# codename0og/codename-rvc-fork-3

Measured on AMD Instinct MI355X. Metric: 48 kHz audio samples/sec end-to-end VC, higher is better.
Workload: dtype f32 (vocoder ResBlock convs and upsamplers, HuBERT, RMVPE's U-Net convs: fp32 operands as exact bf16x3 splits on the bf16 matrix cores -- six products of order <= 2^-16 per multiply-add, fp32 accumulate; everything else fp32 / fp64)

## Files before the change

### codename-rvc-fork-3_amd/csrc/attention.hip

```cpp
#include <stdlib.h>

#include "common.h"

namespace rvc {

constexpr int ATT_W = 10;
constexpr int ATT_NREL = 2 * ATT_W + 1;

__device__ __forceinline__ float fast_exp2(float x) { return __builtin_amdgcn_exp2f(x); }

struct AttParams {
    const float *qkv;
    const float *emb_k;
    const float *emb_v;
    float *out;
    float *part_o;
    float *part_ml;
    int64_t T;
    int n_heads, n_splits, tiles_per_split;
    float scale_log2e;
};

template <int D, bool REL>
__global__ void __launch_bounds__(64) __attribute__((amdgpu_waves_per_eu(1, 2)))
attention_qkv_kernel(const AttParams p) {
    constexpr int NJ = D / 8;
    constexpr int ND = D / 32;
    __shared__ float rel_s[REL ? 32 * 33 : 1];
    __shared__ float band_s[REL ? 32 * 33 : 1];
    const int lane = threadIdx.x, j = lane & 31, h = lane >> 5;
    const int64_t T = p.T;
    const int n_heads = p.n_heads;
    const int64_t q0 = (int64_t)blockIdx.x * 32;
    const int head = blockIdx.y % n_heads;
    const int64_t b = blockIdx.y / n_heads;
    const int split = blockIdx.z;
    const int64_t rs = (int64_t)3 * n_heads * D;
    const float *qp = p.qkv + b * T * rs + (int64_t)head * D;
    const char *kp = reinterpret_cast<const char *>(qp + (int64_t)n_heads * D);
    const char *vp = reinterpret_cast<const char *>(qp + (int64_t)2 * n_heads * D);
    const uint32_t rs_b = (uint32_t)rs * 4u;
    const int nt_all = (int)((T + 31) / 32);
    const int t_begin = split * p.tiles_per_split;
    const int t_end = min(nt_all, t_begin + p.tiles_per_split);
    const bool partial = (T & 31) != 0;

    f32x4 qf[NJ];
    {
        const int64_t q = q0 + j < T ? q0 + j : T - 1;
        const float *ptr = qp + q * rs + 4 * h;
#pragma unroll
        for (int jj = 0; jj < NJ; ++jj) qf[jj] = *reinterpret_cast<const f32x4 *>(ptr + 8 * jj) * p.scale_log2e;
    }
    auto load_k = [&](f32x4 (&ka)[NJ], int t) __attribute__((always_inline)) {
        const int64_t key = (int64_t)t * 32 + j;
        const uint32_t off = (uint32_t)(key < T ? key : T - 1) * rs_b + 16u * h;
#pragma unroll
        for (int jj = 0; jj < NJ; ++jj) ka[jj] = *reinterpret_cast<const f32x4 *>(kp + off + 32u * jj);
    };
    uint32_t voff[16];
#pragma unroll
    for (int r = 0; r < 16; ++r) voff[r] = (uint32_t)((r & 3) + 8 * (r >> 2) + 4 * h) * rs_b + 4u * j;
    auto load_v = [&](float (&va)[16][ND], int t) __attribute__((always_inline)) {
        const char *vt = vp + (int64_t)t * 32 * rs_b;
        if (t + 1 < nt_all || !partial) {
#pragma unroll
            for (int r = 0; r < 16; ++r)
#pragma unroll
                for (int dt = 0; dt < ND; ++dt) va[r][dt] = *reinterpret_cast<const float *>(vt + voff[r] + 128u * dt);
        } else {
#pragma unroll
            for (int r = 0; r < 16; ++r) {
                const int64_t key = (int64_t)t * 32 + (r & 3) + 8 * (r >> 2) + 4 * h;
                const uint32_t off = (uint32_t)(key < T ? key : T - 1) * rs_b + 4u * j;
#pragma unroll
                for (int dt = 0; dt < ND; ++dt) va[r][dt] = *reinterpret_cast<const float *>(vp + off + 128u * dt);
            }
        }
    };
    auto scores = [&](const f32x4 (&ka)[NJ]) __attribute__((always_inline)) {
        f32x16 s;
#pragma unroll
        for (int r = 0; r < 16; ++r) s[r] = 0.f;
#pragma unroll
        for (int jj = 0; jj < NJ; ++jj)
#pragma unroll
            for (int e = 0; e < 4; ++e) s = mfma32(ka[jj][e], qf[jj][e], s);
        return s;
    };

    f32x16 o[ND];
#pragma unroll
    for (int dt = 0; dt < ND; ++dt)
#pragma unroll
        for (int r = 0; r < 16; ++r) o[dt][r] = 0.f;
    float m = -INFINITY, l = 0.f;

    if constexpr (REL) {
        f32x4 ek[NJ];
        const float *eptr = p.emb_k + (int64_t)(j < ATT_NREL ? j : 0) * D + 4 * h;
#pragma unroll
        for (int jj = 0; jj < NJ; ++jj) {
            ek[jj] = *reinterpret_cast<const f32x4 *>(eptr + 8 * jj);
            if (j >= ATT_NREL) ek[jj] = f32x4{0.f, 0.f, 0.f, 0.f};
        }
        const f32x16 rl = scores(ek);
#pragma unroll
        for (int r = 0; r < 16; ++r) {
            const int rr = (r & 3) + 8 * (r >> 2) + 4 * h;
            rel_s[j * 33 + rr] = rl[r];
            band_s[j * 33 + rr] = 0.f;
        }
        __syncthreads();
    }

    auto step = [&](int t, f32x4 (&k_cur)[NJ], const f32x4 (&k_next)[NJ], f32x16 &s_cur, f32x16 &s_next)
                    __attribute__((always_inline)) {
        float va[16][ND];
        load_v(va, t);
        if (t + 2 < t_end) load_k(k_cur, t + 2);
        if (t + 1 < t_end) s_next = scores(k_next);
        const bool near_diag = REL && (int64_t)t * 32 + 31 + ATT_W >= q0 && (int64_t)t * 32 <= q0 + 31 + ATT_W;
        int rr[16];
        if constexpr (REL) {
            if (near_diag) {
#pragma unroll
                for (int r = 0; r < 16; ++r) {
                    rr[r] = (int)((int64_t)t * 32 + (r & 3) + 8 * (r >> 2) + 4 * h - (q0 + j)) + ATT_W;
                    const bool in = rr[r] >= 0 && rr[r] < ATT_NREL;
                    const float add = rel_s[j * 33 + (in ? rr[r] : 0)];
                    s_cur[r] += in ? add : 0.f;
                }
            }
        }
        if (t + 1 == nt_all && partial) {
#pragma unroll
            for (int r = 0; r < 16; ++r)
                s_cur[r] = (int64_t)t * 32 + (r & 3) + 8 * (r >> 2) + 4 * h < T ? s_cur[r] : -INFINITY;
        }
        float mloc = s_cur[0];
#pragma unroll
        for (int r = 1; r < 16; ++r) mloc = fmaxf(mloc, s_cur[r]);
        mloc = fmaxf(mloc, __shfl_xor(mloc, 32));
        if (__any(mloc > m + 8.f)) {
            const float m_new = fmaxf(m, mloc);
            const float alpha = fast_exp2(m - m_new);
            l *= alpha;
#pragma unroll
            for (int dt = 0; dt < ND; ++dt)
#pragma unroll
                for (int r = 0; r < 16; ++r) o[dt][r] *= alpha;
            if constexpr (REL) {
#pragma unroll
                for (int r = 0; r < 16; ++r) band_s[j * 33 + 2 * r + h] *= alpha;
            }
            m = m_new;
        }
        float psum = 0.f;
#pragma unroll
        for (int r = 0; r < 16; ++r) {
            s_cur[r] = fast_exp2(s_cur[r] - m);
            psum += s_cur[r];
        }
        l += psum;
        if constexpr (REL) {
            if (near_diag) {
#pragma unroll
                for (int r = 0; r < 16; ++r)
                    if (rr[r] >= 0 && rr[r] < ATT_NREL) band_s[j * 33 + rr[r]] = s_cur[r];
            }
        }
#pragma unroll
        for (int r = 0; r < 16; ++r)
#pragma unroll
            for (int dt = 0; dt < ND; ++dt) o[dt] = mfma32(va[r][dt], s_cur[r], o[dt]);
    };

    if (t_begin < t_end) {
        f32x4 ka[NJ], kb[NJ];
        f32x16 sa, sb;
        load_k(ka, t_begin);
        if (t_begin + 1 < t_end) load_k(kb, t_begin + 1);
        sa = scores(ka);
        for (int t = t_begin; t < t_end; t += 2) {
            step(t, ka, kb, sa, sb);
            if (t + 1 < t_end) step(t + 1, kb, ka, sb, sa);
        }
    }
    if constexpr (REL) {
        __syncthreads();
#pragma unroll
        for (int sidx = 0; sidx < 16; ++sidx) {
            const int r = 2 * sidx + h;
            const float bval = band_s[j * 33 + r];
            const float *ev = p.emb_v + (int64_t)(r < ATT_NREL ? r : 0) * D + j;
#pragma unroll
            for (int dt = 0; dt < ND; ++dt) o[dt] = mfma32(ev[32 * dt], bval, o[dt]);
        }
    }
    l += __shfl_xor(l, 32);
    if (q0 + j < T) {
        if (p.n_splits == 1) {
            const float inv = 1.f / l;
            float *op = p.out + (b * T + q0 + j) * (int64_t)n_heads * D + (int64_t)head * D + 4 * h;
#pragma unroll
            for (int dt = 0; dt < ND; ++dt)
#pragma unroll
                for (int g = 0; g < 4; ++g) {
                    f32x4 v = {o[dt][4 * g], o[dt][4 * g + 1], o[dt][4 * g + 2], o[dt][4 * g + 3]};
                    *reinterpret_cast<f32x4 *>(op + 32 * dt + 8 * g) = v * inv;
                }
        } else {
            const int64_t row = ((b * n_heads + head) * p.n_splits + split) * T + q0 + j;
            float *op = p.part_o + row * D + 4 * h;
#pragma unroll
            for (int dt = 0; dt < ND; ++dt)
#pragma unroll
                for (int g = 0; g < 4; ++g) {
                    f32x4 v = {o[dt][4 * g], o[dt][4 * g + 1], o[dt][4 * g + 2], o[dt][4 * g + 3]};
                    *reinterpret_cast<f32x4 *>(op + 32 * dt + 8 * g) = v;
                }
            if (h == 0) {
                p.part_ml[row * 2] = m;
                p.part_ml[row * 2 + 1] = l;
            }
        }
    }
}

__global__ void __launch_bounds__(256)
attention_combine_kernel(const float *__restrict__ part_o, const float *__restrict__ part_ml, float *__restrict__ out,
                         int64_t T, int n_heads, int n_splits, int D) {
    const int64_t idx = (int64_t)blockIdx.x * 256 + threadIdx.x;
    const int d4n = D / 4;
    const int64_t total = (int64_t)gridDim.y * n_heads * T * d4n;
    (void)total;
    const int64_t b = blockIdx.y;
    if (idx >= (int64_t)n_heads * T * d4n) return;
    const int d4 = (int)(idx % d4n);
    const int64_t t = (idx / d4n) % T;
    const int head = (int)(idx / d4n / T);
    float mstar = -INFINITY;
    for (int s = 0; s < n_splits; ++s) mstar = fmaxf(mstar, part_ml[(((b * n_heads + head) * n_splits + s) * T + t) * 2]);
    f32x4 acc = {0.f, 0.f, 0.f, 0.f};
    float lsum = 0.f;
    for (int s = 0; s < n_splits; ++s) {
        const int64_t row = ((b * n_heads + head) * n_splits + s) * T + t;
        const float wgt = fast_exp2(part_ml[row * 2] - mstar);
        lsum += wgt * part_ml[row * 2 + 1];
        acc += *reinterpret_cast<const f32x4 *>(part_o + row * D + 4 * d4) * wgt;
    }
    *reinterpret_cast<f32x4 *>(out + (b * T + t) * (int64_t)n_heads * D + (int64_t)head * D + 4 * d4) = acc * (1.f / lsum);
}

struct AttBfParams {
    const float *qkv;
    const void *frag;
    float *out, *part_o, *part_ml;
    int64_t T;
    int n_heads, n_splits, tiles_per_split;
    float scale_log2e;
};
constexpr int ABF_TILE_BYTES = 24 * 1024, ABF_NW = 8;
typedef void __attribute__((address_space(3))) *abf_lptr_t;

__device__ __forceinline__ void abf_split8(const float (&v)[8], u32x4 (&out)[3]) {
    f32x2 r[4] = {f32x2{v[0], v[1]}, f32x2{v[2], v[3]}, f32x2{v[4], v[5]}, f32x2{v[6], v[7]}};
#pragma unroll
    for (int level = 0; level < 3; ++level)
#pragma unroll
        for (int q = 0; q < 4; ++q) {
            const unsigned w = split_word(r[q]);
            out[level][q] = w;
            if (level < 2) r[q] = r[q] - f32x2{__uint_as_float(w << 16), __uint_as_float(w & 0xffff0000u)};
        }
}

__global__ void __launch_bounds__(512) attention_pack_kv_kernel(const float *__restrict__ qkv, unsigned char *__restrict__ frag, int64_t T, int n_heads) {
    const int lane = threadIdx.x & 63, wave = threadIdx.x >> 6, i = lane & 31, h = lane >> 5;
    const int64_t tile = blockIdx.x, n_tiles = gridDim.x;
    const int head = blockIdx.y % n_heads;
    const int64_t b = blockIdx.y / n_heads;
    const int64_t rs = (int64_t)3 * n_heads * 64;
    const float *base = qkv + b * T * rs + (int64_t)head * 64;
    float v[8];
    int piece0;
    if (wave < 4) {
        const int64_t key = tile * 32 + i;
        const float *ptr = base + (int64_t)n_heads * 64 + (key < T ? key : 0) * rs + 16 * wave + 8 * h;
#pragma unroll
        for (int e = 0; e < 8; ++e) v[e] = key < T ? ptr[e] : 0.f;
        piece0 = wave * 3;
    } else {
        const int db = (wave - 4) >> 1, ks = wave & 1;
#pragma unroll
        for (int e = 0; e < 8; ++e) {
            const int r = 8 * ks + e;
            const int64_t key = tile * 32 + (r & 3) + 8 * (r >> 2) + 4 * h;
            v[e] = key < T ? base[(int64_t)2 * n_heads * 64 + key * rs + 32 * db + i] : 0.f;
        }
        piece0 = 12 + (db * 2 + ks) * 3;
    }
    u32x4 d[3];
    abf_split8(v, d);
    unsigned char *dst = frag + ((int64_t)blockIdx.y * n_tiles + tile) * ABF_TILE_BYTES + lane * 16;
#pragma unroll
    for (int sp = 0; sp < 3; ++sp) *reinterpret_cast<u32x4 *>(dst + (piece0 + sp) * 1024) = d[sp];
}

template <int DBG = 0>
__global__ void __launch_bounds__(512) __attribute__((amdgpu_waves_per_eu(2, 2)))
attention_bf_kernel(const AttBfParams p) {
    extern __shared__ __attribute__((aligned(16))) unsigned char abf_smem[];
    const int tid = threadIdx.x, lane = tid & 63, j = lane & 31, h = lane >> 5;
    const int wave = __builtin_amdgcn_readfirstlane(tid >> 6);
    const int64_t T = p.T;
    const int n_heads = p.n_heads;
    const int64_t q0 = ((int64_t)blockIdx.x * ABF_NW + wave) * 32;
    const bool active = q0 < T;
    const int head = blockIdx.y % n_heads;
    const int64_t b = blockIdx.y / n_heads;
    const int split = blockIdx.z;
    const int64_t rs = (int64_t)3 * n_heads * 64;
    const int nt_all = (int)((T + 31) / 32);
    const int t_begin = split * p.tiles_per_split;
    const int t_end = (DBG & 16) ? min(nt_all, t_begin + 1) : min(nt_all, t_begin + p.tiles_per_split);
    const bool partial = (T & 31) != 0;
    constexpr int ia6[6] = {0, 1, 0, 2, 1, 0}, ib6[6] = {2, 1, 1, 0, 0, 0};

    const int64_t n_frag = (int64_t)gridDim.y * nt_all * ABF_TILE_BYTES;
    const __amdgpu_buffer_rsrc_t frs = __builtin_amdgcn_make_buffer_rsrc((void *)p.frag, 0, (int)n_frag, RSRC_RAW32);
    const int bh_base = (int)((int64_t)blockIdx.y * nt_all) * ABF_TILE_BYTES;
    constexpr int HALF = ABF_TILE_BYTES / 2;
    auto dma = [&](int tk, int kslot, int tv, int vslot) __attribute__((always_inline)) {
#pragma unroll
        for (int n = 0; n < 3; ++n) {
            const int piece = wave + ABF_NW * n;
            if (piece < 12) {
                if (tk >= 0) __builtin_amdgcn_raw_ptr_buffer_load_lds(frs, (abf_lptr_t)(abf_smem + kslot * HALF + piece * 1024), 16, 16 * lane, bh_base + tk * ABF_TILE_BYTES + piece * 1024, 0, 0);
            } else {
                if (tv >= 0) __builtin_amdgcn_raw_ptr_buffer_load_lds(frs, (abf_lptr_t)(abf_smem + 2 * HALF + vslot * HALF + (piece - 12) * 1024), 16, 16 * lane, bh_base + tv * ABF_TILE_BYTES + piece * 1024, 0, 0);
            }
        }
    };
    if (t_begin < t_end) {
        dma(t_begin, 0, t_begin, 0);
        dma(t_begin + 1 < t_end ? t_begin + 1 : -1, 1, -1, 0);
    }
    u32x4 qf[4][3];
    {
        const int64_t q = q0 + j < T ? q0 + j : T - 1;
        const float *ptr = p.qkv + b * T * rs + (int64_t)head * 64 + q * rs + 8 * h;
#pragma unroll
        for (int ks = 0; ks < 4; ++ks) {
            const f32x4 lo = *reinterpret_cast<const f32x4 *>(ptr + 16 * ks) * p.scale_log2e, hi = *reinterpret_cast<const f32x4 *>(ptr + 16 * ks + 4) * p.scale_log2e;
            const float v[8] = {lo.x, lo.y, lo.z, lo.w, hi.x, hi.y, hi.z, hi.w};
            abf_split8(v, qf[ks]);
        }
    }
    auto scores = [&](int kslot) __attribute__((always_inline)) {
        const unsigned char *kk = abf_smem + kslot * HALF + lane * 16;
        f32x16 sc;
#pragma unroll
        for (int r = 0; r < 16; ++r) sc[r] = 0.f;
#pragma unroll
        for (int ks = 0; ks < 4; ++ks) {
            bf16x8 kf[3];
#pragma unroll
            for (int sp = 0; sp < 3; ++sp) if (!(DBG & 4)) kf[sp] = __builtin_bit_cast(bf16x8, *reinterpret_cast<const u32x4 *>(kk + (ks * 3 + sp) * 1024));
#pragma unroll
            for (int i = 0; i < 6; ++i) if (!(DBG & 1)) sc = __builtin_amdgcn_mfma_f32_32x32x16_bf16(kf[ia6[i]], __builtin_bit_cast(bf16x8, qf[ks][ib6[i]]), sc, 0, 0, 0);
        }
        return sc;
    };

    f32x16 o[2];
#pragma unroll
    for (int db = 0; db < 2; ++db)
#pragma unroll
        for (int r = 0; r < 16; ++r) o[db][r] = 0.f;
    float m = -INFINITY, l = 0.f;

    if (t_begin < t_end) {
        asm volatile("s_waitcnt vmcnt(0)" ::: "memory");
        __builtin_amdgcn_s_barrier();
        f32x16 s_cur, s_next;
        if (active) s_cur = scores(0);
        asm volatile("s_waitcnt lgkmcnt(0)" ::: "memory");
        __builtin_amdgcn_s_barrier();
        for (int t = t_begin; t < t_end; ++t) {
            const int kb = (t - t_begin) & 1;
            if (!(DBG & 8)) dma(t + 2 < t_end ? t + 2 : -1, kb, t + 1 < t_end ? t + 1 : -1, kb ^ 1);
            if (active) {
                if (t + 1 < t_end) s_next = scores(kb ^ 1);
                f32x16 &sc = s_cur;
                if (t + 1 == nt_all && partial) {
#pragma unroll
                    for (int r = 0; r < 16; ++r) sc[r] = (int64_t)t * 32 + (r & 3) + 8 * (r >> 2) + 4 * h < T ? sc[r] : -INFINITY;
                }
                float mloc = sc[0];
#pragma unroll
                for (int r = 1; r < 16; ++r) mloc = fmaxf(mloc, sc[r]);
                mloc = fmaxf(mloc, __shfl_xor(mloc, 32));
                if (__any(mloc > m + 8.f)) {
                    const float m_new = fmaxf(m, mloc);
                    const float alpha = fast_exp2(m - m_new);
                    l *= alpha;
#pragma unroll
                    for (int db = 0; db < 2; ++db)
#pragma unroll
                        for (int r = 0; r < 16; ++r) o[db][r] *= alpha;
                    m = m_new;
                }
                float psum = 0.f;
                if (!(DBG & 2)) {
#pragma unroll
                    for (int r = 0; r < 16; ++r) {
                        sc[r] = fast_exp2(sc[r] - m);
                        psum += sc[r];
                    }
                }
                l += psum;
                u32x4 pf[2][3];
#pragma unroll
                for (int ks = 0; ks < 2; ++ks) {
                    const float v[8] = {sc[8 * ks], sc[8 * ks + 1], sc[8 * ks + 2], sc[8 * ks + 3], sc[8 * ks + 4], sc[8 * ks + 5], sc[8 * ks + 6], sc[8 * ks + 7]};
                    if (!(DBG & 2)) abf_split8(v, pf[ks]);
                }
                const unsigned char *vv = abf_smem + 2 * HALF + kb * HALF + lane * 16;
#pragma unroll
                for (int ks = 0; ks < 2; ++ks)
#pragma unroll
                    for (int db = 0; db < 2; ++db) {
                        bf16x8 vf[3];
#pragma unroll
                        for (int sp = 0; sp < 3; ++sp)
                            if (!(DBG & 4)) vf[sp] = __builtin_bit_cast(bf16x8, *reinterpret_cast<const u32x4 *>(vv + ((db * 2 + ks) * 3 + sp) * 1024));
#pragma unroll
                        for (int i = 0; i < 6; ++i)
                            if (!(DBG & 1)) o[db] = __builtin_amdgcn_mfma_f32_32x32x16_bf16(vf[ia6[i]], __builtin_bit_cast(bf16x8, pf[ks][ib6[i]]), o[db], 0, 0, 0);
                    }
                s_cur = s_next;
            }
            asm volatile("s_waitcnt vmcnt(0) lgkmcnt(0)" ::: "memory");
            __builtin_amdgcn_s_barrier();
        }
    }
    l += __shfl_xor(l, 32);
    if (active && q0 + j < T) {
        if (p.n_splits == 1) {
            const float inv = 1.f / l;
            float *op = p.out + (b * T + q0 + j) * (int64_t)n_heads * 64 + (int64_t)head * 64 + 4 * h;
#pragma unroll
            for (int db = 0; db < 2; ++db)
#pragma unroll
                for (int g = 0; g < 4; ++g) {
                    f32x4 v = {o[db][4 * g], o[db][4 * g + 1], o[db][4 * g + 2], o[db][4 * g + 3]};
                    *reinterpret_cast<f32x4 *>(op + 32 * db + 8 * g) = v * inv;
                }
        } else {
            const int64_t row = ((b * n_heads + head) * p.n_splits + split) * T + q0 + j;
            float *op = p.part_o + row * 64 + 4 * h;
#pragma unroll
            for (int db = 0; db < 2; ++db)
#pragma unroll
                for (int g = 0; g < 4; ++g) {
                    f32x4 v = {o[db][4 * g], o[db][4 * g + 1], o[db][4 * g + 2], o[db][4 * g + 3]};
                    *reinterpret_cast<f32x4 *>(op + 32 * db + 8 * g) = v;
                }
            if (h == 0) {
                p.part_ml[row * 2] = m;
                p.part_ml[row * 2 + 1] = l;
            }
        }
    }
}

static bool att_bf_enabled() {
    static const int on = knob("RVC_ATT_BF", 1);
    return on != 0;
}
static int choose_splits_bf(int64_t n_frames, int n_heads, int batch) {
    const int64_t nt = ceil_div(n_frames, 32);
    const int64_t groups = ceil_div(n_frames, 32 * ABF_NW) * n_heads * batch;
    int best = 1;
    double best_cost = 1e30;
    for (int s = 1; s <= 8 && s <= nt; ++s) {
        const double cost = (double)ceil_div(groups * s, 256) / s + 0.02 * s;
        if (cost < best_cost - 1e-9) { best_cost = cost; best = s; }
    }
    return best;
}
static size_t att_bf_workspace(int batch, int64_t n_frames, int n_heads, size_t *off_ml, size_t *off_frag) {
    const int splits = choose_splits_bf(n_frames, n_heads, batch);
    const size_t rows = splits == 1 ? 0 : (size_t)batch * n_heads * splits * (size_t)n_frames;
    const size_t o_bytes = align_up(rows * 64 * sizeof(float), 256), ml_bytes = align_up(rows * 2 * sizeof(float), 256);
    if (off_ml) *off_ml = o_bytes;
    if (off_frag) *off_frag = o_bytes + ml_bytes;
    return o_bytes + ml_bytes + align_up((size_t)batch * n_heads * (size_t)ceil_div(n_frames, 32) * ABF_TILE_BYTES, 256);
}

static int choose_splits(int64_t n_frames, int n_heads, int batch) {
    static const int forced = knob("RVC_ATT_SPLITS", 0);
    const int64_t nt = ceil_div(n_frames, 32);
    const int64_t pairs = nt * n_heads * batch;
    int best = 1;
    double best_cost = 1e30;
    for (int s = 1; s <= 8 && s <= nt; ++s) {
        const double cost = (double)ceil_div(pairs * s, 1024) / s + 0.02 * s;
        if (cost < best_cost - 1e-9) { best_cost = cost; best = s; }
    }
    if (forced > 0 && forced <= nt) best = forced;
    return best;
}

}

using namespace rvc;

static bool attention_shape_ok(int batch, int64_t n_frames, int n_heads, int head_dim) {
    return batch > 0 && n_heads > 0 && n_frames >= 0 && (head_dim == 64 || head_dim == 96);
}

extern "C" int rvc_attention_workspace_bytes(int batch, int64_t n_frames, int n_heads, int head_dim, size_t *bytes) {
    if (!bytes) return fail("rvc_attention_workspace_bytes: null pointer");
    if (head_dim != 64 && head_dim != 96) return fail("rvc_attention_workspace_bytes: head_dim must be 64 or 96, got %d", head_dim);
    if (!attention_shape_ok(batch, n_frames, n_heads, head_dim)) return fail("rvc_attention_workspace_bytes: bad shape");
    const int splits = choose_splits(n_frames, n_heads, batch);
    const size_t rows = (size_t)batch * n_heads * splits * (size_t)n_frames;
    *bytes = splits == 1 ? 256 : align_up(rows * head_dim * sizeof(float), 256) + align_up(rows * 2 * sizeof(float), 256);
    if (head_dim == 64 && att_bf_enabled()) {
        const size_t bf = att_bf_workspace(batch, n_frames, n_heads, nullptr, nullptr);
        if (bf > *bytes) *bytes = bf;
    }
    return 0;
}

template <int D, bool REL>
static int launch_attention(AttParams &p, int batch, hipStream_t stream) {
    dim3 grid((unsigned)ceil_div(p.T, 32), (unsigned)(p.n_heads * batch), (unsigned)p.n_splits);
    hipLaunchKernelGGL((attention_qkv_kernel<D, REL>), grid, dim3(64), 0, stream, p);
    RVC_LAUNCH_CHECK();
    if (p.n_splits > 1) {
        const int64_t work = (int64_t)p.n_heads * p.T * (D / 4);
        hipLaunchKernelGGL(attention_combine_kernel, dim3((unsigned)ceil_div(work, 256), (unsigned)batch), dim3(256), 0, stream,
                           p.part_o, p.part_ml, p.out, p.T, p.n_heads, p.n_splits, D);
        RVC_LAUNCH_CHECK();
    }
    return 0;
}

extern "C" int rvc_attention_qkv_f32(const float *qkv_dev, const float *emb_rel_k_dev, const float *emb_rel_v_dev,
                                     float *out_dev, int batch, int64_t n_frames, int n_heads, int head_dim, float scale,
                                     void *workspace_dev, size_t workspace_bytes, void *stream) {
    if (!qkv_dev || !out_dev) return fail("rvc_attention_qkv_f32: null pointer");
    if (head_dim != 64 && head_dim != 96) return fail("rvc_attention_qkv_f32: head_dim must be 64 or 96, got %d", head_dim);
    if ((emb_rel_k_dev == nullptr) != (emb_rel_v_dev == nullptr)) return fail("rvc_attention_qkv_f32: emb_rel_k and emb_rel_v go together");
    if (!attention_shape_ok(batch, n_frames, n_heads, head_dim)) return fail("rvc_attention_qkv_f32: bad shape");
    if (n_frames == 0) return 0;
    if ((int64_t)n_frames * 3 * n_heads * head_dim * 4 >= ((int64_t)1 << 32))
        return fail("rvc_attention_qkv_f32: one batch element of %lld frames exceeds the 4 GB the kernel addresses", (long long)n_frames);
    if (head_dim == 64 && !emb_rel_k_dev && att_bf_enabled() && fits_2gib((int64_t)batch * n_heads * ceil_div(n_frames, 32), ABF_TILE_BYTES)) {
        size_t off_ml = 0, off_frag = 0;
        const size_t need = att_bf_workspace(batch, n_frames, n_heads, &off_ml, &off_frag);
        if (!workspace_dev || workspace_bytes < need) return fail("rvc_attention_qkv_f32: workspace too small (%zu < %zu)", workspace_bytes, need);
        AttBfParams q;
        q.qkv = qkv_dev; q.out = out_dev; q.T = n_frames; q.n_heads = n_heads; q.scale_log2e = scale * 1.4426950408889634f;
        q.n_splits = choose_splits_bf(n_frames, n_heads, batch);
        q.tiles_per_split = (int)ceil_div(ceil_div(n_frames, 32), q.n_splits);
        q.part_o = (float *)workspace_dev; q.part_ml = (float *)((char *)workspace_dev + off_ml); q.frag = (char *)workspace_dev + off_frag;
        hipStream_t st = (hipStream_t)stream;
        const unsigned n_tiles = (unsigned)ceil_div(n_frames, 32);
        const dim3 bgrid((unsigned)ceil_div(n_frames, 32 * ABF_NW), (unsigned)(n_heads * batch), (unsigned)q.n_splits);
        const auto run = [&](auto kernel) -> int {
            if (reserve_whole_cu((const void *)kernel, "rvc_attention_qkv_f32")) return 1;
            hipLaunchKernelGGL(attention_pack_kv_kernel, dim3(n_tiles, (unsigned)(n_heads * batch)), dim3(512), 0, st, qkv_dev, (unsigned char *)q.frag, q.T, n_heads);
            RVC_LAUNCH_CHECK();
            hipLaunchKernelGGL(kernel, bgrid, dim3(512), LDS_WHOLE_CU, st, q);
            RVC_LAUNCH_CHECK();
            return 0;
        };
        int dbg = 0;
#ifdef RVC_ABLATE
        static const int dbg_knob = knob("RVC_ATT_DBG", 0);
        dbg = dbg_knob;
#endif
        int rc;
        switch (dbg) {
#ifdef RVC_ABLATE
            case 1: rc = run(attention_bf_kernel<1>); break;
            case 2: rc = run(attention_bf_kernel<2>); break;
            case 4: rc = run(attention_bf_kernel<4>); break;
            case 8: rc = run(attention_bf_kernel<8>); break;
            case 16: rc = run(attention_bf_kernel<16>); break;
            case 7: rc = run(attention_bf_kernel<7>); break;
#endif
            default: rc = run(attention_bf_kernel<0>); break;
        }
        if (rc) return 1;
        if (q.n_splits > 1) {
            const int64_t work = (int64_t)n_heads * q.T * (64 / 4);
            hipLaunchKernelGGL(attention_combine_kernel, dim3((unsigned)ceil_div(work, 256), (unsigned)batch), dim3(256), 0, st,
                               q.part_o, q.part_ml, q.out, q.T, n_heads, q.n_splits, 64);
            RVC_LAUNCH_CHECK();
        }
        return 0;
    }
    AttParams p;
    p.qkv = qkv_dev; p.emb_k = emb_rel_k_dev; p.emb_v = emb_rel_v_dev; p.out = out_dev;
    p.T = n_frames; p.n_heads = n_heads; p.scale_log2e = scale * 1.4426950408889634f;
    p.n_splits = choose_splits(n_frames, n_heads, batch);
    p.tiles_per_split = (int)ceil_div(ceil_div(n_frames, 32), p.n_splits);
    p.part_o = nullptr; p.part_ml = nullptr;
    if (p.n_splits > 1) {
        size_t need = 0;
        if (rvc_attention_workspace_bytes(batch, n_frames, n_heads, head_dim, &need)) return 1;
        if (!workspace_dev || workspace_bytes < need) return fail("rvc_attention_qkv_f32: workspace too small (%zu < %zu)", workspace_bytes, need);
        const size_t rows = (size_t)batch * n_heads * p.n_splits * (size_t)n_frames;
        p.part_o = (float *)workspace_dev;
        p.part_ml = (float *)((char *)workspace_dev + align_up(rows * head_dim * sizeof(float), 256));
    }
    const bool rel = emb_rel_k_dev != nullptr;
    hipStream_t st = (hipStream_t)stream;
    if (head_dim == 64) return rel ? launch_attention<64, true>(p, batch, st) : launch_attention<64, false>(p, batch, st);
    return rel ? launch_attention<96, true>(p, batch, st) : launch_attention<96, false>(p, batch, st);
}
```

### codename-rvc-fork-3_amd/csrc/bf16x3.h

```cpp
#pragma once

#include <hip/hip_runtime.h>

namespace rvc {

typedef __bf16 bf16x2 __attribute__((ext_vector_type(2)));
typedef __bf16 bf16x8 __attribute__((ext_vector_type(8)));
typedef float f32x2 __attribute__((ext_vector_type(2)));
typedef unsigned u32x2 __attribute__((ext_vector_type(2)));
typedef unsigned u32x4 __attribute__((ext_vector_type(4)));

constexpr int RSRC_RAW32 = 0x00020000;
constexpr unsigned BUF_OOB = 0x80000000u;

__device__ __forceinline__ float sub_np(float a, float b) {
    float r;
    asm("v_sub_f32 %0, %1, %2" : "=v"(r) : "v"(a), "v"(b));
    return r;
}
__device__ __forceinline__ float add_np(float a, float b) {
    float r;
    asm("v_add_f32 %0, %1, %2" : "=v"(r) : "v"(a), "v"(b));
    return r;
}
__device__ __forceinline__ float mul_np(float a, float b) {
    float r;
    asm("v_mul_f32 %0, %1, %2" : "=v"(r) : "v"(a), "v"(b));
    return r;
}

__device__ __forceinline__ unsigned split_word(f32x2 v) { return __builtin_bit_cast(unsigned, __builtin_convertvector(v, bf16x2)); }
__device__ __forceinline__ f32x2 split_rest(f32x2 v, unsigned w) { return v - f32x2{__uint_as_float(w << 16), __uint_as_float(w & 0xffff0000u)}; }
__device__ __forceinline__ void split3(f32x2 v, unsigned w[3]) {
#pragma unroll
    for (int level = 0; level < 3; ++level) {
        w[level] = split_word(v);
        if (level < 2) v = split_rest(v, w[level]);
    }
}
__device__ __forceinline__ void split3_np(float a, float b, unsigned w[3]) {
#pragma unroll
    for (int level = 0; level < 3; ++level) {
        const unsigned ww = split_word(f32x2{a, b});
        w[level] = ww;
        if (level < 2) {
            a = sub_np(a, __uint_as_float(ww << 16));
            b = sub_np(b, __uint_as_float(ww & 0xffff0000u));
        }
    }
}

}
```

### codename-rvc-fork-3_amd/csrc/linbf.hip

```cpp
#include <stdlib.h>

#include <mutex>
#include <vector>

#include "conv.h"

namespace rvc {

struct LinBfParams {
    const void *a = nullptr;
    const void *xs = nullptr;
    const float *bias = nullptr;
    float *y = nullptr;
    void *ys = nullptr;
    int M = 0, K = 0;
    int64_t N = 0, n_pad = 0;
    int mode = 0;
    int64_t x_row_stride = 0, x_plane = 0;
    int steps_per_part = 0;
    int n_col_blocks = 0;
};

constexpr int LBF_BN = 128, LBF_NTH = 512;
constexpr int LBF_SLAB_STEP = 12 * 1024;
constexpr int LBF_B_CHUNK = 3 * LBF_BN * 64;
typedef void __attribute__((address_space(3))) *lbf_lptr_t;

template <int MI>
struct LbfGeom {
    static constexpr int BM = 64 * MI;
    static constexpr int A_STEP = 2 * MI * 3 * 1024;
    static constexpr int D = MI == 2 ? 2 : 1;
    static constexpr int A_RING = 2 * (D + 1), B_RING = D + 1;
    static constexpr int NPIECE = 2 * 2 * MI * 3 + 24;
    static constexpr int UPW = (NPIECE + 7) / 8;
    static constexpr int LDS_USED = A_RING * A_STEP + B_RING * LBF_B_CHUNK;
    static_assert(LDS_USED <= 163840, "");
};

template <int MI>
__global__ void __launch_bounds__(LBF_NTH) __attribute__((amdgpu_waves_per_eu(2, 2)))
linbf_kernel(const LinBfParams p) {
    using GM = LbfGeom<MI>;
    constexpr int BM = GM::BM, A_STEP = GM::A_STEP, D = GM::D, A_RING = GM::A_RING, B_RING = GM::B_RING, NPIECE = GM::NPIECE, UPW = GM::UPW;
    extern __shared__ __attribute__((aligned(16))) unsigned char lbf_smem[];
    unsigned char *const a_ring = lbf_smem;
    unsigned char *const b_ring = lbf_smem + A_RING * A_STEP;
    const int tid = threadIdx.x, lane = tid & 63;
    const int wave = __builtin_amdgcn_readfirstlane(tid >> 6);
    __builtin_assume(wave >= 0 && wave < 8);
    const int wm = wave >> 2, wn = wave & 3;
    const int half = lane >> 5, l31 = lane & 31;
    const int n_m = p.M / BM;
    const int xcd = blockIdx.x & 7, slot = blockIdx.x >> 3;
    const int pairs = p.n_col_blocks * n_m, per_xcd = (pairs + 7) / 8;
    const int w = xcd * per_xcd + slot;
    if (slot >= per_xcd || w >= pairs) return;
    const int col_blk = w / n_m, mblk = w - col_blk * n_m, part = blockIdx.y;
    const int m0 = mblk * BM;
    const int64_t n0 = (int64_t)col_blk * LBF_BN;
    const int n_chunks = p.steps_per_part / 2, s_first = part * p.steps_per_part;
    const int K = p.K;

    const __amdgpu_buffer_rsrc_t ars = __builtin_amdgcn_make_buffer_rsrc((void *)p.a, 0, (int)((int64_t)p.M * K * 6), RSRC_RAW32);
    const __amdgpu_buffer_rsrc_t xrs = __builtin_amdgcn_make_buffer_rsrc((void *)p.xs, 0, (int)(3 * p.x_plane * 2), RSRC_RAW32);
    const int slab_row = (K / 16) * LBF_SLAB_STEP;
    const int plane = (int)(p.x_plane * 2);
    const int row_bytes = (int)(p.x_row_stride * 2);
    const int b_r = lane >> 2, b_j = lane & 3;
    auto dma = [&](int c) __attribute__((always_inline)) {
        const int sg = s_first + 2 * c;
        unsigned char *bslot = b_ring + (c % B_RING) * LBF_B_CHUNK;
#pragma unroll
        for (int i = 0; i < UPW; ++i) {
            int pc = wave + 8 * i;
            if (pc >= NPIECE) pc -= 8;
            if (pc < 12 * MI) {
                const int st = pc / (6 * MI), f = pc - st * (6 * MI);
                const int rb = (m0 >> 5) + f / 3, sp = f - (f / 3) * 3;
                unsigned char *aslot = a_ring + ((2 * c + st) % A_RING) * A_STEP;
                __builtin_amdgcn_raw_ptr_buffer_load_lds(ars, (lbf_lptr_t)(aslot + f * 1024), 16, 16 * lane,
                                                         (rb >> 2) * slab_row + (sg + st) * LBF_SLAB_STEP + ((rb & 3) * 3 + sp) * 1024, 0, 0);
            } else {
                const int q = pc - 12 * MI, sp = q >> 3, r16 = q & 7;
                const int row = r16 * 16 + b_r;
                const int seg = b_j ^ ((row >> 2) & 3);
                const int voff = (int)(n0 + row) * row_bytes + seg * 16;
                __builtin_amdgcn_raw_ptr_buffer_load_lds(xrs, (lbf_lptr_t)(bslot + sp * (LBF_BN * 64) + r16 * 1024), 16, voff, sp * plane + sg * 32, 0, 0);
            }
        }
    };

    f32x16 acc[MI];
#pragma unroll
    for (int mi = 0; mi < MI; ++mi)
#pragma unroll
        for (int r = 0; r < 16; ++r) acc[mi][r] = 0.f;
    auto rd = [&](const unsigned char *ptr) __attribute__((always_inline)) {
        return __builtin_bit_cast(bf16x8, *reinterpret_cast<const u32x4 *>(ptr));
    };
    const int nrow = wn * 32 + l31;
    const int b_lane = nrow * 64, b_sw = (nrow >> 2) & 3;

    auto wait_newer = [&](int newer) __attribute__((always_inline)) {
        if (newer >= 1 && D >= 2) asm volatile("s_waitcnt vmcnt(%0)" ::"n"(UPW) : "memory");
        else asm volatile("s_waitcnt vmcnt(0)" ::: "memory");
    };
    static_assert(D <= 2, "wait_newer distinguishes 0 and 1 newer requests");
#pragma unroll
    for (int c = 0; c < D; ++c)
        if (c < n_chunks) dma(c);
    wait_newer((n_chunks - 1 < D - 1) ? n_chunks - 1 : D - 1);
    lds_barrier();
    for (int c = 0; c < n_chunks; ++c) {
        if (c + D < n_chunks) dma(c + D);
        const unsigned char *bslot = b_ring + (c % B_RING) * LBF_B_CHUNK + b_lane;
#pragma unroll
        for (int t = 0; t < 2; ++t) {
            const unsigned char *ab = a_ring + ((2 * c + t) % A_RING) * A_STEP + wm * MI * 3 * 1024 + lane * 16;
            bf16x8 fa[MI][3], fb[3];
#pragma unroll
            for (int sp = 0; sp < 3; ++sp) fb[sp] = rd(bslot + sp * (LBF_BN * 64) + (((2 * t + half) ^ b_sw) * 16));
#pragma unroll
            for (int mi = 0; mi < MI; ++mi)
#pragma unroll
                for (int sp = 0; sp < 3; ++sp) fa[mi][sp] = rd(ab + (mi * 3 + sp) * 1024);
            constexpr int ia[6] = {2, 0, 1, 1, 0, 0}, ib[6] = {0, 2, 1, 0, 1, 0};
#pragma unroll
            for (int i = 0; i < 6; ++i)
#pragma unroll
                for (int mi = 0; mi < MI; ++mi)
                    acc[mi] = __builtin_amdgcn_mfma_f32_32x32x16_bf16(fa[mi][ia[i]], fb[ib[i]], acc[mi], 0, 0, 0);
        }
        const int newer = (n_chunks - 2 - c) < (D - 1) ? (n_chunks - 2 - c) : (D - 1);
        wait_newer(newer);
        lds_barrier();
    }

    if (p.mode == 1) {
        const int64_t n = n0 + nrow;
        const bool live = n < p.N;
#pragma unroll
        for (int mi = 0; mi < MI; ++mi) {
            const int mb = m0 + wm * 32 * MI + mi * 32;
#pragma unroll
            for (int rp = 0; rp < 2; ++rp) {
                f32x2 v[2][2];
#pragma unroll
                for (int g = 0; g < 2; ++g) {
                    f32x4 o;
#pragma unroll
                    for (int r = 0; r < 4; ++r) o[r] = acc[mi][4 * (2 * rp + g) + r];
                    if (p.bias) o += *reinterpret_cast<const f32x4 *>(p.bias + mb + 4 * half + 8 * (2 * rp + g));
#pragma unroll
                    for (int r = 0; r < 4; ++r) o[r] = 0.5f * o[r] * (1.f + erff(o[r] * 0.70710678118654752f));
                    v[g][0] = f32x2{o[0], o[1]};
                    v[g][1] = f32x2{o[2], o[3]};
                }
#pragma unroll
                for (int sp = 0; sp < 3; ++sp) {
                    unsigned w[2][2];
#pragma unroll
                    for (int g = 0; g < 2; ++g)
#pragma unroll
                        for (int h = 0; h < 2; ++h) {
                            w[g][h] = split_word(v[g][h]);
                            v[g][h] = split_rest(v[g][h], w[g][h]);
                        }
                    const unsigned s0 = half ? w[0][0] : w[1][0], s1 = half ? w[0][1] : w[1][1];
                    const unsigned r0 = (unsigned)__shfl_xor((int)s0, 32, 64), r1 = (unsigned)__shfl_xor((int)s1, 32, 64);
                    const u32x4 out = half ? u32x4{r0, r1, w[1][0], w[1][1]} : u32x4{w[0][0], w[0][1], r0, r1};
                    const int m = mb + 16 * rp + 8 * half;
                    if (live) *reinterpret_cast<u32x4 *>(reinterpret_cast<unsigned char *>(p.ys) + (((int64_t)sp * p.n_pad + n) * p.M + m) * 2) = out;
                }
            }
        }
        return;
    }
#pragma unroll
    for (int mi = 0; mi < MI; ++mi) {
        const int64_t n = n0 + nrow;
        if (n >= p.N) continue;
        const int mb = m0 + wm * 32 * MI + mi * 32 + 4 * half;
#pragma unroll
        for (int rg = 0; rg < 4; ++rg) {
            const int m = mb + 8 * rg;
            f32x4 o;
#pragma unroll
            for (int r = 0; r < 4; ++r) o[r] = acc[mi][4 * rg + r];
            if (p.mode == 2) {
                *reinterpret_cast<f32x4 *>(p.y + ((int64_t)part * p.N + n) * p.M + m) = o;
                continue;
            }
            if (p.bias) o += *reinterpret_cast<const f32x4 *>(p.bias + m);
            if (p.mode == 0) {
                *reinterpret_cast<f32x4 *>(p.y + n * p.M + m) = o;
                continue;
            }
#pragma unroll
            for (int r = 0; r < 4; ++r) o[r] = 0.5f * o[r] * (1.f + erff(o[r] * 0.70710678118654752f));
            *reinterpret_cast<f32x4 *>(p.y + n * p.M + m) = o;
        }
    }
}

__global__ void __launch_bounds__(256) split_rows_kernel(const float *__restrict__ x, unsigned char *__restrict__ xs, int64_t n_rows,
                                                          int64_t n_pad, int k) {
    const int64_t i4 = (int64_t)blockIdx.x * 256 + threadIdx.x;
    const int64_t total4 = n_rows * k / 4;
    if (i4 >= total4) return;
    const f32x4 v = *reinterpret_cast<const f32x4 *>(x + i4 * 4);
    f32x2 v0 = {v.x, v.y}, v1 = {v.z, v.w};
#pragma unroll
    for (int sp = 0; sp < 3; ++sp) {
        const unsigned w0 = split_word(v0), w1 = split_word(v1);
        *reinterpret_cast<u32x2 *>(xs + ((int64_t)sp * n_pad * k + i4 * 4) * 2) = u32x2{w0, w1};
        v0 = split_rest(v0, w0);
        v1 = split_rest(v1, w1);
    }
}

__device__ __forceinline__ float ln_row_mean(float sum, float inv_m) {
    float mean = sum * inv_m;
    asm volatile("" : "+v"(mean));
    return mean;
}

template <int PER_LANE>
__global__ void __launch_bounds__(256) ln_reduce_kernel(const float *__restrict__ parts, int n_parts, const float *__restrict__ bias,
                                                         const float *__restrict__ res, const float *__restrict__ gamma,
                                                         const float *__restrict__ beta, float eps, float *__restrict__ y,
                                                         unsigned char *__restrict__ ys, int64_t n_rows, int64_t n_pad) {
    constexpr int M = 64 * PER_LANE, Q = PER_LANE / 4;
    const int lane = threadIdx.x & 63;
    const int64_t n = (int64_t)blockIdx.x * 4 + (threadIdx.x >> 6);
    if (n >= n_rows) return;
    f32x4 v[Q];
#pragma unroll
    for (int q = 0; q < Q; ++q) {
        const int m = (q * 64 + lane) * 4;
        f32x4 a = bias ? *reinterpret_cast<const f32x4 *>(bias + m) : f32x4{0.f, 0.f, 0.f, 0.f};
        for (int s = 0; s < n_parts; ++s) a += *reinterpret_cast<const f32x4 *>(parts + ((int64_t)s * n_rows + n) * M + m);
        if (res) a += *reinterpret_cast<const f32x4 *>(res + n * M + m);
        v[q] = a;
    }
    float sum = 0.f;
#pragma unroll
    for (int q = 0; q < Q; ++q) sum += (v[q].x + v[q].y) + (v[q].z + v[q].w);
#pragma unroll
    for (int o = 32; o > 0; o >>= 1) sum += __shfl_xor(sum, o, 64);
    const float mean = ln_row_mean(sum, 1.f / M);
    float sq = 0.f;
#pragma unroll
    for (int q = 0; q < Q; ++q) {
        const f32x4 d = v[q] - mean;
        sq += (d.x * d.x + d.y * d.y) + (d.z * d.z + d.w * d.w);
    }
#pragma unroll
    for (int o = 32; o > 0; o >>= 1) sq += __shfl_xor(sq, o, 64);
    const float rstd = 1.f / sqrtf(sq * (1.f / M) + eps);
#pragma unroll
    for (int q = 0; q < Q; ++q) {
        const int m = (q * 64 + lane) * 4;
        f32x4 o = (v[q] - mean) * rstd;
        if (gamma) o *= *reinterpret_cast<const f32x4 *>(gamma + m);
        if (beta) o += *reinterpret_cast<const f32x4 *>(beta + m);
        if (y) *reinterpret_cast<f32x4 *>(y + n * M + m) = o;
        if (ys) {
            f32x2 v0 = {o.x, o.y}, v1 = {o.z, o.w};
#pragma unroll
            for (int sp = 0; sp < 3; ++sp) {
                const unsigned w0 = split_word(v0), w1 = split_word(v1);
                *reinterpret_cast<u32x2 *>(ys + (((int64_t)sp * n_pad + n) * M + m) * 2) = u32x2{w0, w1};
                v0 = split_rest(v0, w0);
                v1 = split_rest(v1, w1);
            }
        }
    }
}

template <int MI>
static int linbf_launch(LinBfParams p, int parts, hipStream_t stream) {
    if (reserve_whole_cu((const void *)linbf_kernel<MI>, "linear bf16x3 (pre-split)")) return 1;
    p.n_col_blocks = (int)ceil_div(p.N, LBF_BN);
    const int n_m = p.M / LbfGeom<MI>::BM;
    dim3 grid((unsigned)(ceil_div((int64_t)p.n_col_blocks * n_m, 8) * 8), (unsigned)parts, 1);
    hipLaunchKernelGGL(linbf_kernel<MI>, grid, dim3(LBF_NTH), LDS_WHOLE_CU, stream, p);
    RVC_LAUNCH_CHECK();
    return 0;
}

}

using namespace rvc;

extern "C" int rvc_split_rows_bf16x3(const float *x_dev, void *xs_dev, int64_t n_rows, int64_t n_rows_padded, int k, void *stream) {
    if (!x_dev || !xs_dev) return fail("rvc_split_rows_bf16x3: null pointer");
    if (k % 16 || n_rows_padded < n_rows || n_rows < 0) return fail("rvc_split_rows_bf16x3: k must be a multiple of 16, n_rows_padded >= n_rows");
    if (n_rows == 0) return 0;
    const int64_t total4 = n_rows * k / 4;
    hipLaunchKernelGGL(split_rows_kernel, dim3((unsigned)ceil_div(total4, 256)), dim3(256), 0, (hipStream_t)stream, x_dev,
                       reinterpret_cast<unsigned char *>(xs_dev), n_rows, n_rows_padded, k);
    RVC_LAUNCH_CHECK();
    return 0;
}

namespace {
int linbf_dispatch(const char *who, const void *xs_dev, int64_t x_row_stride, int64_t x_plane, const void *a_dev, const float *bias_dev,
                   float *y_dev, void *ys_dev, int64_t n_rows, int64_t n_rows_padded, int in_features, int out_features, int mode,
                   int k_parts, void *stream) {
    if (!xs_dev || !a_dev) return fail("%s: null pointer", who);
    if (out_features % 128 || in_features % 16) return fail("%s: out_features must be a multiple of 128, in_features of 16", who);
    if (mode < 0 || mode > 3) return fail("%s: mode must be 0 (fp32 + bias), 1 (bias + GELU -> planes), 2 (partial sums) or 3 (bias + GELU -> fp32)", who);
    if ((mode == 1) ? !ys_dev : !y_dev) return fail("%s: the output of mode %d is missing", who, mode);
    if (k_parts < 1 || (in_features / 32) % k_parts || in_features % 32) return fail("%s: in_features must be a multiple of 32 and k_parts divide in_features / 32", who);
    if (k_parts > 1 && mode != 2) return fail("%s: several K parts only produce partial sums (mode 2)", who);
    if (n_rows_padded % LBF_BN || n_rows_padded < n_rows) return fail("%s: n_rows_padded must be a multiple of 128 and >= n_rows", who);
    if (!fits_2gib((int64_t)out_features * in_features, 6) || !fits_2gib(3 * x_plane, 2) ||
        !fits_2gib((n_rows_padded + LBF_BN) * x_row_stride, 2))
        return fail("%s: an operand exceeds 2 GiB", who);
    if (x_row_stride % 8) return fail("%s: rows must start on 16-byte boundaries", who);
    if (n_rows <= 0) return 0;
    LinBfParams p;
    p.a = a_dev; p.xs = xs_dev; p.bias = bias_dev; p.y = y_dev; p.ys = ys_dev;
    p.M = out_features; p.K = in_features; p.N = n_rows; p.n_pad = n_rows_padded; p.mode = mode;
    p.x_row_stride = x_row_stride; p.x_plane = x_plane;
    p.steps_per_part = in_features / 16 / k_parts;
    const int64_t cols = ceil_div(n_rows, LBF_BN);
    const int cus = 256;
    auto cost = [&](int rows_per_block, double rel) {
        if (out_features % rows_per_block) return 1e30;
        return (double)ceil_div(cols * (out_features / rows_per_block) * k_parts, cus) * rel;
    };
    static const int by_cu_time = knob("RVC_LBF_TP", 0);
    if (by_cu_time) {
        auto cu_time = [&](int rows_per_block, double rel) { return out_features % rows_per_block ? 1e30 : cols * (out_features / rows_per_block) * k_parts * rel; };
        const double t128 = cu_time(128, 1.0), t192 = cu_time(192, 1.5 * 0.85), t256 = cu_time(256, 1.85);
        if (t192 <= t128 && t192 <= t256) return linbf_launch<3>(p, k_parts, (hipStream_t)stream);
        if (t256 < t128) return linbf_launch<4>(p, k_parts, (hipStream_t)stream);
        return linbf_launch<2>(p, k_parts, (hipStream_t)stream);
    }
    const double c128 = cost(128, 1.0), c192 = cost(192, 1.5 * 0.85), c256 = cost(256, 1.85);
    if (c256 < c128 && c256 <= c192) return linbf_launch<4>(p, k_parts, (hipStream_t)stream);
    const bool use192 = c192 < c128;
    return use192 ? linbf_launch<3>(p, k_parts, (hipStream_t)stream) : linbf_launch<2>(p, k_parts, (hipStream_t)stream);
}
}

extern "C" int rvc_linear_bf16x3_presplit(const void *xs_dev, const void *a_dev, const float *bias_dev, float *y_dev, void *ys_dev,
                                          int64_t n_rows, int64_t n_rows_padded, int in_features, int out_features, int mode, int k_parts,
                                          void *stream) {
    return linbf_dispatch("rvc_linear_bf16x3_presplit", xs_dev, in_features, n_rows_padded * in_features, a_dev, bias_dev, y_dev, ys_dev,
                          n_rows, n_rows_padded, in_features, out_features, mode, k_parts, stream);
}

extern "C" int rvc_conv1d_frames_bf16x3(const void *xs_dev, int64_t n_frames_in, int64_t n_frames_in_padded, int channels, int taps,
                                        int stride, const void *a_dev, const float *bias_dev, float *y_dev, void *ys_dev,
                                        int64_t n_frames_out_padded, int out_channels, int mode, void *stream) {
    if (taps < 1 || stride < 1 || channels < 8 || n_frames_in_padded < n_frames_in) return fail("rvc_conv1d_frames_bf16x3: bad argument");
    if (mode == 2) return fail("rvc_conv1d_frames_bf16x3: modes 0 (fp32 + bias), 1 (bias + GELU -> planes), 3 (bias + GELU -> fp32)");
    const int64_t n_out = n_frames_in >= taps ? (n_frames_in - taps) / stride + 1 : 0;
    return linbf_dispatch("rvc_conv1d_frames_bf16x3", xs_dev, (int64_t)stride * channels, n_frames_in_padded * channels, a_dev, bias_dev,
                          y_dev, ys_dev, n_out, n_frames_out_padded, taps * channels, out_channels, mode, 1, stream);
}

extern "C" int rvc_bias_residual_layernorm_bf16x3(const float *parts_dev, int n_parts, const float *bias_dev, const float *res_dev,
                                                  const float *gamma_dev, const float *beta_dev, float eps, float *y_dev, void *ys_dev,
                                                  int64_t n_rows, int64_t n_rows_padded, int features, void *stream) {
    if (!parts_dev || (!y_dev && !ys_dev)) return fail("rvc_bias_residual_layernorm_bf16x3: null pointer");
    if (n_parts < 1 || n_rows_padded < n_rows) return fail("rvc_bias_residual_layernorm_bf16x3: bad argument");
    if (n_rows <= 0) return 0;
    dim3 grid((unsigned)ceil_div(n_rows, 4));
    unsigned char *ys = reinterpret_cast<unsigned char *>(ys_dev);
    hipStream_t st = (hipStream_t)stream;
    if (features == 768)
        hipLaunchKernelGGL(ln_reduce_kernel<12>, grid, dim3(256), 0, st, parts_dev, n_parts, bias_dev, res_dev, gamma_dev, beta_dev, eps, y_dev, ys, n_rows, n_rows_padded);
    else if (features == 1024)
        hipLaunchKernelGGL(ln_reduce_kernel<16>, grid, dim3(256), 0, st, parts_dev, n_parts, bias_dev, res_dev, gamma_dev, beta_dev, eps, y_dev, ys, n_rows, n_rows_padded);
    else if (features == 256)
        hipLaunchKernelGGL(ln_reduce_kernel<4>, grid, dim3(256), 0, st, parts_dev, n_parts, bias_dev, res_dev, gamma_dev, beta_dev, eps, y_dev, ys, n_rows, n_rows_padded);
    else
        return fail("rvc_bias_residual_layernorm_bf16x3: features must be 256, 768 or 1024 (HuBERT-base: 768)");
    RVC_LAUNCH_CHECK();
    return 0;
}
```

### codename-rvc-fork-3_amd/rvc_amd/_native.py

```python
from __future__ import annotations

import ctypes
import threading
import os
from ctypes import POINTER, c_char_p, c_float, c_int, c_int64, c_size_t, c_void_p

import torch

_HERE = os.path.dirname(os.path.abspath(__file__))
LIB_PATH = os.path.join(_HERE, "_lib", "librvc_amd.so")
if os.environ.get("RVC_AMD_LIB"):
    LIB_PATH = os.path.abspath(os.environ["RVC_AMD_LIB"])
    print(f"[rvc_amd] RVC_AMD_LIB: loading {LIB_PATH} instead of the product library", flush=True)


class NativeError(RuntimeError):
    pass


if not os.path.isfile(LIB_PATH):
    raise ImportError(
        f"{LIB_PATH} is missing: build it with `python -c 'import __graft_entry__ as g; g.build()'` "
        "(hipcc --offload-arch=gfx950).  rvc_amd has no fallback path without its HIP library.")

_lib = ctypes.CDLL(LIB_PATH)


class DecoderConfig(ctypes.Structure):
    _fields_ = [
        ("kind", c_int), ("sample_rate", c_int), ("in_channels", c_int), ("upsample_initial_channel", c_int),
        ("gin_channels", c_int), ("n_ups", c_int), ("upsample_rates", c_int * 8), ("upsample_kernel_sizes", c_int * 8),
        ("n_res_kernels", c_int), ("res_kernel_sizes", c_int * 4), ("res_dilations", c_int * 4),
        ("n_res_dilations", c_int), ("weight_storage", c_int),
    ]


class DecoderNoise(ctypes.Structure):
    _fields_ = [("src_rand_dev", c_void_p), ("src_randn_dev", c_void_p), ("adain_randn_dev", c_void_p)]


SYMBOLS = {
    "rvc_abi_version": (c_int, []),
    "rvc_last_error": (c_char_p, []),
    "rvc_knn_index_aux_bytes": (c_int, [c_int64, c_int, POINTER(c_size_t)]),
    "rvc_knn_index_build": (c_int, [c_void_p, c_int64, c_int, c_void_p, c_size_t, c_void_p]),
    "rvc_knn_set_mode": (c_int, [c_int]),
    "rvc_knn_rank_candidates": (c_int, [c_void_p, c_void_p, c_int64, c_int, c_void_p, c_int64, c_void_p, c_int, c_int, c_void_p,
                                        c_void_p, c_void_p]),
    "rvc_knn_workspace_bytes": (c_int, [c_int64, c_int64, c_int, c_int, POINTER(c_size_t)]),
    "rvc_knn_search": (c_int, [c_void_p, c_void_p, c_int64, c_int, c_void_p, c_int64, c_int, c_void_p, c_void_p,
                               c_void_p, c_size_t, c_void_p]),
    "rvc_knn_blend": (c_int, [c_void_p, c_int, c_void_p, c_void_p, c_void_p, c_int64, c_int, c_float, c_void_p,
                              c_void_p]),
    "rvc_logmel_workspace_bytes": (c_int, [c_int, c_int64, POINTER(c_size_t)]),
    "rvc_logmel_rmvpe": (c_int, [c_void_p, c_int, c_int64, c_void_p, c_int64, c_void_p, c_size_t, c_void_p]),
    "rvc_mel_create": (c_int, [c_int, c_int, c_int, c_int, c_float, c_float, c_void_p, c_int, POINTER(c_void_p)]),
    "rvc_mel_destroy": (c_int, [c_void_p]),
    "rvc_mel_frames": (c_int, [c_void_p, c_int64, POINTER(c_int64)]),
    "rvc_mel_workspace_bytes": (c_int, [c_void_p, c_int, c_int64, POINTER(c_size_t)]),
    "rvc_mel_forward": (c_int, [c_void_p, c_void_p, c_int, c_int64, c_void_p, c_void_p, c_void_p, c_size_t, c_void_p]),
    "rvc_resample_poly_f64": (c_int, [c_void_p, c_int64, c_int, c_int, c_void_p, c_int64, c_void_p, c_int64, c_void_p]),
    "rvc_filtfilt_workspace_bytes": (c_int, [c_int64, POINTER(c_size_t)]),
    "rvc_filtfilt_order5": (c_int, [c_void_p, c_int64, c_void_p, c_void_p, c_void_p, c_size_t, c_void_p]),
    "rvc_bigru_workspace_bytes": (c_int, [c_int, POINTER(c_size_t)]),
    "rvc_bigru_forward": (c_int, [c_void_p, c_void_p, c_void_p, c_void_p, c_int, c_int64, c_int, c_void_p, c_size_t,
                                  c_void_p]),
    "rvc_bigru_status": (c_int, [c_void_p, c_int, POINTER(c_int), c_void_p]),
    "rvc_bigru_set_spin_limit": (c_int, [ctypes.c_uint]),
    "rvc_attention_workspace_bytes": (c_int, [c_int, c_int64, c_int, c_int, POINTER(c_size_t)]),
    "rvc_attention_qkv_f32": (c_int, [c_void_p, c_void_p, c_void_p, c_void_p, c_int, c_int64, c_int, c_int, c_float,
                                      c_void_p, c_size_t, c_void_p]),
    "rvc_bias_relu_add_f32": (c_int, [c_void_p, c_void_p, c_void_p, c_void_p, c_int, c_int, c_int64, c_int, c_void_p]),
    "rvc_gate_tanh_sigmoid_f32": (c_int, [c_void_p, c_void_p, c_int, c_int, c_int64, c_void_p]),
    "rvc_rownorm_gelu_f32": (c_int, [c_void_p, c_void_p, c_void_p, c_void_p, c_int, c_int, c_int64, ctypes.c_float, c_void_p]),
    "rvc_set_concurrency_hint": (c_int, [c_int]),
    "rvc_decoder_create": (c_int, [POINTER(DecoderConfig), POINTER(c_void_p)]),
    "rvc_decoder_set_tensor": (c_int, [c_void_p, c_char_p, c_void_p, POINTER(c_int64), c_int]),
    "rvc_decoder_finalize": (c_int, [c_void_p]),
    "rvc_decoder_destroy": (c_int, [c_void_p]),
    "rvc_decoder_upp": (c_int, [c_void_p]),
    "rvc_decoder_workspace_bytes": (c_int, [c_void_p, c_int, c_int64, POINTER(c_size_t)]),
    "rvc_decoder_forward": (c_int, [c_void_p, c_void_p, c_void_p, c_void_p, POINTER(DecoderNoise), c_int, c_int64,
                                    c_void_p, c_void_p, c_size_t, c_void_p]),
    "rvc_decoder_window_margin": (c_int, [POINTER(DecoderConfig), POINTER(c_int)]),
    "rvc_decoder_forward_window": (c_int, [c_void_p, c_void_p, c_void_p, c_void_p, POINTER(DecoderNoise), c_int, c_int64, c_int64,
                                           c_int64, c_void_p, c_void_p, c_size_t, c_void_p]),
    "rvc_decoder_set_tap": (c_int, [c_void_p, c_int, c_void_p]),
    "rvc_decoder_set_concurrency_hint": (c_int, [c_void_p, c_int]),
    "rvc_decoder_set_branch_parallel": (c_int, [c_void_p, c_int]),
    "rvc_posconv_bf16x3_weight_bytes": (c_int, [c_int, c_int, c_int, POINTER(c_size_t)]),
    "rvc_posconv_bf16x3_pack_weight": (c_int, [c_void_p, c_int, c_int, c_int, c_void_p, c_void_p]),
    "rvc_posconv_gelu_bf16x3": (c_int, [c_void_p, c_void_p, c_void_p, c_void_p, c_int64, c_int, c_int, c_int, c_int, c_void_p]),
    "rvc_hubert_conv0_workspace_bytes": (c_int, [c_int, POINTER(c_size_t)]),
    "rvc_hubert_conv0_frames_bf16x3": (c_int, [c_void_p, c_int64, c_void_p, c_int, c_int, c_int, c_void_p, c_void_p, c_float, c_void_p,
                                               c_size_t, c_void_p, c_int64, c_void_p]),
    "rvc_conv1d_frames_bf16x3": (c_int, [c_void_p, c_int64, c_int64, c_int, c_int, c_int, c_void_p, c_void_p, c_void_p, c_void_p, c_int64,
                                         c_int, c_int, c_void_p]),
    "rvc_conv1d_pack_weight": (c_int, [c_void_p, c_int, c_int, c_int, c_void_p, c_void_p]),
    "rvc_conv1d_forward": (c_int, [c_void_p, c_void_p, c_void_p, c_void_p, c_void_p, c_void_p, c_int, c_int, c_int,
                                   c_int64, c_int, c_int, c_float, c_float, c_void_p]),
    "rvc_conv1d_wino_pack_weight": (c_int, [c_void_p, c_int, c_int, c_int, c_void_p, c_void_p]),
    "rvc_conv1d_wino_forward": (c_int, [c_void_p, c_void_p, c_void_p, c_void_p, c_void_p, c_void_p, c_int, c_int, c_int,
                                        c_int64, c_int, c_int, c_float, c_float, c_void_p]),
    "rvc_conv1d_winobf_weight_bytes": (c_int, [c_int, c_int, c_int, POINTER(c_size_t)]),
    "rvc_conv1d_winobf_pack_weight": (c_int, [c_void_p, c_int, c_int, c_int, c_void_p, c_void_p]),
    "rvc_conv1d_winobf_forward": (c_int, [c_void_p, c_void_p, c_void_p, c_void_p, c_void_p, c_void_p, c_int, c_int, c_int,
                                          c_int64, c_int, c_int, c_float, c_float, c_void_p]),
    "rvc_resblock_bf16x3_weight_bytes": (c_int, [c_int, c_int, POINTER(c_size_t)]),
    "rvc_resblock_bf16x3_pack_weight": (c_int, [c_void_p, c_void_p, c_int, c_int, c_void_p, c_void_p]),
    "rvc_resblock_bf16x3_forward": (c_int, [c_void_p, c_void_p, c_void_p, c_void_p, c_void_p, c_void_p, c_int, c_int, c_int64, c_int,
                                            c_int, c_float, c_float, c_void_p]),
    "rvc_resblock_bf16w_weight_bytes": (c_int, [c_int, c_int, POINTER(c_size_t)]),
    "rvc_resblock_bf16w_pack_weight": (c_int, [c_void_p, c_void_p, c_int, c_int, c_void_p, c_void_p]),
    "rvc_resblock_bf16w_forward": (c_int, [c_void_p, c_void_p, c_void_p, c_void_p, c_void_p, c_void_p, c_int, c_int, c_int64, c_int,
                                           c_int, c_float, c_float, c_void_p]),
    "rvc_resblock_bf16x3_set_enabled": (c_int, [c_int]),
    "rvc_upsample_bf16x3_weight_bytes": (c_int, [c_int, c_int, c_int, c_int, c_int, c_int, POINTER(c_size_t)]),
    "rvc_upsample_bf16x3_pack_weight": (c_int, [c_void_p, c_void_p, c_void_p, c_int, c_int, c_int, c_int, c_int, c_int, c_void_p, c_void_p]),
    "rvc_upsample_bf16x3_forward": (c_int, [c_void_p, c_void_p, c_int64, c_void_p, c_void_p, c_void_p, c_int, c_int, c_int, c_int64, c_int, c_int,
                                            c_int, c_int, c_int, c_int, c_float, c_void_p]),
    "rvc_conv1d_f16x2_weight_bytes": (c_int, [c_int, c_int, POINTER(c_size_t)]),
    "rvc_conv1d_f16x2_pack_weight": (c_int, [c_void_p, c_int, c_int, c_void_p, c_void_p]),
    "rvc_conv1d_f16x2_forward": (c_int, [c_void_p, c_void_p, c_void_p, c_void_p, c_void_p, c_void_p, c_int, c_int, c_int64, c_int,
                                         c_int, c_float, c_float, c_void_p]),
    "rvc_decoder_set_arithmetic": (c_int, [c_void_p, c_int]),
    "rvc_conv1d_bf16w_weight_bytes": (c_int, [c_int, c_int, POINTER(c_size_t)]),
    "rvc_conv1d_bf16w_pack_weight": (c_int, [c_void_p, c_int, c_int, c_void_p, c_void_p]),
    "rvc_conv1d_bf16w_forward": (c_int, [c_void_p, c_void_p, c_void_p, c_void_p, c_void_p, c_void_p, c_int, c_int, c_int64, c_int,
                                         c_int, c_float, c_float, c_void_p]),
    "rvc_gemm_bf16x3_weight_bytes": (c_int, [c_int, c_int, POINTER(c_size_t)]),
    "rvc_gemm_bf16x3_pack_weight": (c_int, [c_void_p, c_int, c_int, c_int, c_void_p, c_void_p]),
    "rvc_linear_bf16x3": (c_int, [c_void_p, c_void_p, c_void_p, c_void_p, c_void_p, c_int64, c_int, c_int, c_int, c_void_p]),
    "rvc_conv1d_bf16x3": (c_int, [c_void_p, c_void_p, c_void_p, c_void_p, c_int, c_int, c_int, c_int64, c_int, c_int, c_int, c_int,
                                  c_void_p]),
    "rvc_split_rows_bf16x3": (c_int, [c_void_p, c_void_p, c_int64, c_int64, c_int, c_void_p]),
    "rvc_linear_bf16x3_presplit": (c_int, [c_void_p, c_void_p, c_void_p, c_void_p, c_void_p, c_int64, c_int64, c_int, c_int, c_int, c_int,
                                           c_void_p]),
    "rvc_bias_residual_layernorm_bf16x3": (c_int, [c_void_p, c_int, c_void_p, c_void_p, c_void_p, c_void_p, c_float, c_void_p, c_void_p,
                                                   c_int64, c_int64, c_int, c_void_p]),
    "rvc_conv2d_packed_floats": (c_int, [c_int, c_int, c_int, c_int, POINTER(c_size_t)]),
    "rvc_conv2d_pack_weight": (c_int, [c_void_p, c_int, c_int, c_int, c_int, c_void_p, c_void_p]),
    "rvc_conv2d_workspace_bytes": (c_int, [c_int, c_int, c_int, c_int, c_int, c_int, c_int, POINTER(c_size_t)]),
    "rvc_conv2d_bf16x3_supported": (c_int, [c_int, c_int, c_int, c_int]),
    "rvc_conv2d_bf16x3_weight_bytes": (c_int, [c_int, c_int, c_int, c_int, POINTER(c_size_t)]),
    "rvc_conv2d_bf16x3_pack_weight": (c_int, [c_void_p, c_int, c_int, c_int, c_int, c_void_p, c_void_p]),
    "rvc_conv2d_bf16x3_workspace_bytes": (c_int, [c_int, c_int, c_int, c_int, c_int, POINTER(c_size_t)]),
    "rvc_conv2d_bf16x3_forward": (c_int, [c_void_p, c_void_p, c_void_p, c_void_p, c_void_p, c_int, c_int, c_int, c_int, c_int, c_int,
                                          c_void_p, c_size_t, c_void_p]),
    "rvc_conv2d_forward": (c_int, [c_void_p, c_void_p, c_void_p, c_void_p, c_void_p, c_int, c_int, c_int, c_int, c_int, c_int,
                                   c_int, c_int, c_void_p, c_size_t, c_void_p]),
    "rvc_comm_unique_id": (c_int, [c_void_p]),
    "rvc_comm_create": (c_int, [c_void_p, c_int, c_int, POINTER(c_void_p)]),
    "rvc_comm_destroy": (c_int, [c_void_p]),
    "rvc_comm_info": (c_int, [c_void_p, POINTER(c_int), POINTER(c_int), POINTER(c_int), c_char_p, c_size_t]),
    "rvc_index_broadcast": (c_int, [c_void_p, c_void_p, c_size_t, c_int, c_void_p]),
    "rvc_checksum64": (c_int, [c_void_p, c_size_t, c_void_p, c_void_p]),
    "rvc_glu_dwconv_silu_f32": (c_int, [c_void_p, c_void_p, c_void_p, c_void_p, c_int64, c_int, c_int, c_void_p]),
    "rvc_layernorm_rows_f32": (c_int, [c_void_p, c_void_p, c_void_p, c_float, c_void_p, c_int64, c_int, c_void_p]),
    "rvc_groupnorm_workspace_bytes": (c_int, [c_int, c_int64, c_int, POINTER(c_size_t)]),
    "rvc_groupnorm_lrelu_f32": (c_int, [c_void_p, c_void_p, c_void_p, c_int, c_float, c_float, c_void_p, c_int, c_int64, c_void_p,
                                        c_size_t, c_void_p]),
    "rvc_fcpe_decode_f32": (c_int, [c_void_p, c_void_p, c_int, c_int, c_float, c_float, c_void_p, c_void_p, c_int64, c_void_p]),
    "rvc_kmeans_workspace_bytes": (c_int, [c_int64, c_int64, c_int, POINTER(c_size_t)]),
    "rvc_kmeans_assign": (c_int, [c_void_p, c_int64, c_int, c_void_p, c_int64, c_void_p, c_void_p, c_void_p, c_size_t, c_void_p]),
    "rvc_kmeans_update": (c_int, [c_void_p, c_int64, c_int, c_void_p, c_void_p, c_int64, c_void_p, c_void_p, c_void_p, c_size_t,
                                  c_void_p]),
    "rvc_lfilter_order5_warmup": (c_int, [c_void_p, POINTER(c_int64)]),
    "rvc_lfilter_order5_f64": (c_int, [c_void_p, c_int64, c_void_p, c_void_p, c_void_p]),
    "rvc_frame_rms_frames": (c_int, [c_int64, c_int64, c_int64, POINTER(c_int64), POINTER(c_size_t)]),
    "rvc_frame_rms_f64": (c_int, [c_void_p, c_int64, c_int64, c_int64, c_void_p, c_int64, c_void_p, c_size_t, c_void_p]),
    "rvc_slice_export_f32": (c_int, [c_void_p, c_int64, c_void_p, c_void_p, c_void_p, c_void_p, c_int64, c_int, c_int, c_void_p,
                                     c_int64, c_void_p, c_int64, c_void_p, c_int64, c_void_p]),
    "rvc_spectral_gate_params": (c_int, [c_int, POINTER(c_int), POINTER(c_int), POINTER(ctypes.c_double), c_void_p, c_void_p]),
    "rvc_spectral_gate_workspace_bytes": (c_int, [c_int64, c_int, c_int64, c_int64, POINTER(c_size_t)]),
    "rvc_spectral_gate_f32": (c_int, [c_void_p, c_int64, c_int, c_float, c_int64, c_int64, c_void_p, c_void_p, c_size_t, c_void_p]),
    "rvc_formant_shift_workspace_bytes": (c_int, [c_int64, c_int, POINTER(c_size_t)]),
    "rvc_formant_shift_f32": (c_int, [c_void_p, c_int64, c_int, ctypes.c_double, ctypes.c_double, c_int, c_void_p, c_void_p, c_size_t,
                                      c_void_p]),
    "rvc_mrstft_sums_workspace_bytes": (c_int, [c_int64, POINTER(c_int), POINTER(c_int), POINTER(c_int), c_int, POINTER(c_size_t)]),
    "rvc_mrstft_sums_f32": (c_int, [c_void_p, c_void_p, c_int64, POINTER(c_int), POINTER(c_int), POINTER(c_int), c_int, ctypes.c_double,
                                    c_void_p, c_void_p, c_size_t, c_void_p]),
    "rvc_si_sdr_sums_workspace_bytes": (c_int, [c_int64, POINTER(c_size_t)]),
    "rvc_si_sdr_sums_f32": (c_int, [c_void_p, c_void_p, c_int64, c_void_p, c_void_p, c_size_t, c_void_p]),
    "rvc_mean_abs_diff_workspace_bytes": (c_int, [c_int64, c_int64, POINTER(c_size_t)]),
    "rvc_mean_abs_diff_f32": (c_int, [c_void_p, c_int64, c_void_p, c_int64, c_int64, c_int64, c_void_p, c_void_p, c_size_t, c_void_p]),
}

for _name, (_res, _args) in SYMBOLS.items():
    _fn = getattr(_lib, _name)
    _fn.restype = _res
    _fn.argtypes = _args

ABI_VERSION = 4
if _lib.rvc_abi_version() != ABI_VERSION:
    raise ImportError(f"librvc_amd.so ABI {_lib.rvc_abi_version()} != {ABI_VERSION}: rebuild it")


def _check(rc: int, what: str):
    if rc != 0:
        raise NativeError(f"{what}: {_lib.rvc_last_error().decode(errors='replace')}")


def _stream() -> int:
    return torch.cuda.current_stream().cuda_stream


def _call(name: str, device: torch.device, *args, stream: bool = True) -> None:
    if device.index != torch.cuda.current_device():
        if device.type != "cuda" or device.index is None:
            raise NativeError(f"{name}: every tensor must live in HBM, got one on {device}")
        with torch.cuda.device(device):
            return _call(name, device, *args, stream=stream)
    if stream:
        args += (torch.cuda.current_stream(device.index).cuda_stream,)
    _check(getattr(_lib, name)(*args), name)


def _device(*tensors) -> torch.device:
    device = None
    for t in tensors:
        if t is None:
            continue
        if device is None:
            device = t.device
        elif t.device != device:
            raise NativeError(f"the tensors of one call must share a device, got {device} and {t.device}")
    return device


def _cuda_device(device=None) -> torch.device:
    device = torch.device("cuda" if device is None else device)
    if device.type != "cuda":
        raise NativeError(f"a HIP device is needed, got {device} (no CPU fallback)")
    return device if device.index is not None else torch.device("cuda", torch.cuda.current_device())


def _ptr(t):
    return t.data_ptr() if t is not None else None


def _host(w: torch.Tensor) -> torch.Tensor:
    return w.detach().float().cpu().contiguous()


def _dev_f32(t: torch.Tensor, name: str) -> torch.Tensor:
    if not t.is_cuda:
        raise NativeError(f"{name} must live in HBM (got a {t.device} tensor); the HIP path has no CPU fallback")
    if t.dtype != torch.float32:
        raise NativeError(f"{name} must be float32, got {t.dtype}")
    return t.contiguous()


class _Workspace:

    def __init__(self):
        self._buf = {}
        self._lock = threading.Lock()

    def get(self, tag: str, nbytes: int, device) -> torch.Tensor:
        key = (tag, str(device), torch.cuda.current_stream(device).cuda_stream)
        with self._lock:
            buf = self._buf.get(key)
            if buf is None or buf.numel() < nbytes:
                buf = torch.empty(max(nbytes, 256), dtype=torch.uint8, device=device)
                self._buf[key] = buf
        return buf


_ws = _Workspace()


def _size(query: str, device, *dims) -> int:
    need = c_size_t()
    _call(query, device, *dims, ctypes.byref(need), stream=False)
    return need.value


def _workspace(tag: str, device, query: str, *dims) -> torch.Tensor:
    return _ws.get(tag, _size(query, device, *dims), device)


def _pack_slab(stem: str, device, host: tuple, size_dims: tuple, pack_dims: tuple = None) -> torch.Tensor:
    device = _cuda_device(device)
    slab = torch.empty(_size(stem + "_weight_bytes", device, *size_dims) // 2, dtype=torch.int16, device=device)
    _call(stem + "_pack_weight", device, *(_ptr(w) for w in host), *(size_dims if pack_dims is None else pack_dims), slab.data_ptr())
    return slab


def knn_index_build(index: torch.Tensor) -> torch.Tensor:
    index = _dev_f32(index, "index")
    n, d = index.shape[0], index.shape[1]
    aux = torch.empty(_size("rvc_knn_index_aux_bytes", index.device, n, d), dtype=torch.uint8, device=index.device)
    _call("rvc_knn_index_build", index.device, index.data_ptr(), n, d, aux.data_ptr(), aux.numel())
    return aux


knn_index_norms = knn_index_build


def knn_set_mode(mode: int) -> None:
    _check(_lib.rvc_knn_set_mode(int(mode)), "rvc_knn_set_mode")


def knn_search(index: torch.Tensor, aux: torch.Tensor, queries: torch.Tensor, k: int = 8):
    index, queries = _dev_f32(index, "index"), _dev_f32(queries, "queries")
    if not aux.is_cuda or aux.dtype != torch.uint8:
        raise NativeError("aux must be the uint8 HBM blob returned by knn_index_build")
    dev = _device(index, aux, queries)
    nq = queries.shape[0]
    d2 = torch.empty((nq, k), dtype=torch.float32, device=dev)
    ids = torch.empty((nq, k), dtype=torch.int64, device=dev)
    if nq == 0:
        return d2, ids
    ws = _workspace("knn", dev, "rvc_knn_workspace_bytes", index.shape[0], nq, index.shape[1], k)
    _call("rvc_knn_search", dev, index.data_ptr(), aux.data_ptr(), index.shape[0], index.shape[1], queries.data_ptr(), nq, k,
          d2.data_ptr(), ids.data_ptr(), ws.data_ptr(), ws.numel())
    return d2, ids


def knn_rank_candidates(index: torch.Tensor, aux: torch.Tensor, queries: torch.Tensor, cand: torch.Tensor, k: int = 8):
    index, queries = _dev_f32(index, "index"), _dev_f32(queries, "queries")
    if not cand.is_cuda or cand.dtype != torch.int32 or cand.dim() != 2 or cand.shape[0] != queries.shape[0]:
        raise NativeError("cand must be an int32 HBM tensor [n_queries, cap]")
    cand = cand.contiguous()
    dev = _device(index, aux, queries, cand)
    nq = queries.shape[0]
    d2 = torch.empty((nq, k), dtype=torch.float32, device=dev)
    ids = torch.empty((nq, k), dtype=torch.int64, device=dev)
    _call("rvc_knn_rank_candidates", dev, index.data_ptr(), aux.data_ptr(), index.shape[0], index.shape[1], queries.data_ptr(), nq,
          cand.data_ptr(), cand.shape[1], k, d2.data_ptr(), ids.data_ptr())
    return d2, ids


def knn_blend(index: torch.Tensor, feats: torch.Tensor, d2: torch.Tensor, ids: torch.Tensor, index_rate: float):
    index, feats, d2 = _dev_f32(index, "index"), _dev_f32(feats, "feats"), _dev_f32(d2, "d2")
    ids = ids.contiguous()
    out = torch.empty_like(feats)
    _call("rvc_knn_blend", _device(index, feats, d2, ids), index.data_ptr(), index.shape[1], feats.data_ptr(), d2.data_ptr(),
          ids.data_ptr(), feats.shape[0], d2.shape[1], float(index_rate), out.data_ptr())
    return out


def kmeans_assign(x: torch.Tensor, centroids: torch.Tensor):
    x, centroids = _dev_f32(x, "x"), _dev_f32(centroids, "centroids")
    if x.dim() != 2 or centroids.dim() != 2 or x.shape[1] != centroids.shape[1]:
        raise NativeError(f"x {tuple(x.shape)} and centroids {tuple(centroids.shape)} must be [n, d] and [k, d]")
    dev = _device(x, centroids)
    n, d = x.shape
    ids = torch.empty(n, dtype=torch.int32, device=dev)
    d2 = torch.empty(n, dtype=torch.float32, device=dev)
    if n == 0:
        return ids, d2
    ws = _workspace("kmeans", dev, "rvc_kmeans_workspace_bytes", n, centroids.shape[0], d)
    _call("rvc_kmeans_assign", dev, x.data_ptr(), n, d, centroids.data_ptr(), centroids.shape[0], ids.data_ptr(), d2.data_ptr(),
          ws.data_ptr(), ws.numel())
    return ids, d2


def kmeans_update(x: torch.Tensor, order: torch.Tensor, offsets: torch.Tensor, old: torch.Tensor) -> torch.Tensor:
    x, old = _dev_f32(x, "x"), _dev_f32(old, "old")
    n, d = x.shape
    k = old.shape[0]
    if (not order.is_cuda or order.dtype != torch.int32 or order.numel() != n or not offsets.is_cuda
            or offsets.dtype != torch.int64 or offsets.numel() != k + 1 or old.shape[1] != d):
        raise NativeError("order must be an int32 HBM tensor [n], offsets an int64 HBM tensor [k + 1], old [k, d]")
    if n == 0:
        return old.clone()
    order, offsets = order.contiguous(), offsets.contiguous()
    dev = _device(x, order, offsets, old)
    out = torch.empty_like(old)
    ws = _workspace("kmeans", dev, "rvc_kmeans_workspace_bytes", n, k, d)
    _call("rvc_kmeans_update", dev, x.data_ptr(), n, d, order.data_ptr(), offsets.data_ptr(), k, old.data_ptr(), out.data_ptr(),
          ws.data_ptr(), ws.numel())
    return out


def knn_roofline_report(n_rows: int, n_queries: int, dim: int, seconds: float, peak_hbm_gbs: float,
                        peak_f32_tflops: float, peak_f16_tflops: float, traffic=None, traffic_source=None) -> dict:
    screened = n_queries > 64 and n_rows >= 16384 and dim % 256 == 0
    stream = n_queries <= 64
    q_tile = 256 if screened else (32 if stream else 128)
    passes = -(-n_queries // q_tile)
    bytes_8d = passes * n_rows * dim * 4.0
    bytes_moved = passes * n_rows * dim * (2.0 if screened else 4.0) + (8.0 * n_queries * dim * 4 if screened else 0.0)
    flops = 2.0 * n_queries * n_rows * dim
    mfma_peak = peak_f16_tflops if screened else peak_f32_tflops
    hbm_gbs = bytes_moved / seconds / 1e9
    mfma_tf = flops / seconds / 1e12
    bound = "hbm" if stream else "mfma"
    out = {"kernel": ("knn_screen_kernel<false> (sample) + knn_select_kernel + knn_screen_kernel<true> (main, fp16 MFMA) + "
                      "knn_finalize_kernel (exact fp32 re-scoring)" if screened else
                      ("knn_direct_kernel" if stream else "knn_partial_kernel") + " + knn_finalize_kernel"),
           "regime": "fp16-screened, exact re-scoring" if screened else ("fp32 streaming" if stream else "fp32 GEMM"),
           "shape": f"{n_queries} queries x {n_rows} rows x {dim}", "bound": bound, "query_tile": q_tile, "passes": passes,
           "bytes_per_pass_8d": n_rows * dim * 4}
    if bound == "hbm":
        out.update({"achieved": round(hbm_gbs, 1), "peak": peak_hbm_gbs, "unit": "GB/s", "frac": round(hbm_gbs / peak_hbm_gbs, 4),
                    "frac_is": "physical: bytes the pass reads (n_rows x dim x 4) / search time / HBM peak"})
    else:
        out.update({"achieved": round(mfma_tf, 2), "peak": mfma_peak, "unit": "TFLOP/s", "frac": round(mfma_tf / mfma_peak, 4),
                    "frac_is": "2 x queries x rows x dim / search time / the dense " + ("fp16" if screened else "fp32") + " MFMA peak "
                               "(round 5 and earlier printed an HBM fraction here: now hbm_frac_physical / frac_8d)"})
    out.update({"bytes_moved_per_search": bytes_moved,
                "hbm_gbs_physical": round(hbm_gbs, 1), "hbm_frac_physical": round(hbm_gbs / peak_hbm_gbs, 4),
                "achieved_8d": round(bytes_8d / seconds / 1e9, 1), "frac_8d": round(bytes_8d / seconds / 1e9 / peak_hbm_gbs, 4),
                "frac_8d_is": "SURVEY 8d's formula (passes x n_rows x dim x 4 B / t / 8 TB/s): fp32 bytes the screened kernel never reads -- a footnote",
                "traffic": traffic, "traffic_source": traffic_source,
                "mfma_tflops": round(mfma_tf, 2), "mfma_frac": round(mfma_tf / mfma_peak, 4),
                "mfma_peak_used": "fp16 dense 2500 TF" if screened else "fp32 157.3 TF",
                "avg_search_ms": round(seconds * 1e3, 4)})
    return out


def logmel_rmvpe(audio: torch.Tensor, pad_to: int = 32) -> tuple[torch.Tensor, int]:
    audio = _dev_f32(audio, "audio")
    b, n = audio.shape
    t = n // 160 + 1
    t_pad = pad_to * ((t - 1) // pad_to + 1) if pad_to > 1 else t
    mel = torch.empty((b, 128, t_pad), dtype=torch.float32, device=audio.device)
    ws = _workspace("logmel", audio.device, "rvc_logmel_workspace_bytes", b, n)
    _call("rvc_logmel_rmvpe", audio.device, audio.data_ptr(), b, n, mel.data_ptr(), t_pad, ws.data_ptr(), ws.numel())
    return mel, t


class MelTransform:

    def __init__(self, n_fft: int, hop: int, win_length: int, pad: int, mel_matrix, mag_eps: float = 0.0, log_floor: float = 1e-5,
                 device=None):
        import numpy as np
        m = np.ascontiguousarray(mel_matrix, dtype=np.float32)
        if m.ndim != 2 or m.shape[1] != n_fft // 2 + 1:
            raise NativeError(f"mel matrix must be [n_mels, {n_fft // 2 + 1}], got {m.shape}")
        self.n_fft, self.hop, self.n_mels, self.bins = n_fft, hop, m.shape[0], n_fft // 2 + 1
        self.device = _cuda_device(device)
        self._h = c_void_p()
        with torch.cuda.device(self.device):
            _check(_lib.rvc_mel_create(n_fft, hop, win_length, pad, float(mag_eps), float(log_floor), m.ctypes.data, m.shape[0],
                                       ctypes.byref(self._h)), "rvc_mel_create")

    def __del__(self):
        if getattr(self, "_h", None) and _lib is not None:
            _lib.rvc_mel_destroy(self._h)
            self._h = None

    def n_frames(self, n_samples: int) -> int:
        t = c_int64()
        _check(_lib.rvc_mel_frames(self._h, n_samples, ctypes.byref(t)), "rvc_mel_frames")
        return t.value

    def forward(self, audio: torch.Tensor, want_mel: bool = True, want_spec: bool = False):
        audio = _dev_f32(audio, "audio")
        dev = self.device
        if audio.device != dev:
            raise NativeError(f"MelTransform of {dev} got audio on {audio.device}")
        b, n = audio.shape
        t = self.n_frames(n)
        mel = torch.empty((b, self.n_mels, t), dtype=torch.float32, device=dev) if want_mel else None
        spec = torch.empty((b, self.bins, t), dtype=torch.float32, device=dev) if want_spec else None
        ws = _workspace("mel", dev, "rvc_mel_workspace_bytes", self._h, b, n)
        _call("rvc_mel_forward", dev, self._h, audio.data_ptr(), b, n, _ptr(mel), _ptr(spec), ws.data_ptr(), ws.numel())
        return mel, spec


def resample_poly(x: torch.Tensor, up: int, down: int, h: torch.Tensor) -> torch.Tensor:
    if not (x.is_cuda and x.dtype == torch.float64 and x.dim() == 1 and h.is_cuda and h.dtype == torch.float64):
        raise NativeError("resample_poly wants 1-D float64 HBM tensors")
    x, h = x.contiguous(), h.contiguous()
    n_out = -(-x.numel() * up // down)
    y = torch.empty(n_out, dtype=torch.float64, device=x.device)
    _call("rvc_resample_poly_f64", _device(x, h), x.data_ptr(), x.numel(), int(up), int(down), h.data_ptr(), h.numel(), y.data_ptr(), n_out)
    return y


_ff_coef_cache = {}


def _filtfilt_coef(b, a):
    import numpy as np
    from scipy import signal
    key = (tuple(b), tuple(a))
    if key not in _ff_coef_cache:
        b = np.asarray(b, dtype=np.float64)
        a = np.asarray(a, dtype=np.float64)
        if not (b.shape == (6,) and a.shape == (6,) and a[0] == 1.0):
            raise NativeError("filtfilt_order5 wants b[6], a[6] with a[0] == 1")
        _ff_coef_cache[key] = np.ascontiguousarray(np.concatenate([b, a, signal.lfilter_zi(b, a)]))
    return _ff_coef_cache[key]


def filtfilt_order5(x: torch.Tensor, b, a) -> torch.Tensor:
    if not x.is_cuda or x.dtype != torch.float64 or x.dim() != 1:
        raise NativeError("filtfilt_order5 wants a 1-D float64 HBM tensor")
    x = x.contiguous()
    coef = _filtfilt_coef(b, a)
    y = torch.empty_like(x)
    ws = _workspace("filtfilt", x.device, "rvc_filtfilt_workspace_bytes", x.numel())
    _call("rvc_filtfilt_order5", x.device, x.data_ptr(), x.numel(), coef.ctypes.data, y.data_ptr(), ws.data_ptr(), ws.numel())
    return y


def _lfilter_coef(b, a):
    import numpy as np
    b = np.asarray(b, dtype=np.float64)
    a = np.asarray(a, dtype=np.float64)
    if b.shape != (6,) or a.shape != (6,):
        raise NativeError("lfilter_order5 wants b[6], a[6]")
    return np.ascontiguousarray(np.concatenate([b, a]))


def lfilter_warmup(b, a) -> int:
    coef, warm = _lfilter_coef(b, a), c_int64()
    _check(_lib.rvc_lfilter_order5_warmup(coef.ctypes.data, ctypes.byref(warm)), "rvc_lfilter_order5_warmup")
    return warm.value


def lfilter_order5(x: torch.Tensor, b, a) -> torch.Tensor:
    if not torch.is_tensor(x) or not x.is_cuda or x.dtype != torch.float64 or x.dim() != 1:
        raise NativeError("lfilter_order5 wants a 1-D float64 HBM tensor")
    x = x.contiguous()
    coef = _lfilter_coef(b, a)
    y = torch.empty_like(x)
    if x.numel() == 0:
        lfilter_warmup(b, a)
        return y
    _call("rvc_lfilter_order5_f64", x.device, x.data_ptr(), x.numel(), coef.ctypes.data, y.data_ptr())
    return y


def frame_rms(x: torch.Tensor, frame_length: int, hop_length: int) -> torch.Tensor:
    if not torch.is_tensor(x) or not x.is_cuda or x.dtype != torch.float64 or x.dim() != 1:
        raise NativeError("frame_rms wants a 1-D float64 HBM tensor")
    x = x.contiguous()
    n_frames, need = c_int64(), c_size_t()
    _check(_lib.rvc_frame_rms_frames(x.numel(), int(frame_length), int(hop_length), ctypes.byref(n_frames), ctypes.byref(need)),
           "rvc_frame_rms_frames")
    out = torch.empty(n_frames.value, dtype=torch.float64, device=x.device)
    ws = _ws.get("frame_rms", need.value, x.device)
    _call("rvc_frame_rms_f64", x.device, x.data_ptr() or ws.data_ptr(), x.numel(), int(frame_length), int(hop_length),
          out.data_ptr() or ws.data_ptr(), n_frames.value, ws.data_ptr(), ws.numel())
    return out


def slice_export(x: torch.Tensor, bounds, up: int, down: int, h: torch.Tensor):
    import numpy as np
    if not (torch.is_tensor(x) and x.is_cuda and x.dtype == torch.float64 and x.dim() == 1
            and torch.is_tensor(h) and h.is_cuda and h.dtype == torch.float64 and h.dim() == 1 and h.device == x.device):
        raise NativeError("slice_export wants 1-D float64 HBM tensors on one device")
    x, h = x.contiguous(), h.contiguous()
    try:
        tab = np.ascontiguousarray(np.asarray(bounds, dtype=np.int64).reshape(-1, 2))
    except (TypeError, ValueError, OverflowError) as e:
        raise NativeError(f"slice_export: bounds must be (start, end) integer pairs ({e})")
    up, down = int(up), int(down)
    if up < 1 or down < 1:
        raise NativeError(f"slice_export: up = {up}, down = {down} must be at least 1")
    n_seg = tab.shape[0]
    length = np.maximum(tab[:, 1] - tab[:, 0], 0)
    off_full = np.concatenate([[0], np.cumsum(length)]).astype(np.int64)
    off_lo = np.concatenate([[0], np.cumsum(-(-(length * up) // down))]).astype(np.int64)
    tables = torch.from_numpy(np.concatenate([tab.reshape(-1), off_full, off_lo])).to(x.device)
    full = torch.empty(int(off_full[-1]), dtype=torch.float32, device=x.device)
    lo = torch.empty(int(off_lo[-1]), dtype=torch.float32, device=x.device)
    seg_ptr = tables.data_ptr()
    _call("rvc_slice_export_f32", x.device, x.data_ptr() or seg_ptr, x.numel(), tab.ctypes.data, seg_ptr, seg_ptr + 16 * n_seg,
          seg_ptr + 16 * n_seg + 8 * (n_seg + 1), n_seg, up, down, h.data_ptr(), h.numel(),
          full.data_ptr() or seg_ptr, full.numel(), lo.data_ptr() or seg_ptr, lo.numel())
    return full, lo, off_full.tolist(), off_lo.tolist()


def spectral_gate_params(sr: int):
    import numpy as np
    nf, nt, b = c_int(), c_int(), ctypes.c_double()
    ft, tt = np.zeros(51, dtype=np.float64), np.zeros(51, dtype=np.float64)
    _check(_lib.rvc_spectral_gate_params(int(sr), ctypes.byref(nf), ctypes.byref(nt), ctypes.byref(b), ft.ctypes.data, tt.ctypes.data),
           "rvc_spectral_gate_params")
    return nf.value, nt.value, b.value, ft[:nf.value + 1].copy(), tt[:nt.value + 1].copy()


def spectral_gate(y: torch.Tensor, sr: int, prop_decrease: float = 1.0, chunk_size: int = 600000, padding: int = 30000) -> torch.Tensor:
    if not torch.is_tensor(y) or y.dim() != 1:
        raise NativeError("spectral_gate wants a 1-D float32 HBM tensor")
    y = _dev_f32(y, "y")
    out = torch.empty_like(y)
    n = y.numel()
    dims = (n, int(sr), int(chunk_size), int(padding))
    ws = _workspace("spectral_gate", y.device, "rvc_spectral_gate_workspace_bytes", *dims)
    _call("rvc_spectral_gate_f32", y.device, y.data_ptr() or ws.data_ptr(), n, int(sr), float(prop_decrease), int(chunk_size), int(padding),
          out.data_ptr() or ws.data_ptr(), ws.data_ptr(), ws.numel())
    return out


def formant_shift(x: torch.Tensor, sr: int, quefrency_s: float, distortion: float, group_frames: int = 0) -> torch.Tensor:
    if not torch.is_tensor(x) or x.dim() != 1:
        raise NativeError("formant_shift wants a 1-D float32 HBM tensor")
    x = _dev_f32(x, "x")
    n = x.numel()
    ws = _workspace("formant_shift", x.device, "rvc_formant_shift_workspace_bytes", n, int(group_frames))
    out = torch.empty_like(x)
    _call("rvc_formant_shift_f32", x.device, x.data_ptr(), n, int(sr), float(quefrency_s), float(distortion), int(group_frames),
          out.data_ptr(), ws.data_ptr(), ws.numel())
    return out


def _signal_pair(x: torch.Tensor, y: torch.Tensor, what: str):
    if x.dim() != 1 or y.dim() != 1 or x.shape != y.shape:
        raise NativeError(f"{what} wants two 1-D signals of equal length, got shapes {tuple(x.shape)} and {tuple(y.shape)}")
    _device(x, y)
    return _dev_f32(x, f"{what}: x"), _dev_f32(y, f"{what}: y")


def mrstft_sums(x: torch.Tensor, y: torch.Tensor, fft_sizes, hop_sizes, win_lengths, eps: float = 1e-8) -> torch.Tensor:
    x, y = _signal_pair(x, y, "mrstft_sums")
    n_res = len(fft_sizes)
    if not (len(hop_sizes) == len(win_lengths) == n_res):
        raise NativeError("mrstft_sums: fft_sizes, hop_sizes and win_lengths must have one entry per resolution")
    arr = [(c_int * max(n_res, 1))(*[int(v) for v in vals]) for vals in (fft_sizes, hop_sizes, win_lengths)]
    ws = _workspace("mrstft_sums", x.device, "rvc_mrstft_sums_workspace_bytes", x.numel(), *arr, n_res)
    out = torch.empty(max(n_res, 1), 4, dtype=torch.float64, device=x.device)
    _call("rvc_mrstft_sums_f32", x.device, x.data_ptr(), y.data_ptr(), x.numel(), *arr, n_res, float(eps), out.data_ptr(),
          ws.data_ptr(), ws.numel())
    return out


def si_sdr_sums(preds: torch.Tensor, target: torch.Tensor) -> torch.Tensor:
    preds, target = _signal_pair(preds, target, "si_sdr_sums")
    ws = _workspace("si_sdr_sums", preds.device, "rvc_si_sdr_sums_workspace_bytes", preds.numel())
    out = torch.empty(5, dtype=torch.float64, device=preds.device)
    _call("rvc_si_sdr_sums_f32", preds.device, preds.data_ptr(), target.data_ptr(), preds.numel(), out.data_ptr(), ws.data_ptr(), ws.numel())
    return out


def mean_abs_diff_sum(a: torch.Tensor, b: torch.Tensor, min_t: int) -> torch.Tensor:
    if a.dim() != 2 or b.dim() != 2 or a.shape[0] != b.shape[0]:
        raise NativeError(f"mean_abs_diff_sum wants two matrices with as many rows, got shapes {tuple(a.shape)} and {tuple(b.shape)}")
    if min_t > min(a.shape[1], b.shape[1]):
        raise NativeError(f"mean_abs_diff_sum: min_t = {min_t} exceeds a width ({a.shape[1]}, {b.shape[1]})")
    _device(a, b)
    a, b = (t if t.is_cuda and t.dtype == torch.float32 and t.stride(1) == 1 and t.stride(0) >= t.shape[1] else
            _dev_f32(t, "mean_abs_diff_sum: matrix") for t in (a, b))
    rows = a.shape[0]
    ws = _workspace("mean_abs_diff", a.device, "rvc_mean_abs_diff_workspace_bytes", rows, int(min_t))
    out = torch.empty(1, dtype=torch.float64, device=a.device)
    _call("rvc_mean_abs_diff_f32", a.device, a.data_ptr(), a.stride(0), b.data_ptr(), b.stride(0), rows, int(min_t), out.data_ptr(),
          ws.data_ptr(), ws.numel())
    return out


def bigru_forward(gi: torch.Tensor, whh_t: torch.Tensor, bhh: torch.Tensor, multi_cu: bool = True) -> torch.Tensor:
    gi, whh_t, bhh = _dev_f32(gi, "gi"), _dev_f32(whh_t, "whh_t"), _dev_f32(bhh, "bhh")
    dev = _device(gi, whh_t, bhh)
    b, t = gi.shape[0], gi.shape[1]
    out = torch.empty((b, t, 512), dtype=torch.float32, device=dev)
    ws = _workspace("bigru", dev, "rvc_bigru_workspace_bytes", b) if multi_cu else None
    _call("rvc_bigru_forward", dev, gi.data_ptr(), whh_t.data_ptr(), bhh.data_ptr(), out.data_ptr(), b, t, 256, _ptr(ws),
          ws.numel() if multi_cu else 0)
    return out


def bigru_redone(batch: int = 1, device=None) -> int:
    device = _cuda_device(device)
    ws = _workspace("bigru", device, "rvc_bigru_workspace_bytes", batch)
    n = c_int()
    _call("rvc_bigru_status", device, ws.data_ptr(), batch, ctypes.byref(n))
    return n.value


def bigru_set_spin_limit(polls: int) -> None:
    _check(_lib.rvc_bigru_set_spin_limit(int(polls)), "rvc_bigru_set_spin_limit")


def _is_f32_hbm(t: torch.Tensor) -> bool:
    return t.is_cuda and t.dtype == torch.float32 and t.is_contiguous()


def attention_qkv(qkv: torch.Tensor, n_heads: int, scale: float, emb_rel_k: torch.Tensor = None,
                  emb_rel_v: torch.Tensor = None) -> torch.Tensor:
    if not (_is_f32_hbm(qkv) and qkv.dim() == 3):
        raise NativeError("attention_qkv wants a contiguous float32 HBM tensor [B, T, 3 * n_heads * d]")
    b, t, c = qkv.shape
    hd = c // (3 * n_heads)
    rel = (emb_rel_k, emb_rel_v) if emb_rel_k is not None else (None, None)
    if rel[0] is not None and not all(e is not None and _is_f32_hbm(e) and tuple(e.shape) == (21, hd) for e in rel):
        raise NativeError(f"attention_qkv wants emb_rel_k and emb_rel_v as contiguous float32 HBM tensors [21, {hd}]")
    dev = _device(qkv, *rel)
    out = torch.empty(b, t, n_heads * hd, dtype=torch.float32, device=dev)
    ws = _workspace("attention", dev, "rvc_attention_workspace_bytes", b, t, n_heads, hd)
    _call("rvc_attention_qkv_f32", dev, qkv.data_ptr(), _ptr(rel[0]), _ptr(rel[1]), out.data_ptr(), b, t, n_heads, hd, float(scale),
          ws.data_ptr(), ws.numel())
    return out


def bias_relu_add_(x: torch.Tensor, bias: torch.Tensor = None, res: torch.Tensor = None, relu: bool = True) -> torch.Tensor:
    if not (_is_f32_hbm(x) and x.dim() >= 3):
        raise NativeError("bias_relu_add_ wants a contiguous float32 HBM tensor [B, C, ...]")
    b, c = x.shape[0], x.shape[1]
    inner = x.numel() // (b * c)
    if res is not None and not (_is_f32_hbm(res) and res.shape == x.shape):
        raise NativeError("bias_relu_add_ wants res as a contiguous float32 HBM tensor of x's shape")
    _call("rvc_bias_relu_add_f32", _device(x, bias, res), x.data_ptr(), _ptr(bias), _ptr(res), x.data_ptr(), b, c, inner, int(relu))
    return x


def rownorm_gelu_(x: torch.Tensor, gamma: torch.Tensor = None, beta: torch.Tensor = None, eps: float = 1e-5) -> torch.Tensor:
    if not (_is_f32_hbm(x) and x.dim() == 3):
        raise NativeError("rownorm_gelu_ wants a contiguous float32 HBM tensor [B, C, L]")
    b, c, length = x.shape
    _call("rvc_rownorm_gelu_f32", _device(x, gamma, beta), x.data_ptr(), _ptr(gamma), _ptr(beta), x.data_ptr(), b, c, length, float(eps))
    return x


def gate_tanh_sigmoid(x: torch.Tensor) -> torch.Tensor:
    if not (_is_f32_hbm(x) and x.dim() == 3 and x.shape[1] % 2 == 0):
        raise NativeError("gate_tanh_sigmoid wants a contiguous float32 HBM tensor [B, 2H, T]")
    b, c2, t = x.shape
    out = torch.empty(b, c2 // 2, t, dtype=torch.float32, device=x.device)
    _call("rvc_gate_tanh_sigmoid_f32", x.device, x.data_ptr(), out.data_ptr(), b, c2 // 2, t)
    return out


def set_concurrency_hint(utterances_in_flight: int) -> None:
    _check(_lib.rvc_set_concurrency_hint(int(utterances_in_flight)), "rvc_set_concurrency_hint")


COMM_ID_BYTES = 128


def comm_unique_id() -> bytes:
    buf = ctypes.create_string_buffer(COMM_ID_BYTES)
    _check(_lib.rvc_comm_unique_id(buf), "rvc_comm_unique_id")
    return buf.raw


class Comm:

    def __init__(self, unique_id: bytes, n_ranks: int, rank: int):
        if len(unique_id) != COMM_ID_BYTES:
            raise NativeError(f"Comm wants the {COMM_ID_BYTES}-byte id of comm_unique_id, got {len(unique_id)} bytes")
        self._h = c_void_p()
        _check(_lib.rvc_comm_create(ctypes.create_string_buffer(unique_id, COMM_ID_BYTES), int(n_ranks), int(rank),
                                    ctypes.byref(self._h)), "rvc_comm_create")

    def info(self) -> dict:
        n, r, v = c_int(), c_int(), c_int()
        path = ctypes.create_string_buffer(512)
        _check(_lib.rvc_comm_info(self._h, ctypes.byref(n), ctypes.byref(r), ctypes.byref(v), path, 512), "rvc_comm_info")
        return {"n_ranks": n.value, "rank": r.value, "rccl_version": v.value, "library": path.value.decode()}

    def broadcast_(self, t: torch.Tensor, root: int = 0) -> torch.Tensor:
        if not t.is_cuda or not t.is_contiguous():
            raise NativeError("Comm.broadcast_ wants a contiguous HBM tensor")
        _call("rvc_index_broadcast", t.device, self._h, t.data_ptr(), t.numel() * t.element_size(), int(root))
        return t

    def destroy(self):
        h, self._h = self._h, None
        if h:
            _check(_lib.rvc_comm_destroy(h), "rvc_comm_destroy")

    def __del__(self):
        if getattr(self, "_h", None) and _lib is not None:
            _lib.rvc_comm_destroy(self._h)
            self._h = None


def checksum64(t: torch.Tensor) -> torch.Tensor:
    if not t.is_cuda or not t.is_contiguous():
        raise NativeError("checksum64 wants a contiguous HBM tensor")
    out = torch.empty(2, dtype=torch.int64, device=t.device)
    _call("rvc_checksum64", t.device, t.data_ptr(), t.numel() * t.element_size(), out.data_ptr())
    return out


def conv1d_pack_weight(w: torch.Tensor, device) -> torch.Tensor:
    w = _host(w)
    packed = torch.empty(w.numel(), dtype=torch.float32, device=device)
    _call("rvc_conv1d_pack_weight", packed.device, w.data_ptr(), w.shape[0], w.shape[1], w.shape[2], packed.data_ptr())
    return packed


def conv1d_wino_pack_weight(w: torch.Tensor, device) -> torch.Tensor:
    w = _host(w)
    c_out, c_in, k = w.shape
    u = torch.empty(3 * ((k + 2) // 3) * c_in * c_out, dtype=torch.float32, device=device)
    _call("rvc_conv1d_wino_pack_weight", u.device, w.data_ptr(), c_out, c_in, k, u.data_ptr())
    return u


def conv1d_winobf_pack_weight(w: torch.Tensor, device) -> torch.Tensor:
    w = _host(w)
    return _pack_slab("rvc_conv1d_winobf", device, (w,), tuple(w.shape))


def _conv1d_square_pack(stem: str, w: torch.Tensor, device) -> torch.Tensor:
    w = _host(w)
    c, c_in, k = w.shape
    if c != c_in:
        raise NativeError(f"{stem[4:]}: a square conv expected, got {tuple(w.shape)}")
    return _pack_slab(stem, device, (w,), (c, k))


def conv1d_bf16w_pack_weight(w: torch.Tensor, device) -> torch.Tensor:
    return _conv1d_square_pack("rvc_conv1d_bf16w", w, device)


def conv1d_f16x2_pack_weight(w: torch.Tensor, device) -> torch.Tensor:
    return _conv1d_square_pack("rvc_conv1d_f16x2", w, device)


def _conv1d(name: str, x, w_packed, bias, c_out, k, dilation, slope_in, res, acc, out_scale, out):
    x = _dev_f32(x, "x")
    b, c_in, length = x.shape
    square = c_out is None
    y = out if out is not None else torch.empty((b, c_in if square else c_out, length), dtype=torch.float32, device=x.device)
    if square and y.data_ptr() == x.data_ptr():
        raise NativeError(f"{name[4:-8]}: x and y must not alias")
    _call(name, _device(x, w_packed, bias, res, acc, y), x.data_ptr(), w_packed.data_ptr(), _ptr(bias), _ptr(res), _ptr(acc), y.data_ptr(),
          b, *((c_in,) if square else (c_in, c_out)), length, k, dilation, float(slope_in), float(out_scale))
    return y


def conv1d_forward(x, w_packed, bias, c_out, k, dilation=1, slope_in=1.0, res=None, acc=None, out_scale=1.0):
    return _conv1d("rvc_conv1d_forward", x, w_packed, bias, c_out, k, dilation, slope_in, res, acc, out_scale, None)


def conv1d_forward_into(x, w_packed, bias, c_out, k, dilation=1, slope_in=1.0, res=None, acc=None, out_scale=1.0, out=None):
    return _conv1d("rvc_conv1d_forward", x, w_packed, bias, c_out, k, dilation, slope_in, res, acc, out_scale, out)


def conv1d_wino_forward(x, u_packed, bias, c_out, k, dilation=1, slope_in=1.0, res=None, acc=None, out_scale=1.0, out=None):
    return _conv1d("rvc_conv1d_wino_forward", x, u_packed, bias, c_out, k, dilation, slope_in, res, acc, out_scale, out)


def conv1d_winobf_forward(x, u_packed, bias, c_out, k, dilation=1, slope_in=1.0, res=None, acc=None, out_scale=1.0, out=None):
    return _conv1d("rvc_conv1d_winobf_forward", x, u_packed, bias, c_out, k, dilation, slope_in, res, acc, out_scale, out)


def conv1d_bf16w_forward(x, u_packed, bias, k, dilation=1, slope_in=1.0, res=None, acc=None, out_scale=1.0, out=None):
    return _conv1d("rvc_conv1d_bf16w_forward", x, u_packed, bias, None, k, dilation, slope_in, res, acc, out_scale, out)


def conv1d_f16x2_forward(x, u_packed, bias, k, dilation=1, slope_in=1.0, res=None, acc=None, out_scale=1.0, out=None):
    return _conv1d("rvc_conv1d_f16x2_forward", x, u_packed, bias, None, k, dilation, slope_in, res, acc, out_scale, out)


def resblock_bf16x3_pack_weight(w1: torch.Tensor, w2: torch.Tensor, device, bf16_taps: bool = False) -> torch.Tensor:
    w1, w2 = _host(w1), _host(w2)
    c, c_in, k = w1.shape
    if c != c_in or w2.shape != w1.shape:
        raise NativeError(f"resblock pair: square convs of one shape expected, got {tuple(w1.shape)} and {tuple(w2.shape)}")
    return _pack_slab("rvc_resblock_bf16w" if bf16_taps else "rvc_resblock_bf16x3", device, (w1, w2), (c, k))


def resblock_bf16x3_forward(x, u_packed, b1, b2, k, dilation=1, slope=0.1, acc=None, out_scale=1.0, out=None, bf16_taps: bool = False):
    x = _dev_f32(x, "x")
    b, c, length = x.shape
    y = out if out is not None else torch.empty_like(x)
    if y.data_ptr() == x.data_ptr():
        raise NativeError("resblock pair: x and y must not alias")
    _call("rvc_resblock_bf16w_forward" if bf16_taps else "rvc_resblock_bf16x3_forward", _device(x, u_packed, b1, b2, acc, y),
          x.data_ptr(), u_packed.data_ptr(), _ptr(b1), _ptr(b2), _ptr(acc), y.data_ptr(), b, c, length, k, dilation, float(slope),
          float(out_scale))
    return y


def upsample_bf16x3_pack_weight(up_w: torch.Tensor, noise_w, bias, rate: int, nc_stride: int, device):
    up_w = _host(up_w)
    c_in, c_out, ksize = up_w.shape
    nw = _host(noise_w).reshape(c_out, -1).contiguous() if noise_w is not None else None
    nc_k = nw.shape[1] if nw is not None else 0
    b = _host(bias) if bias is not None else None
    u = _pack_slab("rvc_upsample_bf16x3", device, (up_w, nw, b), (c_in, c_out, rate, ksize, nc_k, nc_stride))
    return u, (nw.to(device) if nw is not None else None), (b.to(device) if b is not None else None)


def upsample_bf16x3_forward(x, har, packed, c_out, rate, ksize, pad, nc_stride=1, nc_pad=0, slope=0.1):
    u, nw, bias = packed
    x = _dev_f32(x, "x")
    b, c_in, length = x.shape
    l_out = (length - 1) * rate - 2 * pad + ksize
    y = torch.empty((b, c_out, l_out), dtype=torch.float32, device=x.device)
    if har is not None:
        har = _dev_f32(har, "har")
    _call("rvc_upsample_bf16x3_forward", _device(x, har, u, bias), x.data_ptr(), _ptr(har), har.shape[-1] if har is not None else 0,
          u.data_ptr(), _ptr(bias), y.data_ptr(), b, c_in, c_out, length, rate, ksize, pad, nw.shape[1] if nw is not None else 0,
          nc_stride, nc_pad, float(slope))
    return y


def resblock_bf16x3_set_enabled(enabled: bool) -> None:
    _check(_lib.rvc_resblock_bf16x3_set_enabled(1 if enabled else 0), "rvc_resblock_bf16x3_set_enabled")


def gemm_bf16x3_pack_weight(w: torch.Tensor, device) -> torch.Tensor:
    w = _host(w)
    taps = w.shape[2] if w.dim() == 3 else 1
    m, k_total = w.shape[0], w.shape[1] * taps
    return _pack_slab("rvc_gemm_bf16x3", device, (w,), (m, k_total), (m, k_total, taps))


def linear_bf16x3(x: torch.Tensor, a_packed: torch.Tensor, bias, out_features: int, act: str = "none", res=None) -> torch.Tensor:
    x = _dev_f32(x, "x")
    in_features = x.shape[-1]
    n_rows = x.numel() // in_features
    y = torch.empty(x.shape[:-1] + (out_features,), dtype=torch.float32, device=x.device)
    if res is not None:
        res = _dev_f32(res, "res")
        if res.shape != y.shape:
            raise NativeError(f"linear_bf16x3: res {tuple(res.shape)} must have the result's shape {tuple(y.shape)}")
    _call("rvc_linear_bf16x3", _device(x, a_packed, bias, res), x.data_ptr(), a_packed.data_ptr(), _ptr(bias), _ptr(res), y.data_ptr(),
          n_rows, in_features, out_features, {"none": 0, "gelu": 1}[act])
    return y


def glu_dwconv_silu(x: torch.Tensor, w: torch.Tensor, bias: torch.Tensor) -> torch.Tensor:
    x, w, bias = _dev_f32(x, "x"), _dev_f32(w, "w"), _dev_f32(bias, "bias")
    n_rows, c = x.shape[0], x.shape[1] // 2
    y = torch.empty((n_rows, c), dtype=torch.float32, device=x.device)
    _call("rvc_glu_dwconv_silu_f32", _device(x, w, bias), x.data_ptr(), w.data_ptr(), bias.data_ptr(), y.data_ptr(), n_rows, c, w.shape[1])
    return y


def layernorm_rows(x: torch.Tensor, gamma: torch.Tensor, beta: torch.Tensor, eps: float = 1e-5) -> torch.Tensor:
    x, gamma, beta = _dev_f32(x, "x"), _dev_f32(gamma, "gamma"), _dev_f32(beta, "beta")
    f = x.shape[-1]
    y = torch.empty_like(x)
    _call("rvc_layernorm_rows_f32", _device(x, gamma, beta), x.data_ptr(), gamma.data_ptr(), beta.data_ptr(), float(eps), y.data_ptr(),
          x.numel() // f, f)
    return y


def groupnorm_lrelu(x: torch.Tensor, gamma: torch.Tensor, beta: torch.Tensor, groups: int, eps: float = 1e-5,
                    slope: float = 0.01) -> torch.Tensor:
    x = _dev_f32(x, "x")
    c, length = x.shape
    ws = _workspace("groupnorm", x.device, "rvc_groupnorm_workspace_bytes", c, length, groups)
    y = torch.empty_like(x)
    gamma, beta = _dev_f32(gamma, "gamma"), _dev_f32(beta, "beta")
    _call("rvc_groupnorm_lrelu_f32", _device(x, gamma, beta), x.data_ptr(), gamma.data_ptr(), beta.data_ptr(), groups, float(eps),
          float(slope), y.data_ptr(), c, length, ws.data_ptr(), ws.numel())
    return y


def fcpe_decode(logits: torch.Tensor, cent_table: torch.Tensor, out_dims: int, threshold: float, f0_min: float,
                want_latent: bool = False):
    logits, cent_table = _dev_f32(logits, "logits"), _dev_f32(cent_table, "cent_table")
    n_rows, ld = logits.shape
    if cent_table.numel() != out_dims:
        raise NativeError(f"cent_table has {cent_table.numel()} entries, out_dims is {out_dims}")
    dev = _device(logits, cent_table)
    f0 = torch.empty(n_rows, dtype=torch.float32, device=dev)
    latent = torch.empty((n_rows, out_dims), dtype=torch.float32, device=dev) if want_latent else None
    _call("rvc_fcpe_decode_f32", dev, logits.data_ptr(), cent_table.data_ptr(), out_dims, ld, float(threshold), float(f0_min),
          f0.data_ptr(), _ptr(latent), n_rows)
    return f0, latent


def rows_padded(n_rows: int, tile: int = 128) -> int:
    return -(-n_rows // tile) * tile


def planes_empty(n_rows: int, features: int, device) -> torch.Tensor:
    return torch.empty((3, rows_padded(n_rows), features), dtype=torch.bfloat16, device=device)


def split_rows_bf16x3(x: torch.Tensor, out: torch.Tensor | None = None) -> torch.Tensor:
    x = _dev_f32(x, "x")
    n_rows, k = x.shape
    xs = out if out is not None else planes_empty(n_rows, k, x.device)
    _call("rvc_split_rows_bf16x3", _device(x, xs), x.data_ptr(), xs.data_ptr(), n_rows, xs.shape[1], k)
    return xs


def linear_bf16x3_presplit(xs: torch.Tensor, a_packed: torch.Tensor, bias, n_rows: int, out_features: int, mode: str = "f32",
                           k_parts: int = 1, out: torch.Tensor | None = None) -> torch.Tensor:
    _, n_pad, in_features = xs.shape
    m = {"f32": 0, "gelu_planes": 1, "parts": 2, "gelu_f32": 3}[mode]
    if m in (0, 3):
        y = out if out is not None else torch.empty((n_rows, out_features), dtype=torch.float32, device=xs.device)
    elif m == 1:
        y = out if out is not None else torch.empty((3, n_pad, out_features), dtype=torch.bfloat16, device=xs.device)
    else:
        y = out if out is not None else torch.empty((k_parts, n_rows, out_features), dtype=torch.float32, device=xs.device)
    _call("rvc_linear_bf16x3_presplit", _device(xs, a_packed, bias, y), xs.data_ptr(), a_packed.data_ptr(), _ptr(bias),
          y.data_ptr() if m != 1 else None, y.data_ptr() if m == 1 else None, n_rows, n_pad, in_features, out_features, m, k_parts)
    return y


def posconv_bf16x3_pack_weight(w: torch.Tensor, groups: int, device) -> torch.Tensor:
    w = _host(w)
    return _pack_slab("rvc_posconv_bf16x3", device, (w,), (w.shape[0], groups, w.shape[2]))


def posconv_gelu_bf16x3(x: torch.Tensor, a_packed: torch.Tensor, bias, groups: int, taps: int, padding: int) -> torch.Tensor:
    x = _dev_f32(x, "x")
    t, d = x.shape
    y = torch.empty_like(x)
    _call("rvc_posconv_gelu_bf16x3", _device(x, a_packed, bias), x.data_ptr(), a_packed.data_ptr(), _ptr(bias), y.data_ptr(), t, d, groups,
          taps, padding)
    return y


def hubert_conv0_frames_bf16x3(wav: torch.Tensor, w: torch.Tensor, gamma, beta, eps: float, stride: int = 5) -> tuple[torch.Tensor, int]:
    wav = _dev_f32(wav, "wav")
    w2 = _dev_f32(w.reshape(w.shape[0], -1), "w")
    dev = _device(wav, w2, gamma, beta)
    c, taps = w2.shape
    n = wav.numel()
    frames = (n - taps) // stride + 1
    ys = planes_empty(frames, c, dev)
    ws = _workspace("hubert_conv0", dev, "rvc_hubert_conv0_workspace_bytes", c)
    _call("rvc_hubert_conv0_frames_bf16x3", dev, wav.data_ptr(), n, w2.data_ptr(), c, taps, stride, _ptr(gamma), _ptr(beta), float(eps),
          ws.data_ptr(), ws.numel(), ys.data_ptr(), ys.shape[1])
    return ys, frames


def conv1d_frames_bf16x3(xs: torch.Tensor, n_frames_in: int, a_packed: torch.Tensor, bias, out_channels: int, taps: int, stride: int,
                         mode: str = "gelu_planes") -> tuple[torch.Tensor, int]:
    _, n_pad_in, c = xs.shape
    m = {"f32": 0, "gelu_planes": 1, "gelu_f32": 3}[mode]
    frames = (n_frames_in - taps) // stride + 1
    if frames <= 0:
        raise NativeError("conv1d_frames_bf16x3: the input is shorter than one window")
    y = planes_empty(frames, out_channels, xs.device) if m == 1 else torch.empty((frames, out_channels), dtype=torch.float32, device=xs.device)
    _call("rvc_conv1d_frames_bf16x3", _device(xs, a_packed, bias), xs.data_ptr(), n_frames_in, n_pad_in, c, taps, stride, a_packed.data_ptr(),
          _ptr(bias), y.data_ptr() if m != 1 else None, y.data_ptr() if m == 1 else None, rows_padded(frames), out_channels, m)
    return y, frames


def bias_residual_layernorm_bf16x3(parts: torch.Tensor, bias, res, gamma, beta, eps: float, want_planes: bool = True,
                                   y: torch.Tensor | None = None, ys: torch.Tensor | None = None):
    n_parts, n_rows, m = parts.shape
    y = y if y is not None else torch.empty((n_rows, m), dtype=torch.float32, device=parts.device)
    if want_planes and ys is None:
        ys = planes_empty(n_rows, m, parts.device)
    _call("rvc_bias_residual_layernorm_bf16x3", _device(parts, bias, res, gamma, beta, y, ys), parts.data_ptr(), n_parts, _ptr(bias),
          _ptr(res), _ptr(gamma), _ptr(beta), float(eps), y.data_ptr(), _ptr(ys), n_rows, ys.shape[1] if ys is not None else n_rows, m)
    return y, ys


def conv1d_bf16x3(x: torch.Tensor, a_packed: torch.Tensor, bias, c_out: int, k: int, stride: int = 1, padding: int = 0,
                  act: str = "none") -> torch.Tensor:
    x = _dev_f32(x, "x")
    b, c_in, l_in = x.shape
    l_out = max((l_in + 2 * padding - k) // stride + 1, 0)
    y = torch.empty((b, c_out, l_out), dtype=torch.float32, device=x.device)
    if y.numel() == 0:
        return y
    _call("rvc_conv1d_bf16x3", _device(x, a_packed, bias), x.data_ptr(), a_packed.data_ptr(), _ptr(bias), y.data_ptr(), b, c_in, c_out, l_in,
          k, stride, padding, {"none": 0, "gelu": 1}[act])
    return y


def conv2d_pack_weight(w: torch.Tensor, device) -> torch.Tensor:
    w = _host(w)
    device = _cuda_device(device)
    out = torch.empty(_size("rvc_conv2d_packed_floats", device, *w.shape), dtype=torch.float32, device=device)
    _call("rvc_conv2d_pack_weight", device, w.data_ptr(), *w.shape, out.data_ptr())
    return out


def conv2d_supported(c_in: int, width: int) -> bool:
    return c_in % 8 == 0 and 4 <= width <= 128 and width & (width - 1) == 0


def conv2d_bf16x3_supported(c_in: int, c_out: int, height: int, width: int) -> bool:
    return bool(_lib.rvc_conv2d_bf16x3_supported(c_in, c_out, height, width))


def conv2d_bf16x3_packable(c_in: int, c_out: int) -> bool:
    m_pad = (c_out + 31) // 32 * 32
    return c_in % 16 == 0 and (m_pad in (32, 64) or m_pad % 128 == 0)


def conv2d_bf16x3_pack_weight(w: torch.Tensor, device) -> torch.Tensor:
    w = _host(w)
    return _pack_slab("rvc_conv2d_bf16x3", device, (w,), tuple(w.shape))


def _conv2d(stem: str, x, w_packed, bias, c_out, taps: tuple, relu, res, out):
    x = _dev_f32(x, "x")
    b, c_in, h, wd = x.shape
    y = out if out is not None else torch.empty((b, c_out, h, wd), dtype=torch.float32, device=x.device)
    dev = _device(x, w_packed, bias, res, y)
    need = _size(stem + "_workspace_bytes", dev, b, c_in, c_out, h, wd, *taps)
    ws = _ws.get("conv2d", need, dev) if need else None
    _call(stem + "_forward", dev, x.data_ptr(), w_packed.data_ptr(), _ptr(bias), _ptr(res), y.data_ptr(), b, c_in, c_out, h, wd, *taps,
          1 if relu else 0, _ptr(ws), need)
    return y


def conv2d_forward(x, w_packed, bias, c_out, ksize=3, relu=False, res=None, out=None):
    return _conv2d("rvc_conv2d", x, w_packed, bias, c_out, (ksize, ksize), relu, res, out)


def conv2d_bf16x3_forward(x, u, bias, c_out, relu=False, res=None, out=None):
    return _conv2d("rvc_conv2d_bf16x3", x, u, bias, c_out, (), relu, res, out)


DEC_KINDS = {"HiFi-GAN": 0, "MRF HiFi-GAN": 1, "RefineGAN": 2}
DEC_ARITHMETIC = {"exact": 0, "fp16x2": 1}


def _decoder_config(vocoder, sr, *, in_channels=192, upsample_initial_channel=512, gin_channels=256,
                    upsample_rates=(12, 10, 2, 2), upsample_kernel_sizes=(24, 20, 4, 4), res_kernel_sizes=(3, 7, 11),
                    res_dilations=(1, 3, 5), weight_storage: str = "f32") -> DecoderConfig:
    cfg = DecoderConfig()
    cfg.kind = DEC_KINDS[vocoder]
    cfg.sample_rate = sr
    cfg.in_channels = in_channels
    cfg.upsample_initial_channel = upsample_initial_channel
    cfg.gin_channels = gin_channels
    cfg.n_ups = len(upsample_rates)
    for i, (u, k) in enumerate(zip(upsample_rates, upsample_kernel_sizes)):
        cfg.upsample_rates[i] = int(u)
        cfg.upsample_kernel_sizes[i] = int(k)
    cfg.n_res_kernels = len(res_kernel_sizes)
    for i, k in enumerate(res_kernel_sizes):
        cfg.res_kernel_sizes[i] = int(k)
    cfg.weight_storage = {"f32": 0, "bf16": 1}[weight_storage]
    cfg.n_res_dilations = len(res_dilations)
    for i, d in enumerate(res_dilations):
        cfg.res_dilations[i] = int(d)
    return cfg


def _window_margin(cfg: DecoderConfig) -> int:
    frames = c_int()
    _check(_lib.rvc_decoder_window_margin(ctypes.byref(cfg), ctypes.byref(frames)), "rvc_decoder_window_margin")
    return frames.value


def decoder_window_margin(vocoder: str, sr: int = 48000, **config) -> int:
    return _window_margin(_decoder_config(vocoder, sr, **config))


class Decoder:

    def __init__(self, vocoder: str, sr: int, folded_weights: dict, *, in_channels=192, upsample_initial_channel=512,
                 gin_channels=256, upsample_rates=(12, 10, 2, 2), upsample_kernel_sizes=(24, 20, 4, 4),
                 res_kernel_sizes=(3, 7, 11), res_dilations=(1, 3, 5), weight_storage: str = "f32",
                 arithmetic: str = "exact", device=None):
        if not torch.cuda.is_available():
            raise NativeError("rvc_amd.Decoder needs a HIP device (no CPU fallback)")
        if arithmetic not in DEC_ARITHMETIC:
            raise NativeError(f"rvc_amd.Decoder: arithmetic must be one of {sorted(DEC_ARITHMETIC)}, got {arithmetic!r}")
        cfg = self._cfg = _decoder_config(vocoder, sr, in_channels=in_channels, upsample_initial_channel=upsample_initial_channel,
                                          gin_channels=gin_channels, upsample_rates=upsample_rates,
                                          upsample_kernel_sizes=upsample_kernel_sizes, res_kernel_sizes=res_kernel_sizes,
                                          res_dilations=res_dilations, weight_storage=weight_storage)
        self.device = _cuda_device(device)
        self._h = c_void_p()
        self.vocoder = vocoder
        _check(_lib.rvc_decoder_create(ctypes.byref(cfg), ctypes.byref(self._h)), "rvc_decoder_create")
        self.arithmetic = arithmetic
        if arithmetic != "exact":
            _check(_lib.rvc_decoder_set_arithmetic(self._h, DEC_ARITHMETIC[arithmetic]), "rvc_decoder_set_arithmetic")
        for name, t in folded_weights.items():
            t = _host(t)
            shape = (c_int64 * t.dim())(*t.shape)
            _check(_lib.rvc_decoder_set_tensor(self._h, name.encode(), t.data_ptr(), shape, t.dim()),
                   f"rvc_decoder_set_tensor({name})")
        with torch.cuda.device(self.device):
            _check(_lib.rvc_decoder_finalize(self._h), "rvc_decoder_finalize")
        self.upp = _lib.rvc_decoder_upp(self._h)

    def __del__(self):
        h = getattr(self, "_h", None)
        if h and _lib is not None:
            _lib.rvc_decoder_destroy(h)
            self._h = None

    def set_concurrency_hint(self, utterances_in_flight: int):
        _check(_lib.rvc_decoder_set_concurrency_hint(self._h, int(utterances_in_flight)), "rvc_decoder_set_concurrency_hint")

    def set_branch_parallel(self, side_streams: int):
        _check(_lib.rvc_decoder_set_branch_parallel(self._h, int(side_streams)), "rvc_decoder_set_branch_parallel")

    def set_tap(self, stage: int, tap: torch.Tensor | None):
        _check(_lib.rvc_decoder_set_tap(self._h, stage, _ptr(tap)), "rvc_decoder_set_tap")

    def window_margin(self) -> int:
        return _window_margin(self._cfg)

    def forward(self, z: torch.Tensor, f0: torch.Tensor, g: torch.Tensor, *, src_randn: torch.Tensor,
                src_rand: torch.Tensor | None = None, adain_randn: torch.Tensor | None = None,
                keep: tuple | None = None) -> torch.Tensor:
        z, f0, g, src_randn = _dev_f32(z, "z"), _dev_f32(f0, "f0"), _dev_f32(g, "g"), _dev_f32(src_randn, "src_randn")
        src_rand = _dev_f32(src_rand, "src_rand") if src_rand is not None else None
        adain_randn = _dev_f32(adain_randn, "adain_randn") if adain_randn is not None else None
        dev = self.device
        if _device(z, f0, g, src_randn, src_rand, adain_randn) != dev:
            raise NativeError(f"Decoder of {dev} got tensors on {z.device}")
        b, _, t = z.shape
        noise = DecoderNoise(_ptr(src_rand), src_randn.data_ptr(), _ptr(adain_randn))
        ws = _workspace("decoder", dev, "rvc_decoder_workspace_bytes", self._h, b, t)
        if keep is not None:
            lo, hi = int(keep[0]), int(keep[1])
            out = torch.empty((b, 1, max(hi - lo, 0) * self.upp), dtype=torch.float32, device=dev)
            _call("rvc_decoder_forward_window", dev, self._h, z.data_ptr(), f0.data_ptr(), g.data_ptr(), ctypes.byref(noise), b, t,
                  lo, hi, out.data_ptr(), ws.data_ptr(), ws.numel())
            return out
        out = torch.empty((b, 1, t * self.upp), dtype=torch.float32, device=dev)
        _call("rvc_decoder_forward", dev, self._h, z.data_ptr(), f0.data_ptr(), g.data_ptr(), ctypes.byref(noise), b, t,
              out.data_ptr(), ws.data_ptr(), ws.numel())
        return out
```

### codename-rvc-fork-3_amd/rvc_amd/lib/hubert.py

```python
from __future__ import annotations

from typing import Dict

import torch
import torch.nn.functional as F

from rvc_amd.lib.algorithm.weights import fold_weight_norm

CONV_STRIDES = (5, 2, 2, 2, 2, 2, 2)


class HubertModelWithFinalProj:
    def __init__(self, state_dict: Dict[str, torch.Tensor] | None = None, device="cpu", n_layers=12, n_heads=12):
        self.n_layers, self.n_heads = n_layers, n_heads
        self.device = torch.device(device)
        self.w: Dict[str, torch.Tensor] = {}
        self.consume_layerdrop_rng = False
        self.native_min_rows = 900
        self.frame_convs = True
        self.native_posconv = True
        self.frame_convs_min_samples = 400
        if state_dict is not None:
            self.load_state_dict(state_dict)

    def load_state_dict(self, sd, strict: bool = True):
        w = fold_weight_norm(sd)
        self.w = {k: v.to(self.device) for k, v in w.items() if v.is_floating_point()}
        self._conv_bf = {}
        if self.device.type == "cuda":
            from rvc_amd import _native
            for i in (0, 1, 2, 3):
                cw = self.w[f"feature_extractor.conv_layers.{i}.conv.weight"]
                if cw.shape[0] % 128 == 0 and (cw.shape[1] % 16 == 0 or (cw.shape[1] == 1 and cw.shape[2] <= 16)):
                    self._conv_bf[i] = _native.gemm_bf16x3_pack_weight(cw, self.device)
        self._pack_frame_convs()
        self._pack_posconv()
        self._lin = {}
        self._qkv = {}
        for i in range(self.n_layers):
            L = f"encoder.layers.{i}.attention"
            hd = self.w[L + ".q_proj.weight"].shape[0] // self.n_heads
            scale = hd ** -0.5
            self._qkv[i] = (torch.cat([self.w[L + ".q_proj.weight"], self.w[L + ".k_proj.weight"],
                                       self.w[L + ".v_proj.weight"]], 0).contiguous(),
                            torch.cat([self.w[L + ".q_proj.bias"], self.w[L + ".k_proj.bias"],
                                       self.w[L + ".v_proj.bias"]], 0).contiguous(), scale)
        self._pack_linears()
        return self

    def _pack_frame_convs(self):
        self._conv_fr = {}
        if self.device.type != "cuda":
            return
        from rvc_amd import _native
        n = len(CONV_STRIDES)
        ws = [self.w[f"feature_extractor.conv_layers.{i}.conv.weight"] for i in range(n)]
        c = ws[0].shape[0]
        ok = ws[0].shape[1] == 1 and ws[0].shape[2] == 10 and c % 128 == 0 and \
            all(w.shape[0] == c and w.shape[1] == c and (w.shape[2] * c) % 32 == 0 for w in ws[1:]) and \
            not any(f"feature_extractor.conv_layers.{i}.conv.bias" in self.w for i in range(n))
        if not ok:
            return
        for i in range(1, n):
            self._conv_fr[i] = _native.gemm_bf16x3_pack_weight(ws[i].permute(0, 2, 1).reshape(c, -1).contiguous(), self.device)

    def _pack_posconv(self):
        self._posconv = None
        if self.device.type != "cuda":
            return
        from rvc_amd import _native
        pw = self.w["encoder.pos_conv_embed.conv.weight"]
        d, cg, taps = pw.shape
        if d % cg == 0 and cg in (48, 64) and taps <= 128:
            self._posconv = (_native.posconv_bf16x3_pack_weight(pw, d // cg, self.device), d // cg, taps)

    def _frame_convs_max_samples(self) -> int:
        c = self.w["feature_extractor.conv_layers.0.conv.weight"].shape[0]
        frames = ((1 << 31) - (1 << 20)) // (6 * c) // 128 * 128 - 128
        return frames * CONV_STRIDES[0]

    def _features_native(self, wav):
        from rvc_amd import _native as N
        w = self.w
        xs, n = N.hubert_conv0_frames_bf16x3(wav[0], w["feature_extractor.conv_layers.0.conv.weight"],
                                             w["feature_extractor.conv_layers.0.layer_norm.weight"],
                                             w["feature_extractor.conv_layers.0.layer_norm.bias"], 1e-5, stride=CONV_STRIDES[0])
        last = len(CONV_STRIDES) - 1
        for i in range(1, last + 1):
            cw = w[f"feature_extractor.conv_layers.{i}.conv.weight"]
            xs, n = N.conv1d_frames_bf16x3(xs, n, self._conv_fr[i], None, cw.shape[0], cw.shape[2], CONV_STRIDES[i],
                                           "gelu_planes" if i < last else "gelu_f32")
        return xs[None]

    def _pack_linears(self):
        self._lin = {}
        if self.device.type != "cuda":
            return
        from rvc_amd import _native
        for i in range(self.n_layers):
            L = f"encoder.layers.{i}"
            ws = [self._qkv[i][0], self.w[L + ".attention.out_proj.weight"], self.w[L + ".feed_forward.intermediate_dense.weight"],
                  self.w[L + ".feed_forward.output_dense.weight"]]
            d = ws[1].shape[0]
            if any(w.shape[0] % 128 or w.shape[1] % 96 for w in ws) or d not in (256, 768, 1024):
                self._lin = {}
                return
            self._lin[i] = [_native.gemm_bf16x3_pack_weight(w, self.device) for w in ws]

    def to(self, device):
        self.device = torch.device(device)
        self.w = {k: v.to(self.device) for k, v in self.w.items()}
        self._qkv = {i: (a.to(self.device), b.to(self.device), s) for i, (a, b, s) in self._qkv.items()}
        self._conv_bf = {i: a.to(self.device) for i, a in self._conv_bf.items()} if self.device.type == "cuda" else {}
        self._pack_frame_convs()
        self._pack_posconv()
        self._pack_linears()
        return self

    def float(self):
        return self

    def eval(self):
        return self

    def final_proj(self, x):
        return F.linear(x, self.w["final_proj.weight"], self.w["final_proj.bias"])

    @torch.no_grad()
    def __call__(self, wav: torch.Tensor):
        w = self.w
        if wav.is_cuda and wav.shape[0] == 1 and self._conv_fr and self.frame_convs and \
                self.frame_convs_min_samples <= wav.shape[1] <= self._frame_convs_max_samples():
            return self._encode(self._features_native(wav))
        x = wav[:, None, :]
        for i, s in enumerate(CONV_STRIDES):
            cw = w[f"feature_extractor.conv_layers.{i}.conv.weight"]
            if i in self._conv_bf and x.is_cuda and (i > 0 or x.shape[0] == 1):
                from rvc_amd import _native
                x = _native.conv1d_bf16x3(x, self._conv_bf[i], None, cw.shape[0], cw.shape[2], stride=s, act="gelu" if i > 0 else "none")
                if i > 0:
                    continue
            else:
                x = F.conv1d(x, cw, None, stride=s)
            if i == 0 and x.is_cuda and x.is_contiguous():
                from rvc_amd import _native
                x = _native.rownorm_gelu_(x, w["feature_extractor.conv_layers.0.layer_norm.weight"],
                                          w["feature_extractor.conv_layers.0.layer_norm.bias"], 1e-5)
                continue
            if i == 0:
                x = F.group_norm(x, x.shape[1], w["feature_extractor.conv_layers.0.layer_norm.weight"],
                                 w["feature_extractor.conv_layers.0.layer_norm.bias"], 1e-5)
            x = F.gelu(x)
        return self._encode(x.transpose(1, 2))

    def _encode(self, x):
        w = self.w
        x = F.layer_norm(x, (x.shape[-1],), w["feature_projection.layer_norm.weight"],
                         w["feature_projection.layer_norm.bias"], 1e-5)
        x = F.linear(x, w["feature_projection.projection.weight"], w["feature_projection.projection.bias"])
        d = x.shape[-1]
        b, t, _ = x.shape
        if x.is_cuda and b == 1 and self._posconv is not None and self.native_posconv:
            from rvc_amd import _native as N
            a_pc, groups, taps = self._posconv
            x2 = x.reshape(t, d).contiguous()
            pos = N.posconv_gelu_bf16x3(x2, a_pc, w["encoder.pos_conv_embed.conv.bias"], groups, taps, taps // 2)
            if d in (256, 768, 1024):
                x, _ = N.bias_residual_layernorm_bf16x3(pos[None], None, x2, w["encoder.layer_norm.weight"], w["encoder.layer_norm.bias"],
                                                        1e-5, want_planes=False)
                x = x[None]
            else:
                x = F.layer_norm(x + pos[None], (d,), w["encoder.layer_norm.weight"], w["encoder.layer_norm.bias"], 1e-5)
        else:
            pw = w["encoder.pos_conv_embed.conv.weight"]
            taps = pw.shape[2]
            pos = F.conv1d(x.transpose(1, 2), pw, w["encoder.pos_conv_embed.conv.bias"], padding=taps // 2, groups=d // pw.shape[1])
            if taps % 2 == 0:
                pos = pos[:, :, :-1]
            x = x + F.gelu(pos).transpose(1, 2)
            x = F.layer_norm(x, (d,), w["encoder.layer_norm.weight"], w["encoder.layer_norm.bias"], 1e-5)
        h = self.n_heads
        hd = d // h
        if x.is_cuda and self._lin and b * t >= self.native_min_rows:
            return {"last_hidden_state": self._encoder_native(x, b, t, d, h)}
        for i in range(self.n_layers):
            L = f"encoder.layers.{i}"
            if self.consume_layerdrop_rng:
                torch.rand([])
            wqkv, bqkv, scale = self._qkv[i]
            qkv = F.linear(x, wqkv, bqkv)
            if qkv.is_cuda:
                from rvc_amd import _native
                a = _native.attention_qkv(qkv, h, scale)
            else:
                qkv = qkv.view(b, t, 3, h, hd).permute(2, 0, 3, 1, 4)
                a = F.scaled_dot_product_attention(qkv[0], qkv[1], qkv[2], scale=scale).transpose(1, 2).reshape(b, t, d)
            a = F.linear(a, w[L + ".attention.out_proj.weight"], w[L + ".attention.out_proj.bias"])
            x = F.layer_norm(x + a, (d,), w[L + ".layer_norm.weight"], w[L + ".layer_norm.bias"], 1e-5)
            f = F.gelu(F.linear(x, w[L + ".feed_forward.intermediate_dense.weight"],
                                w[L + ".feed_forward.intermediate_dense.bias"]))
            f = F.linear(f, w[L + ".feed_forward.output_dense.weight"], w[L + ".feed_forward.output_dense.bias"])
            x = F.layer_norm(x + f, (d,), w[L + ".final_layer_norm.weight"], w[L + ".final_layer_norm.bias"], 1e-5)
        return {"last_hidden_state": x}

    def _encoder_native(self, x, b, t, d, h):
        from rvc_amd import _native as N
        w = self.w
        n = b * t
        x = x.reshape(n, d).contiguous()
        xs = N.split_rows_bf16x3(x)
        a_s = N.planes_empty(n, d, x.device)
        d_ff = w["encoder.layers.0.feed_forward.intermediate_dense.weight"].shape[0]
        fs = N.planes_empty(n, d_ff, x.device)
        parts = torch.empty((3, n, d), dtype=torch.float32, device=x.device)
        qkv = torch.empty((n, 3 * d), dtype=torch.float32, device=x.device)
        x1, x1s = torch.empty_like(x), N.planes_empty(n, d, x.device)
        for i in range(self.n_layers):
            L = f"encoder.layers.{i}"
            if self.consume_layerdrop_rng:
                torch.rand([])
            a_qkv, a_o, a_1, a_2 = self._lin[i]
            _, bqkv, scale = self._qkv[i]
            N.linear_bf16x3_presplit(xs, a_qkv, bqkv, n, 3 * d, "f32", out=qkv)
            a = N.attention_qkv(qkv.view(b, t, 3 * d), h, scale)
            N.split_rows_bf16x3(a.view(n, d), out=a_s)
            N.linear_bf16x3_presplit(a_s, a_o, None, n, d, "parts", 3, out=parts)
            N.bias_residual_layernorm_bf16x3(parts, w[L + ".attention.out_proj.bias"], x, w[L + ".layer_norm.weight"],
                                             w[L + ".layer_norm.bias"], 1e-5, y=x1, ys=x1s)
            N.linear_bf16x3_presplit(x1s, a_1, w[L + ".feed_forward.intermediate_dense.bias"], n, d_ff, "gelu_planes", out=fs)
            N.linear_bf16x3_presplit(fs, a_2, None, n, d, "parts", 3, out=parts)
            N.bias_residual_layernorm_bf16x3(parts, w[L + ".feed_forward.output_dense.bias"], x1, w[L + ".final_layer_norm.weight"],
                                             w[L + ".final_layer_norm.bias"], 1e-5, y=x, ys=xs)
        return x.view(b, t, d)
```

### include/rvc_amd.h

```cpp
#ifndef RVC_AMD_H
#define RVC_AMD_H

#include <stddef.h>
#include <stdint.h>

#ifdef __cplusplus
extern "C" {
#endif

#define RVC_AMD_ABI_VERSION 4


int rvc_abi_version(void);
const char *rvc_last_error(void);


int rvc_knn_index_aux_bytes(int64_t n_rows, int dim, size_t *bytes);
int rvc_knn_index_build(const float *index_dev, int64_t n_rows, int dim, void *aux_dev, size_t aux_bytes, void *stream);

int rvc_knn_workspace_bytes(int64_t n_rows, int64_t n_queries, int dim, int k, size_t *bytes);

int rvc_knn_search(const float *index_dev, const void *aux_dev, int64_t n_rows, int dim,
                   const float *queries_dev, int64_t n_queries, int k,
                   float *out_d2_dev, int64_t *out_ids_dev,
                   void *workspace_dev, size_t workspace_bytes, void *stream);

int rvc_knn_rank_candidates(const float *index_dev, const void *aux_dev, int64_t n_rows, int dim, const float *queries_dev,
                            int64_t n_queries, const int32_t *cand_ids_dev, int cap, int k, float *out_d2_dev,
                            int64_t *out_ids_dev, void *stream);

int rvc_knn_set_mode(int mode);

int rvc_knn_blend(const float *index_dev, int dim, const float *feats_dev, const float *d2_dev,
                  const int64_t *ids_dev, int64_t n_queries, int k, float index_rate,
                  float *out_dev, void *stream);

int rvc_logmel_workspace_bytes(int batch, int64_t n_samples, size_t *bytes);
int rvc_logmel_rmvpe(const float *audio_dev, int batch, int64_t n_samples, float *mel_dev,
                     int64_t n_frames_padded, void *workspace_dev, size_t workspace_bytes, void *stream);

typedef struct rvc_mel rvc_mel;
int rvc_mel_create(int n_fft, int hop, int win_length, int pad, float mag_eps, float log_floor, const float *mel_host, int n_mels,
                   rvc_mel **out);
int rvc_mel_destroy(rvc_mel *h);
int rvc_mel_frames(const rvc_mel *h, int64_t n_samples, int64_t *n_frames);
int rvc_mel_workspace_bytes(const rvc_mel *h, int batch, int64_t n_samples, size_t *bytes);
int rvc_mel_forward(const rvc_mel *h, const float *audio_dev, int batch, int64_t n_samples, float *mel_dev, float *spec_dev,
                    void *workspace_dev, size_t workspace_bytes, void *stream);

int rvc_resample_poly_f64(const double *x_dev, int64_t n_in, int up, int down, const double *h_dev, int64_t n_taps,
                          double *y_dev, int64_t n_out, void *stream);

int rvc_filtfilt_workspace_bytes(int64_t n, size_t *bytes);
int rvc_filtfilt_order5(const double *x_dev, int64_t n, const double *coef_host, double *y_dev,
                        void *workspace_dev, size_t workspace_bytes, void *stream);

int rvc_bigru_workspace_bytes(int batch, size_t *bytes);
int rvc_bigru_status(const void *workspace_dev, int batch, int *n_redone_host, void *stream);
int rvc_bigru_set_spin_limit(unsigned polls);
int rvc_bigru_forward(const float *gi_dev, const float *whhT_dev, const float *bhh_dev, float *out_dev,
                      int batch, int64_t n_steps, int hidden, void *workspace_dev, size_t workspace_bytes, void *stream);

int rvc_attention_workspace_bytes(int batch, int64_t n_frames, int n_heads, int head_dim, size_t *bytes);
int rvc_attention_qkv_f32(const float *qkv_dev, const float *emb_rel_k_dev, const float *emb_rel_v_dev, float *out_dev,
                          int batch, int64_t n_frames, int n_heads, int head_dim, float scale, void *workspace_dev,
                          size_t workspace_bytes, void *stream);

int rvc_bias_relu_add_f32(const float *x_dev, const float *bias_dev, const float *res_dev, float *out_dev, int batch,
                          int channels, int64_t inner, int relu, void *stream);

int rvc_rownorm_gelu_f32(const float *x_dev, const float *gamma_dev, const float *beta_dev, float *out_dev, int batch, int channels,
                         int64_t length, float eps, void *stream);

int rvc_gate_tanh_sigmoid_f32(const float *x_dev, float *out_dev, int batch, int hidden, int64_t length, void *stream);

int rvc_set_concurrency_hint(int utterances_in_flight);

typedef struct rvc_decoder rvc_decoder;

enum { RVC_DEC_NSF = 0, RVC_DEC_MRF = 1, RVC_DEC_REFINE = 2 };

typedef struct rvc_decoder_config {
    int kind;
    int sample_rate;
    int in_channels;
    int upsample_initial_channel;
    int gin_channels;
    int n_ups;
    int upsample_rates[8];
    int upsample_kernel_sizes[8];
    int n_res_kernels;
    int res_kernel_sizes[4];
    int res_dilations[4];
    int n_res_dilations;
    int weight_storage;
} rvc_decoder_config;

int rvc_decoder_create(const rvc_decoder_config *cfg, rvc_decoder **out);
int rvc_decoder_set_tensor(rvc_decoder *dec, const char *name, const float *data_host,
                           const int64_t *shape, int ndim);
int rvc_decoder_finalize(rvc_decoder *dec);
int rvc_decoder_destroy(rvc_decoder *dec);

int rvc_decoder_upp(const rvc_decoder *dec);
int rvc_decoder_workspace_bytes(const rvc_decoder *dec, int batch, int64_t n_frames, size_t *bytes);

typedef struct rvc_decoder_noise {
    const float *src_rand_dev;
    const float *src_randn_dev;
    const float *adain_randn_dev;
} rvc_decoder_noise;

int rvc_decoder_forward(rvc_decoder *dec, const float *z_dev, const float *f0_dev, const float *g_dev,
                        const rvc_decoder_noise *noise, int batch, int64_t n_frames, float *out_dev,
                        void *workspace_dev, size_t workspace_bytes, void *stream);

int rvc_decoder_window_margin(const rvc_decoder_config *cfg, int *frames);
int rvc_decoder_forward_window(rvc_decoder *dec, const float *z_dev, const float *f0_dev, const float *g_dev,
                               const rvc_decoder_noise *noise, int batch, int64_t n_frames, int64_t keep_lo, int64_t keep_hi,
                               float *out_dev, void *workspace_dev, size_t workspace_bytes, void *stream);

int rvc_decoder_set_concurrency_hint(rvc_decoder *dec, int utterances_in_flight);

int rvc_decoder_set_branch_parallel(rvc_decoder *dec, int side_streams);

int rvc_decoder_set_arithmetic(rvc_decoder *dec, int mode);

int rvc_decoder_set_tap(rvc_decoder *dec, int stage, float *tap_dev);

int rvc_conv1d_pack_weight(const float *w_host, int c_out, int c_in, int k, float *w_packed_dev, void *stream);
int rvc_conv1d_forward(const float *x_dev, const float *w_packed_dev, const float *bias_dev,
                       const float *res_dev, const float *acc_dev, float *y_dev,
                       int batch, int c_in, int c_out, int64_t length, int k, int dilation,
                       float slope_in, float out_scale, void *stream);

typedef struct rvc_comm rvc_comm;
#define RVC_COMM_ID_BYTES 128
int rvc_comm_unique_id(unsigned char *id_host );
int rvc_comm_create(const unsigned char *id_host, int n_ranks, int rank, rvc_comm **out);
int rvc_comm_destroy(rvc_comm *comm);
int rvc_comm_info(const rvc_comm *comm, int *n_ranks, int *rank, int *rccl_version, char *library_path,
                  size_t library_path_bytes);
int rvc_index_broadcast(rvc_comm *comm, void *buf_dev, size_t bytes, int root, void *stream);
int rvc_checksum64(const void *buf_dev, size_t bytes, uint64_t *out2_dev, void *stream);

int rvc_conv2d_packed_floats(int c_out, int c_in, int kh, int kw, size_t *out);
int rvc_conv2d_pack_weight(const float *w_host, int c_out, int c_in, int kh, int kw, float *w_dev, void *stream);
int rvc_conv2d_workspace_bytes(int batch, int c_in, int c_out, int height, int width, int kh, int kw, size_t *out);
int rvc_conv2d_forward(const float *x_dev, const float *w_packed_dev, const float *bias_dev, const float *res_dev,
                       float *y_dev, int batch, int c_in, int c_out, int height, int width, int kh, int kw, int relu,
                       void *workspace_dev, size_t workspace_bytes, void *stream);

int rvc_conv2d_bf16x3_supported(int c_in, int c_out, int height, int width);
int rvc_conv2d_bf16x3_weight_bytes(int c_out, int c_in, int kh, int kw, size_t *bytes);
int rvc_conv2d_bf16x3_pack_weight(const float *w_host, int c_out, int c_in, int kh, int kw, void *u_dev, void *stream);
int rvc_conv2d_bf16x3_workspace_bytes(int batch, int c_in, int c_out, int height, int width, size_t *out);
int rvc_conv2d_bf16x3_forward(const float *x_dev, const void *u_dev, const float *bias_dev, const float *res_dev, float *y_dev,
                              int batch, int c_in, int c_out, int height, int width, int relu, void *workspace_dev,
                              size_t workspace_bytes, void *stream);

int rvc_conv1d_wino_pack_weight(const float *w_host, int c_out, int c_in, int k, float *u_dev, void *stream);
int rvc_conv1d_wino_forward(const float *x_dev, const float *u_dev, const float *bias_dev, const float *res_dev,
                            const float *acc_dev, float *y_dev, int batch, int c_in, int c_out, int64_t length, int k,
                            int dilation, float slope_in, float out_scale, void *stream);

int rvc_conv1d_winobf_weight_bytes(int c_out, int c_in, int k, size_t *bytes);
int rvc_conv1d_winobf_pack_weight(const float *w_host, int c_out, int c_in, int k, void *u_dev, void *stream);
int rvc_conv1d_winobf_forward(const float *x_dev, const void *u_dev, const float *bias_dev, const float *res_dev,
                              const float *acc_dev, float *y_dev, int batch, int c_in, int c_out, int64_t length, int k,
                              int dilation, float slope_in, float out_scale, void *stream);

int rvc_resblock_bf16x3_weight_bytes(int c, int k, size_t *bytes);
int rvc_resblock_bf16x3_pack_weight(const float *w1_host, const float *w2_host, int c, int k, void *u_dev, void *stream);
int rvc_resblock_bf16x3_forward(const float *x_dev, const void *u_dev, const float *b1_dev, const float *b2_dev,
                                const float *acc_dev, float *y_dev, int batch, int c, int64_t length, int k, int dilation,
                                float slope, float out_scale, void *stream);
int rvc_resblock_bf16w_weight_bytes(int c, int k, size_t *bytes);
int rvc_resblock_bf16w_pack_weight(const float *w1_host, const float *w2_host, int c, int k, void *u_dev, void *stream);
int rvc_resblock_bf16w_forward(const float *x_dev, const void *u_dev, const float *b1_dev, const float *b2_dev,
                               const float *acc_dev, float *y_dev, int batch, int c, int64_t length, int k, int dilation,
                               float slope, float out_scale, void *stream);
int rvc_conv1d_bf16w_weight_bytes(int c, int k, size_t *bytes);
int rvc_conv1d_bf16w_pack_weight(const float *w_host, int c, int k, void *u_dev, void *stream);
int rvc_conv1d_bf16w_forward(const float *x_dev, const void *u_dev, const float *bias_dev, const float *res_dev,
                             const float *acc_dev, float *y_dev, int batch, int c, int64_t length, int k, int dilation,
                             float slope_in, float out_scale, void *stream);
int rvc_conv1d_f16x2_weight_bytes(int c, int k, size_t *bytes);
int rvc_conv1d_f16x2_pack_weight(const float *w_host, int c, int k, void *u_dev, void *stream);
int rvc_conv1d_f16x2_forward(const float *x_dev, const void *u_dev, const float *bias_dev, const float *res_dev,
                             const float *acc_dev, float *y_dev, int batch, int c, int64_t length, int k, int dilation,
                             float slope_in, float out_scale, void *stream);
int rvc_upsample_bf16x3_weight_bytes(int c_in, int c_out, int rate, int ksize, int nc_k, int nc_stride, size_t *bytes);
int rvc_upsample_bf16x3_pack_weight(const float *up_w_host, const float *noise_w_host, const float *bias_host, int c_in, int c_out,
                                    int rate, int ksize, int nc_k, int nc_stride, void *u_dev, void *stream);
int rvc_upsample_bf16x3_forward(const float *x_dev, const float *har_dev, int64_t har_len, const void *u_dev, const float *bias_dev,
                                float *y_dev, int batch, int c_in, int c_out, int64_t length_in, int rate, int ksize, int pad,
                                int nc_k, int nc_stride, int nc_pad, float slope_in, void *stream);
int rvc_resblock_bf16x3_set_enabled(int enabled);

int rvc_gemm_bf16x3_weight_bytes(int m, int k_total, size_t *bytes);
int rvc_gemm_bf16x3_pack_weight(const float *w_host, int m, int k_total, int conv_taps, void *a_dev, void *stream);
int rvc_linear_bf16x3(const float *x_dev, const void *a_dev, const float *bias_dev, const float *res_dev, float *y_dev,
                      int64_t n_rows, int in_features, int out_features, int act, void *stream);
int rvc_conv1d_bf16x3(const float *x_dev, const void *a_dev, const float *bias_dev, float *y_dev, int batch, int c_in,
                      int c_out, int64_t l_in, int k, int stride, int padding, int act, void *stream);

int rvc_split_rows_bf16x3(const float *x_dev, void *xs_dev, int64_t n_rows, int64_t n_rows_padded, int k, void *stream);
int rvc_linear_bf16x3_presplit(const void *xs_dev, const void *a_dev, const float *bias_dev, float *y_dev, void *ys_dev,
                               int64_t n_rows, int64_t n_rows_padded, int in_features, int out_features, int mode, int k_parts,
                               void *stream);
int rvc_bias_residual_layernorm_bf16x3(const float *parts_dev, int n_parts, const float *bias_dev, const float *res_dev,
                                       const float *gamma_dev, const float *beta_dev, float eps, float *y_dev, void *ys_dev,
                                       int64_t n_rows, int64_t n_rows_padded, int features, void *stream);

int rvc_hubert_conv0_workspace_bytes(int channels, size_t *bytes);
int rvc_hubert_conv0_frames_bf16x3(const float *wav_dev, int64_t n_samples, const float *w_dev, int channels, int taps, int stride,
                                   const float *gamma_dev, const float *beta_dev, float eps, void *workspace_dev,
                                   size_t workspace_bytes, void *ys_dev, int64_t n_frames_padded, void *stream);
int rvc_conv1d_frames_bf16x3(const void *xs_dev, int64_t n_frames_in, int64_t n_frames_in_padded, int channels, int taps, int stride,
                             const void *a_dev, const float *bias_dev, float *y_dev, void *ys_dev, int64_t n_frames_out_padded,
                             int out_channels, int mode, void *stream);

int rvc_posconv_bf16x3_weight_bytes(int d, int groups, int taps, size_t *bytes);
int rvc_posconv_bf16x3_pack_weight(const float *w_host, int d, int groups, int taps, void *a_dev, void *stream);
int rvc_posconv_gelu_bf16x3(const float *x_dev, const void *a_dev, const float *bias_dev, float *y_dev, int64_t n_frames, int d,
                            int groups, int taps, int padding, void *stream);

int rvc_glu_dwconv_silu_f32(const float *x_dev, const float *w_dev, const float *bias_dev, float *y_dev, int64_t n_rows, int C, int K,
                            void *stream);
int rvc_layernorm_rows_f32(const float *x_dev, const float *gamma_dev, const float *beta_dev, float eps, float *y_dev, int64_t n_rows,
                           int F, void *stream);
int rvc_groupnorm_workspace_bytes(int C, int64_t L, int groups, size_t *bytes);
int rvc_groupnorm_lrelu_f32(const float *x_dev, const float *gamma_dev, const float *beta_dev, int groups, float eps, float slope,
                            float *y_dev, int C, int64_t L, void *workspace_dev, size_t workspace_bytes, void *stream);
int rvc_fcpe_decode_f32(const float *logits_dev, const float *cent_table_dev, int out_dims, int ld, float threshold, float f0_min,
                        float *f0_dev, float *latent_dev, int64_t n_rows, void *stream);

int rvc_kmeans_workspace_bytes(int64_t n_rows, int64_t n_centroids, int dim, size_t *bytes);
int rvc_kmeans_assign(const float *x_dev, int64_t n_rows, int dim, const float *centroids_dev, int64_t n_centroids,
                      int32_t *out_ids_dev, float *out_d2_dev, void *workspace_dev, size_t workspace_bytes, void *stream);
int rvc_kmeans_update(const float *x_dev, int64_t n_rows, int dim, const int32_t *order_dev, const int64_t *offsets_dev,
                      int64_t n_centroids, const float *old_centroids_dev, float *out_centroids_dev, void *workspace_dev,
                      size_t workspace_bytes, void *stream);

int rvc_lfilter_order5_warmup(const double *coef_host, int64_t *warm);
int rvc_lfilter_order5_f64(const double *x_dev, int64_t n, const double *coef_host, double *y_dev, void *stream);
int rvc_frame_rms_frames(int64_t n, int64_t frame_length, int64_t hop, int64_t *n_frames, size_t *workspace_bytes);
int rvc_frame_rms_f64(const double *x_dev, int64_t n, int64_t frame_length, int64_t hop, double *out_dev, int64_t n_frames,
                      void *workspace_dev, size_t workspace_bytes, void *stream);
int rvc_slice_export_f32(const double *x_dev, int64_t n, const int64_t *bounds_host, const int64_t *seg_dev,
                         const int64_t *off_full_dev, const int64_t *off_lo_dev, int64_t n_seg, int up, int down,
                         const double *h_dev, int64_t n_taps, float *full_dev, int64_t n_full, float *lo_dev, int64_t n_lo,
                         void *stream);

int rvc_spectral_gate_params(int sr, int *nf, int *nt, double *b, double *freq_taps, double *time_taps);
int rvc_spectral_gate_workspace_bytes(int64_t n, int sr, int64_t chunk_size, int64_t padding, size_t *bytes);
int rvc_spectral_gate_f32(const float *y_dev, int64_t n, int sr, float prop_decrease, int64_t chunk_size, int64_t padding,
                          float *out_dev, void *workspace_dev, size_t workspace_bytes, void *hip_stream);

int rvc_formant_shift_workspace_bytes(int64_t n, int group_frames, size_t *bytes);
int rvc_formant_shift_f32(const float *x_dev, int64_t n, int sr, double quefrency_s, double distortion, int group_frames,
                          float *out_dev, void *workspace_dev, size_t workspace_bytes, void *hip_stream);

int rvc_mrstft_sums_workspace_bytes(int64_t n, const int *n_fft, const int *hop, const int *win, int n_res, size_t *bytes);
int rvc_mrstft_sums_f32(const float *x_dev, const float *y_dev, int64_t n, const int *n_fft, const int *hop, const int *win, int n_res,
                        double eps, double *out_dev, void *workspace_dev, size_t workspace_bytes, void *hip_stream);
int rvc_si_sdr_sums_workspace_bytes(int64_t n, size_t *bytes);
int rvc_si_sdr_sums_f32(const float *preds_dev, const float *target_dev, int64_t n, double *out_dev, void *workspace_dev,
                        size_t workspace_bytes, void *hip_stream);
int rvc_mean_abs_diff_workspace_bytes(int64_t rows, int64_t min_t, size_t *bytes);
int rvc_mean_abs_diff_f32(const float *a_dev, int64_t a_stride, const float *b_dev, int64_t b_stride, int64_t rows, int64_t min_t,
                          double *out_dev, void *workspace_dev, size_t workspace_bytes, void *hip_stream);

#ifdef __cplusplus
}
#endif
#endif
```

Baseline: 61.40 million.

## Fuse QKV projection with K/V fragment packing and attention output plane split

Adds a GEMM epilogue mode that writes Q as fp32 and K/V directly into the bf16x3 fragment layout the attention kernel consumes, so the separate pack_kv pass and the full fp32 QKV buffer round trip are no longer needed. The attention kernel (and the split combine kernel) can now emit its output directly as three bf16 planes, which removes the separate split_rows pass before the output projection. HuBERT layers use this fused path by default when batch is 1 and the shape fits. The cost is extra epilogue complexity in the linear kernel and extra shuffles in the attention store.

```diff
diff --git a/codename-rvc-fork-3_amd/csrc/attention.hip b/codename-rvc-fork-3_amd/csrc/attention.hip
--- a/codename-rvc-fork-3_amd/csrc/attention.hip
+++ b/codename-rvc-fork-3_amd/csrc/attention.hip
@@ -230,7 +230,7 @@
 
 __global__ void __launch_bounds__(256)
 attention_combine_kernel(const float *__restrict__ part_o, const float *__restrict__ part_ml, float *__restrict__ out,
-                         int64_t T, int n_heads, int n_splits, int D) {
+                         unsigned char *__restrict__ planes, int64_t n_pad, int64_t T, int n_heads, int n_splits, int D) {
     const int64_t idx = (int64_t)blockIdx.x * 256 + threadIdx.x;
     const int d4n = D / 4;
     const int64_t total = (int64_t)gridDim.y * n_heads * T * d4n;
@@ -250,31 +250,35 @@
         lsum += wgt * part_ml[row * 2 + 1];
         acc += *reinterpret_cast<const f32x4 *>(part_o + row * D + 4 * d4) * wgt;
     }
-    *reinterpret_cast<f32x4 *>(out + (b * T + t) * (int64_t)n_heads * D + (int64_t)head * D + 4 * d4) = acc * (1.f / lsum);
+    f32x4 res = acc * (1.f / lsum);
+    const int64_t at = (b * T + t) * (int64_t)n_heads * D + (int64_t)head * D + 4 * d4;
+    if (!planes) {
+        *reinterpret_cast<f32x4 *>(out + at) = res;
+        return;
+    }
+    f32x2 v0 = {rounded(res.x), rounded(res.y)}, v1 = {rounded(res.z), rounded(res.w)};
+#pragma unroll
+    for (int sp = 0; sp < 3; ++sp) {
+        const unsigned w0 = split_word(v0), w1 = split_word(v1);
+        *reinterpret_cast<u32x2 *>(planes + ((int64_t)sp * n_pad * n_heads * D + at) * 2) = u32x2{w0, w1};
+        v0 = split_rest(v0, w0);
+        v1 = split_rest(v1, w1);
+    }
 }
 
 struct AttBfParams {
-    const float *qkv;
+    const float *q;
+    int64_t q_stride;
     const void *frag;
     float *out, *part_o, *part_ml;
+    unsigned char *planes;
+    int64_t n_pad;
     int64_t T;
     int n_heads, n_splits, tiles_per_split;
     float scale_log2e;
 };
-constexpr int ABF_TILE_BYTES = 24 * 1024, ABF_NW = 8;
+constexpr int ABF_NW = 8;
 typedef void __attribute__((address_space(3))) *abf_lptr_t;
-
-__device__ __forceinline__ void abf_split8(const float (&v)[8], u32x4 (&out)[3]) {
-    f32x2 r[4] = {f32x2{v[0], v[1]}, f32x2{v[2], v[3]}, f32x2{v[4], v[5]}, f32x2{v[6], v[7]}};
-#pragma unroll
-    for (int level = 0; level < 3; ++level)
-#pragma unroll
-        for (int q = 0; q < 4; ++q) {
-            const unsigned w = split_word(r[q]);
-            out[level][q] = w;
-            if (level < 2) r[q] = r[q] - f32x2{__uint_as_float(w << 16), __uint_as_float(w & 0xffff0000u)};
-        }
-}
 
 __global__ void __launch_bounds__(512) attention_pack_kv_kernel(const float *__restrict__ qkv, unsigned char *__restrict__ frag, int64_t T, int n_heads) {
     const int lane = threadIdx.x & 63, wave = threadIdx.x >> 6, i = lane & 31, h = lane >> 5;
@@ -321,7 +325,7 @@
     const int head = blockIdx.y % n_heads;
     const int64_t b = blockIdx.y / n_heads;
     const int split = blockIdx.z;
-    const int64_t rs = (int64_t)3 * n_heads * 64;
+    const int64_t rs = p.q_stride;
     const int nt_all = (int)((T + 31) / 32);
     const int t_begin = split * p.tiles_per_split;
     const int t_end = (DBG & 16) ? min(nt_all, t_begin + 1) : min(nt_all, t_begin + p.tiles_per_split);
@@ -350,7 +354,7 @@
     u32x4 qf[4][3];
     {
         const int64_t q = q0 + j < T ? q0 + j : T - 1;
-        const float *ptr = p.qkv + b * T * rs + (int64_t)head * 64 + q * rs + 8 * h;
+        const float *ptr = p.q + b * T * rs + (int64_t)head * 64 + q * rs + 8 * h;
 #pragma unroll
         for (int ks = 0; ks < 4; ++ks) {
             const f32x4 lo = *reinterpret_cast<const f32x4 *>(ptr + 16 * ks) * p.scale_log2e, hi = *reinterpret_cast<const f32x4 *>(ptr + 16 * ks + 4) * p.scale_log2e;
@@ -447,7 +451,40 @@
         }
     }
     l += __shfl_xor(l, 32);
-    if (active && q0 + j < T) {
+    if (active && p.n_splits == 1 && p.planes) {
+        const float inv = 1.f / l;
+        const int64_t n = b * T + q0 + j;
+        const bool live = q0 + j < T;
+#pragma unroll
+        for (int db = 0; db < 2; ++db)
+#pragma unroll
+            for (int rp = 0; rp < 2; ++rp) {
+                f32x2 v[2][2];
+#pragma unroll
+                for (int g = 0; g < 2; ++g) {
+                    const int r0 = 4 * (2 * rp + g);
+                    const f32x4 q4 = f32x4{o[db][r0], o[db][r0 + 1], o[db][r0 + 2], o[db][r0 + 3]} * inv;
+                    v[g][0] = f32x2{rounded(q4.x), rounded(q4.y)};
+                    v[g][1] = f32x2{rounded(q4.z), rounded(q4.w)};
+                }
+#pragma unroll
+                for (int sp = 0; sp < 3; ++sp) {
+                    unsigned w[2][2];
+#pragma unroll
+                    for (int g = 0; g < 2; ++g)
+#pragma unroll
+                        for (int e = 0; e < 2; ++e) {
+                            w[g][e] = split_word(v[g][e]);
+                            v[g][e] = split_rest(v[g][e], w[g][e]);
+                        }
+                    const unsigned s0 = h ? w[0][0] : w[1][0], s1 = h ? w[0][1] : w[1][1];
+                    const unsigned x0 = (unsigned)__shfl_xor((int)s0, 32, 64), x1 = (unsigned)__shfl_xor((int)s1, 32, 64);
+                    const u32x4 out = h ? u32x4{x0, x1, w[1][0], w[1][1]} : u32x4{w[0][0], w[0][1], x0, x1};
+                    const int64_t m = (int64_t)head * 64 + 32 * db + 16 * rp + 8 * h;
+                    if (live) *reinterpret_cast<u32x4 *>(p.planes + (((int64_t)sp * p.n_pad + n) * n_heads * 64 + m) * 2) = out;
+                }
+            }
+    } else if (active && q0 + j < T) {
         if (p.n_splits == 1) {
             const float inv = 1.f / l;
             float *op = p.out + (b * T + q0 + j) * (int64_t)n_heads * 64 + (int64_t)head * 64 + 4 * h;
@@ -544,7 +581,49 @@
     if (p.n_splits > 1) {
         const int64_t work = (int64_t)p.n_heads * p.T * (D / 4);
         hipLaunchKernelGGL(attention_combine_kernel, dim3((unsigned)ceil_div(work, 256), (unsigned)batch), dim3(256), 0, stream,
-                           p.part_o, p.part_ml, p.out, p.T, p.n_heads, p.n_splits, D);
+                           p.part_o, p.part_ml, p.out, nullptr, 0, p.T, p.n_heads, p.n_splits, D);
+        RVC_LAUNCH_CHECK();
+    }
+    return 0;
+}
+
+static int launch_attention_bf(const char *who, AttBfParams &q, int batch, const float *pack_from, hipStream_t st) {
+    const int n_heads = q.n_heads;
+    const unsigned n_tiles = (unsigned)ceil_div(q.T, 32);
+    q.tiles_per_split = (int)ceil_div(ceil_div(q.T, 32), q.n_splits);
+    const dim3 bgrid((unsigned)ceil_div(q.T, 32 * ABF_NW), (unsigned)(n_heads * batch), (unsigned)q.n_splits);
+    const auto run = [&](auto kernel) -> int {
+        if (reserve_whole_cu((const void *)kernel, who)) return 1;
+        if (pack_from) {
+            hipLaunchKernelGGL(attention_pack_kv_kernel, dim3(n_tiles, (unsigned)(n_heads * batch)), dim3(512), 0, st, pack_from, (unsigned char *)q.frag, q.T, n_heads);
+            RVC_LAUNCH_CHECK();
+        }
+        hipLaunchKernelGGL(kernel, bgrid, dim3(512), LDS_WHOLE_CU, st, q);
+        RVC_LAUNCH_CHECK();
+        return 0;
+    };
+    int dbg = 0;
+#ifdef RVC_ABLATE
+    static const int dbg_knob = knob("RVC_ATT_DBG", 0);
+    dbg = dbg_knob;
+#endif
+    int rc;
+    switch (dbg) {
+#ifdef RVC_ABLATE
+        case 1: rc = run(attention_bf_kernel<1>); break;
+        case 2: rc = run(attention_bf_kernel<2>); break;
+        case 4: rc = run(attention_bf_kernel<4>); break;
+        case 8: rc = run(attention_bf_kernel<8>); break;
+        case 16: rc = run(attention_bf_kernel<16>); break;
+        case 7: rc = run(attention_bf_kernel<7>); break;
+#endif
+        default: rc = run(attention_bf_kernel<0>); break;
+    }
+    if (rc) return 1;
+    if (q.n_splits > 1) {
+        const int64_t work = (int64_t)n_heads * q.T * (64 / 4);
+        hipLaunchKernelGGL(attention_combine_kernel, dim3((unsigned)ceil_div(work, 256), (unsigned)batch), dim3(256), 0, st,
+                           q.part_o, q.part_ml, q.out, q.planes, q.n_pad, q.T, n_heads, q.n_splits, 64);
         RVC_LAUNCH_CHECK();
     }
     return 0;
@@ -565,46 +644,11 @@
         const size_t need = att_bf_workspace(batch, n_frames, n_heads, &off_ml, &off_frag);
         if (!workspace_dev || workspace_bytes < need) return fail("rvc_attention_qkv_f32: workspace too small (%zu < %zu)", workspace_bytes, need);
         AttBfParams q;
-        q.qkv = qkv_dev; q.out = out_dev; q.T = n_frames; q.n_heads = n_heads; q.scale_log2e = scale * 1.4426950408889634f;
+        q.q = qkv_dev; q.q_stride = (int64_t)3 * n_heads * 64; q.out = out_dev; q.planes = nullptr; q.n_pad = 0;
+        q.T = n_frames; q.n_heads = n_heads; q.scale_log2e = scale * 1.4426950408889634f;
         q.n_splits = choose_splits_bf(n_frames, n_heads, batch);
-        q.tiles_per_split = (int)ceil_div(ceil_div(n_frames, 32), q.n_splits);
         q.part_o = (float *)workspace_dev; q.part_ml = (float *)((char *)workspace_dev + off_ml); q.frag = (char *)workspace_dev + off_frag;
-        hipStream_t st = (hipStream_t)stream;
-        const unsigned n_tiles = (unsigned)ceil_div(n_frames, 32);
-        const dim3 bgrid((unsigned)ceil_div(n_frames, 32 * ABF_NW), (unsigned)(n_heads * batch), (unsigned)q.n_splits);
-        const auto run = [&](auto kernel) -> int {
-            if (reserve_whole_cu((const void *)kernel, "rvc_attention_qkv_f32")) return 1;
-            hipLaunchKernelGGL(attention_pack_kv_kernel, dim3(n_tiles, (unsigned)(n_heads * batch)), dim3(512), 0, st, qkv_dev, (unsigned char *)q.frag, q.T, n_heads);
-            RVC_LAUNCH_CHECK();
-            hipLaunchKernelGGL(kernel, bgrid, dim3(512), LDS_WHOLE_CU, st, q);
-            RVC_LAUNCH_CHECK();
-            return 0;
-        };
-        int dbg = 0;
-#ifdef RVC_ABLATE
-        static const int dbg_knob = knob("RVC_ATT_DBG", 0);
-        dbg = dbg_knob;
-#endif
-        int rc;
-        switch (dbg) {
-#ifdef RVC_ABLATE
-            case 1: rc = run(attention_bf_kernel<1>); break;
-            case 2: rc = run(attention_bf_kernel<2>); break;
-            case 4: rc = run(attention_bf_kernel<4>); break;
-            case 8: rc = run(attention_bf_kernel<8>); break;
-            case 16: rc = run(attention_bf_kernel<16>); break;
-            case 7: rc = run(attention_bf_kernel<7>); break;
-#endif
-            default: rc = run(attention_bf_kernel<0>); break;
-        }
-        if (rc) return 1;
-        if (q.n_splits > 1) {
-            const int64_t work = (int64_t)n_heads * q.T * (64 / 4);
-            hipLaunchKernelGGL(attention_combine_kernel, dim3((unsigned)ceil_div(work, 256), (unsigned)batch), dim3(256), 0, st,
-                               q.part_o, q.part_ml, q.out, q.T, n_heads, q.n_splits, 64);
-            RVC_LAUNCH_CHECK();
-        }
-        return 0;
+        return launch_attention_bf("rvc_attention_qkv_f32", q, batch, qkv_dev, (hipStream_t)stream);
     }
     AttParams p;
     p.qkv = qkv_dev; p.emb_k = emb_rel_k_dev; p.emb_v = emb_rel_v_dev; p.out = out_dev;
@@ -625,3 +669,62 @@
     if (head_dim == 64) return rel ? launch_attention<64, true>(p, batch, st) : launch_attention<64, false>(p, batch, st);
     return rel ? launch_attention<96, true>(p, batch, st) : launch_attention<96, false>(p, batch, st);
 }
+
+static bool att_frag_shape_ok(int batch, int64_t n_frames, int n_heads, int head_dim) {
+    return batch > 0 && n_heads > 0 && n_frames >= 0 && head_dim == 64 && fits_2gib((int64_t)batch * n_heads * ceil_div(n_frames, 32), ABF_TILE_BYTES);
+}
+static bool att_frag_splits_ok(int64_t n_frames, int n_splits) {
+    return n_splits == 0 || (n_splits >= 1 && n_splits <= 8 && n_splits <= ceil_div(n_frames, 32));
+}
+
+extern "C" int rvc_attention_kv_frag_bytes(int batch, int64_t n_frames, int n_heads, int head_dim, size_t *bytes) {
+    if (!bytes) return fail("rvc_attention_kv_frag_bytes: null pointer");
+    if (!att_frag_shape_ok(batch, n_frames, n_heads, head_dim))
+        return fail("rvc_attention_kv_frag_bytes: batch > 0, n_heads > 0, n_frames >= 0, head_dim 64, a slab below 2 GiB");
+    *bytes = (size_t)batch * n_heads * (size_t)ceil_div(n_frames, 32) * ABF_TILE_BYTES;
+    return 0;
+}
+
+extern "C" int rvc_attention_pack_kv(const float *qkv_dev, void *frag_dev, int batch, int64_t n_frames, int n_heads, int head_dim, void *stream) {
+    if (!qkv_dev || !frag_dev) return fail("rvc_attention_pack_kv: null pointer");
+    if (!att_frag_shape_ok(batch, n_frames, n_heads, head_dim))
+        return fail("rvc_attention_pack_kv: batch > 0, n_heads > 0, n_frames >= 0, head_dim 64, a slab below 2 GiB");
+    if (n_frames == 0) return 0;
+    hipLaunchKernelGGL(attention_pack_kv_kernel, dim3((unsigned)ceil_div(n_frames, 32), (unsigned)(n_heads * batch)), dim3(512), 0, (hipStream_t)stream,
+                       qkv_dev, (unsigned char *)frag_dev, n_frames, n_heads);
+    RVC_LAUNCH_CHECK();
+    return 0;
+}
+
+extern "C" int rvc_attention_frag_workspace_bytes(int batch, int64_t n_frames, int n_heads, int head_dim, int n_splits, size_t *bytes) {
+    if (!bytes) return fail("rvc_attention_frag_workspace_bytes: null pointer");
+    if (!att_frag_shape_ok(batch, n_frames, n_heads, head_dim) || !att_frag_splits_ok(n_frames, n_splits))
+        return fail("rvc_attention_frag_workspace_bytes: batch > 0, n_heads > 0, n_frames >= 0, head_dim 64, n_splits 0 or 1 .. min(8, key tiles)");
+    const int splits = n_splits ? n_splits : choose_splits_bf(n_frames, n_heads, batch);
+    const size_t rows = splits == 1 ? 0 : (size_t)batch * n_heads * splits * (size_t)n_frames;
+    *bytes = 256 + align_up(rows * 64 * sizeof(float), 256) + align_up(rows * 2 * sizeof(float), 256);
+    return 0;
+}
+
+extern "C" int rvc_attention_frag_bf16x3(const float *q_dev, int64_t q_row_stride, const void *frag_dev, float *out_dev, void *planes_dev,
+                                         int64_t n_rows_padded, int batch, int64_t n_frames, int n_heads, int head_dim, float scale,
+                                         int n_splits, void *workspace_dev, size_t workspace_bytes, void *stream) {
+    const char *who = "rvc_attention_frag_bf16x3";
+    if (!q_dev || !frag_dev) return fail("%s: null pointer", who);
+    if ((out_dev == nullptr) == (planes_dev == nullptr)) return fail("%s: exactly one of out_dev (fp32 rows) and planes_dev (bf16x3 planes)", who);
+    if (!att_frag_shape_ok(batch, n_frames, n_heads, head_dim) || !att_frag_splits_ok(n_frames, n_splits))
+        return fail("%s: batch > 0, n_heads > 0, n_frames >= 0, head_dim 64, n_splits 0 or 1 .. min(8, key tiles)", who);
+    if (q_row_stride < (int64_t)n_heads * 64 || q_row_stride % 4) return fail("%s: q_row_stride must be a multiple of 4 and >= n_heads * 64", who);
+    if (planes_dev && n_rows_padded < (int64_t)batch * n_frames) return fail("%s: n_rows_padded must be >= batch * n_frames", who);
+    if (n_frames == 0) return 0;
+    size_t need = 0;
+    if (rvc_attention_frag_workspace_bytes(batch, n_frames, n_heads, head_dim, n_splits, &need)) return 1;
+    if (!workspace_dev || workspace_bytes < need) return fail("%s: workspace too small (%zu < %zu)", who, workspace_bytes, need);
+    AttBfParams q;
+    q.q = q_dev; q.q_stride = q_row_stride; q.frag = frag_dev; q.out = out_dev; q.planes = (unsigned char *)planes_dev; q.n_pad = n_rows_padded;
+    q.T = n_frames; q.n_heads = n_heads; q.scale_log2e = scale * 1.4426950408889634f;
+    q.n_splits = n_splits ? n_splits : choose_splits_bf(n_frames, n_heads, batch);
+    const size_t rows = q.n_splits == 1 ? 0 : (size_t)batch * n_heads * q.n_splits * (size_t)n_frames;
+    q.part_o = (float *)workspace_dev; q.part_ml = (float *)((char *)workspace_dev + align_up(rows * 64 * sizeof(float), 256));
+    return launch_attention_bf(who, q, batch, nullptr, (hipStream_t)stream);
+}
diff --git a/codename-rvc-fork-3_amd/csrc/bf16x3.h b/codename-rvc-fork-3_amd/csrc/bf16x3.h
--- a/codename-rvc-fork-3_amd/csrc/bf16x3.h
+++ b/codename-rvc-fork-3_amd/csrc/bf16x3.h
@@ -50,4 +50,22 @@
     }
 }
 
+__device__ __forceinline__ float rounded(float v) {
+    asm volatile("" : "+v"(v));
+    return v;
 }
+
+constexpr int ABF_TILE_BYTES = 24 * 1024;
+__device__ __forceinline__ void abf_split8(const float (&v)[8], u32x4 (&out)[3]) {
+    f32x2 r[4] = {f32x2{v[0], v[1]}, f32x2{v[2], v[3]}, f32x2{v[4], v[5]}, f32x2{v[6], v[7]}};
+#pragma unroll
+    for (int level = 0; level < 3; ++level)
+#pragma unroll
+        for (int q = 0; q < 4; ++q) {
+            const unsigned w = split_word(r[q]);
+            out[level][q] = w;
+            if (level < 2) r[q] = r[q] - f32x2{__uint_as_float(w << 16), __uint_as_float(w & 0xffff0000u)};
+        }
+}
+
+}
diff --git a/codename-rvc-fork-3_amd/csrc/linbf.hip b/codename-rvc-fork-3_amd/csrc/linbf.hip
--- a/codename-rvc-fork-3_amd/csrc/linbf.hip
+++ b/codename-rvc-fork-3_amd/csrc/linbf.hip
@@ -19,6 +19,8 @@
     int64_t x_row_stride = 0, x_plane = 0;
     int steps_per_part = 0;
     int n_col_blocks = 0;
+    void *frag = nullptr;
+    int64_t n_tiles = 0;
 };
 
 constexpr int LBF_BN = 128, LBF_NTH = 512;
@@ -137,6 +139,103 @@
         lds_barrier();
     }
 
+    if constexpr (MI == 2) {
+        if (p.mode == 4) {
+            const int dm = p.M / 3;
+            const int sec = m0 / dm;
+            const int64_t n = n0 + nrow;
+            const bool live = n < p.N;
+            const int mw = m0 + wm * 64;
+            if (sec == 0) {
+                if (!live) return;
+#pragma unroll
+                for (int mi = 0; mi < MI; ++mi)
+#pragma unroll
+                    for (int rg = 0; rg < 4; ++rg) {
+                        const int m = mw + mi * 32 + 4 * half + 8 * rg;
+                        f32x4 o;
+#pragma unroll
+                        for (int r = 0; r < 4; ++r) o[r] = acc[mi][4 * rg + r];
+                        if (p.bias) o += *reinterpret_cast<const f32x4 *>(p.bias + m);
+                        *reinterpret_cast<f32x4 *>(p.y + n * dm + m) = o;
+                    }
+                return;
+            }
+            const int64_t tile = (n0 >> 5) + wn;
+            const bool tile_ok = tile < p.n_tiles;
+            const int head = (mw - sec * dm) >> 6;
+            unsigned char *dst = reinterpret_cast<unsigned char *>(p.frag) + ((int64_t)head * p.n_tiles + (tile_ok ? tile : 0)) * ABF_TILE_BYTES + lane * 16;
+            if (sec == 1) {
+                if (!tile_ok) return;
+#pragma unroll
+                for (int mi = 0; mi < MI; ++mi)
+#pragma unroll
+                    for (int rp = 0; rp < 2; ++rp) {
+                        f32x2 v[2][2];
+#pragma unroll
+                        for (int g = 0; g < 2; ++g) {
+                            f32x4 o;
+#pragma unroll
+                            for (int r = 0; r < 4; ++r) o[r] = acc[mi][4 * (2 * rp + g) + r];
+                            if (p.bias) o += *reinterpret_cast<const f32x4 *>(p.bias + mw + mi * 32 + 4 * half + 8 * (2 * rp + g));
+#pragma unroll
+                            for (int r = 0; r < 4; ++r) o[r] = live ? rounded(o[r]) : 0.f;
+                            v[g][0] = f32x2{o[0], o[1]};
+                            v[g][1] = f32x2{o[2], o[3]};
+                        }
+#pragma unroll
+                        for (int sp = 0; sp < 3; ++sp) {
+                            unsigned w[2][2];
+#pragma unroll
+                            for (int g = 0; g < 2; ++g)
+#pragma unroll
+                                for (int h = 0; h < 2; ++h) {
+                                    w[g][h] = split_word(v[g][h]);
+                                    v[g][h] = split_rest(v[g][h], w[g][h]);
+                                }
+                            const unsigned s0 = half ? w[0][0] : w[1][0], s1 = half ? w[0][1] : w[1][1];
+                            const unsigned r0 = (unsigned)__shfl_xor((int)s0, 32, 64), r1 = (unsigned)__shfl_xor((int)s1, 32, 64);
+                            const u32x4 out = half ? u32x4{r0, r1, w[1][0], w[1][1]} : u32x4{w[0][0], w[0][1], r0, r1};
+                            *reinterpret_cast<u32x4 *>(dst + ((2 * mi + rp) * 3 + sp) * 1024) = out;
+                        }
+                    }
+                return;
+            }
+            constexpr int TS = 68;
+            float *ts = reinterpret_cast<float *>(lbf_smem) + wave * (32 * TS);
+#pragma unroll
+            for (int mi = 0; mi < MI; ++mi)
+#pragma unroll
+                for (int rg = 0; rg < 4; ++rg) {
+                    const int ml = mi * 32 + 4 * half + 8 * rg;
+                    f32x4 o;
+#pragma unroll
+                    for (int r = 0; r < 4; ++r) o[r] = acc[mi][4 * rg + r];
+                    if (p.bias) o += *reinterpret_cast<const f32x4 *>(p.bias + mw + ml);
+#pragma unroll
+                    for (int r = 0; r < 4; ++r) o[r] = live ? o[r] : 0.f;
+                    *reinterpret_cast<f32x4 *>(ts + l31 * TS + ml) = o;
+                }
+            __syncthreads();
+            if (!tile_ok) return;
+#pragma unroll
+            for (int db = 0; db < 2; ++db)
+#pragma unroll
+                for (int ks = 0; ks < 2; ++ks) {
+                    float v[8];
+#pragma unroll
+                    for (int e = 0; e < 8; ++e) {
+                        const int r = 8 * ks + e;
+                        v[e] = ts[((r & 3) + 8 * (r >> 2) + 4 * half) * TS + 32 * db + l31];
+                    }
+                    u32x4 d[3];
+                    abf_split8(v, d);
+#pragma unroll
+                    for (int sp = 0; sp < 3; ++sp) *reinterpret_cast<u32x4 *>(dst + (12 + (db * 2 + ks) * 3 + sp) * 1024) = d[sp];
+                }
+            return;
+        }
+    }
     if (p.mode == 1) {
         const int64_t n = n0 + nrow;
         const bool live = n < p.N;
@@ -354,6 +453,27 @@
                           n_rows, n_rows_padded, in_features, out_features, mode, k_parts, stream);
 }
 
+extern "C" int rvc_linear_qkv_frag_bf16x3(const void *xs_dev, const void *a_dev, const float *bias_dev, float *q_dev, void *frag_dev,
+                                          int64_t n_frames, int64_t n_rows_padded, int in_features, int n_heads, int head_dim, void *stream) {
+    const char *who = "rvc_linear_qkv_frag_bf16x3";
+    if (!xs_dev || !a_dev || !q_dev || !frag_dev) return fail("%s: null pointer", who);
+    if (head_dim != 64 || n_heads < 2 || n_heads % 2) return fail("%s: head_dim must be 64 and n_heads even (a block is two heads of one projection)", who);
+    if (in_features < 32 || in_features % 32) return fail("%s: in_features must be a multiple of 32", who);
+    if (n_frames < 0 || n_rows_padded % LBF_BN || n_rows_padded < n_frames) return fail("%s: n_rows_padded must be a multiple of 128 and >= n_frames", who);
+    const int64_t out_features = (int64_t)3 * n_heads * 64;
+    if (!fits_2gib(out_features * in_features, 6) || !fits_2gib(3 * n_rows_padded * in_features, 2) ||
+        !fits_2gib((n_rows_padded + LBF_BN) * in_features, 2) || !fits_2gib((int64_t)n_heads * ceil_div(n_frames, 32), ABF_TILE_BYTES))
+        return fail("%s: an operand exceeds 2 GiB", who);
+    if (n_frames == 0) return 0;
+    LinBfParams p;
+    p.a = a_dev; p.xs = xs_dev; p.bias = bias_dev; p.y = q_dev; p.frag = frag_dev;
+    p.M = (int)out_features; p.K = in_features; p.N = n_frames; p.n_pad = n_rows_padded; p.mode = 4;
+    p.x_row_stride = in_features; p.x_plane = n_rows_padded * in_features;
+    p.steps_per_part = in_features / 16;
+    p.n_tiles = ceil_div(n_frames, 32);
+    return linbf_launch<2>(p, 1, (hipStream_t)stream);
+}
+
 extern "C" int rvc_conv1d_frames_bf16x3(const void *xs_dev, int64_t n_frames_in, int64_t n_frames_in_padded, int channels, int taps,
                                         int stride, const void *a_dev, const float *bias_dev, float *y_dev, void *ys_dev,
                                         int64_t n_frames_out_padded, int out_channels, int mode, void *stream) {
diff --git a/codename-rvc-fork-3_amd/rvc_amd/_native.py b/codename-rvc-fork-3_amd/rvc_amd/_native.py
--- a/codename-rvc-fork-3_amd/rvc_amd/_native.py
+++ b/codename-rvc-fork-3_amd/rvc_amd/_native.py
@@ -70,6 +70,11 @@
     "rvc_attention_workspace_bytes": (c_int, [c_int, c_int64, c_int, c_int, POINTER(c_size_t)]),
     "rvc_attention_qkv_f32": (c_int, [c_void_p, c_void_p, c_void_p, c_void_p, c_int, c_int64, c_int, c_int, c_float,
                                       c_void_p, c_size_t, c_void_p]),
+    "rvc_attention_kv_frag_bytes": (c_int, [c_int, c_int64, c_int, c_int, POINTER(c_size_t)]),
+    "rvc_attention_pack_kv": (c_int, [c_void_p, c_void_p, c_int, c_int64, c_int, c_int, c_void_p]),
+    "rvc_attention_frag_workspace_bytes": (c_int, [c_int, c_int64, c_int, c_int, c_int, POINTER(c_size_t)]),
+    "rvc_attention_frag_bf16x3": (c_int, [c_void_p, c_int64, c_void_p, c_void_p, c_void_p, c_int64, c_int, c_int64, c_int, c_int, c_float,
+                                          c_int, c_void_p, c_size_t, c_void_p]),
     "rvc_bias_relu_add_f32": (c_int, [c_void_p, c_void_p, c_void_p, c_void_p, c_int, c_int, c_int64, c_int, c_void_p]),
     "rvc_gate_tanh_sigmoid_f32": (c_int, [c_void_p, c_void_p, c_int, c_int, c_int64, c_void_p]),
     "rvc_rownorm_gelu_f32": (c_int, [c_void_p, c_void_p, c_void_p, c_void_p, c_int, c_int, c_int64, ctypes.c_float, c_void_p]),
@@ -136,6 +141,7 @@
     "rvc_split_rows_bf16x3": (c_int, [c_void_p, c_void_p, c_int64, c_int64, c_int, c_void_p]),
     "rvc_linear_bf16x3_presplit": (c_int, [c_void_p, c_void_p, c_void_p, c_void_p, c_void_p, c_int64, c_int64, c_int, c_int, c_int, c_int,
                                            c_void_p]),
+    "rvc_linear_qkv_frag_bf16x3": (c_int, [c_void_p, c_void_p, c_void_p, c_void_p, c_void_p, c_int64, c_int64, c_int, c_int, c_int, c_void_p]),
     "rvc_bias_residual_layernorm_bf16x3": (c_int, [c_void_p, c_int, c_void_p, c_void_p, c_void_p, c_void_p, c_float, c_void_p, c_void_p,
                                                    c_int64, c_int64, c_int, c_void_p]),
     "rvc_conv2d_packed_floats": (c_int, [c_int, c_int, c_int, c_int, POINTER(c_size_t)]),
@@ -690,6 +696,53 @@
     return out
 
 
+def _kv_frag_bytes(batch: int, n_frames: int, n_heads: int) -> int:
+    return batch * n_heads * (-(-n_frames // 32)) * 24576
+
+
+def attention_kv_frag_empty(batch: int, n_frames: int, n_heads: int, device, head_dim: int = 64) -> torch.Tensor:
+    device = _cuda_device(device)
+    return torch.empty(_size("rvc_attention_kv_frag_bytes", device, batch, n_frames, n_heads, head_dim), dtype=torch.uint8, device=device)
+
+
+def attention_kv_frag_workspace(batch: int, n_frames: int, n_heads: int, device) -> torch.Tensor:
+    device = _cuda_device(device)
+    nbytes = _kv_frag_bytes(batch, n_frames, n_heads)
+    if nbytes >= 1 << 31:
+        raise NativeError("attention_kv_frag_workspace: the slab must stay below 2 GiB")
+    return _ws.get("attention_kv_frag", nbytes, device)[:nbytes]
+
+
+def attention_pack_kv(qkv: torch.Tensor, n_heads: int, out: torch.Tensor | None = None) -> torch.Tensor:
+    if not (_is_f32_hbm(qkv) and qkv.dim() == 3):
+        raise NativeError("attention_pack_kv wants a contiguous float32 HBM tensor [B, T, 3 * n_heads * 64]")
+    b, t, c = qkv.shape
+    hd = c // (3 * n_heads)
+    frag = out if out is not None else attention_kv_frag_empty(b, t, n_heads, qkv.device, hd)
+    _call("rvc_attention_pack_kv", _device(qkv, frag), qkv.data_ptr(), frag.data_ptr(), b, t, n_heads, hd)
+    return frag
+
+
+def attention_frag(q: torch.Tensor, frag: torch.Tensor, n_heads: int, scale: float, planes: torch.Tensor | None = None,
+                   n_splits: int = 0, q_row_stride: int | None = None) -> torch.Tensor:
+    if not (_is_f32_hbm(q) and q.dim() == 3):
+        raise NativeError("attention_frag wants q as a contiguous float32 HBM tensor [B, T, C]")
+    b, t, c = q.shape
+    stride = c if q_row_stride is None else q_row_stride
+    dev = _device(q, frag, planes)
+    d = n_heads * 64
+    if planes is not None and not (planes.dtype == torch.bfloat16 and planes.dim() == 3 and planes.shape[0] == 3 and planes.shape[2] == d
+                                   and planes.is_contiguous()):
+        raise NativeError(f"attention_frag wants planes as a contiguous bfloat16 tensor [3, rows_padded, {d}]")
+    if frag.numel() * frag.element_size() < _kv_frag_bytes(b, t, n_heads):
+        raise NativeError("attention_frag: the fragment slab is smaller than rvc_attention_kv_frag_bytes()")
+    out = None if planes is not None else torch.empty(b, t, d, dtype=torch.float32, device=dev)
+    ws = _workspace("attention_frag", dev, "rvc_attention_frag_workspace_bytes", b, t, n_heads, 64, n_splits)
+    _call("rvc_attention_frag_bf16x3", dev, q.data_ptr(), stride, frag.data_ptr(), _ptr(out), _ptr(planes),
+          planes.shape[1] if planes is not None else 0, b, t, n_heads, 64, float(scale), n_splits, ws.data_ptr(), ws.numel())
+    return planes if planes is not None else out
+
+
 def bias_relu_add_(x: torch.Tensor, bias: torch.Tensor = None, res: torch.Tensor = None, relu: bool = True) -> torch.Tensor:
     if not (_is_f32_hbm(x) and x.dim() >= 3):
         raise NativeError("bias_relu_add_ wants a contiguous float32 HBM tensor [B, C, ...]")
@@ -984,6 +1037,21 @@
     _call("rvc_linear_bf16x3_presplit", _device(xs, a_packed, bias, y), xs.data_ptr(), a_packed.data_ptr(), _ptr(bias),
           y.data_ptr() if m != 1 else None, y.data_ptr() if m == 1 else None, n_rows, n_pad, in_features, out_features, m, k_parts)
     return y
+
+
+def linear_qkv_frag_bf16x3(xs: torch.Tensor, a_packed: torch.Tensor, bias, n_frames: int, n_heads: int, q: torch.Tensor | None = None,
+                           frag: torch.Tensor | None = None) -> tuple[torch.Tensor, torch.Tensor]:
+    _, n_pad, in_features = xs.shape
+    dev = _device(xs, a_packed, bias, q, frag)
+    if q is None:
+        q = torch.empty((n_frames, n_heads * 64), dtype=torch.float32, device=dev)
+    if frag is None:
+        frag = attention_kv_frag_empty(1, n_frames, n_heads, dev)
+    if q.numel() < n_frames * n_heads * 64 or frag.numel() * frag.element_size() < _kv_frag_bytes(1, n_frames, n_heads):
+        raise NativeError("linear_qkv_frag_bf16x3: an output buffer is too small")
+    _call("rvc_linear_qkv_frag_bf16x3", dev, xs.data_ptr(), a_packed.data_ptr(), _ptr(bias), q.data_ptr(), frag.data_ptr(), n_frames, n_pad,
+          in_features, n_heads, 64)
+    return q, frag
 
 
 def posconv_bf16x3_pack_weight(w: torch.Tensor, groups: int, device) -> torch.Tensor:
diff --git a/codename-rvc-fork-3_amd/rvc_amd/lib/hubert.py b/codename-rvc-fork-3_amd/rvc_amd/lib/hubert.py
--- a/codename-rvc-fork-3_amd/rvc_amd/lib/hubert.py
+++ b/codename-rvc-fork-3_amd/rvc_amd/lib/hubert.py
@@ -19,6 +19,7 @@
         self.native_min_rows = 900
         self.frame_convs = True
         self.native_posconv = True
+        self.fused_attention = True
         self.frame_convs_min_samples = 400
         if state_dict is not None:
             self.load_state_dict(state_dict)
@@ -213,17 +214,26 @@
         d_ff = w["encoder.layers.0.feed_forward.intermediate_dense.weight"].shape[0]
         fs = N.planes_empty(n, d_ff, x.device)
         parts = torch.empty((3, n, d), dtype=torch.float32, device=x.device)
-        qkv = torch.empty((n, 3 * d), dtype=torch.float32, device=x.device)
         x1, x1s = torch.empty_like(x), N.planes_empty(n, d, x.device)
+        fused = self.fused_attention and b == 1 and d == 64 * h and h % 2 == 0 and h * -(-n // 32) * 24576 < 2 ** 31
+        if fused:
+            q = torch.empty((1, n, d), dtype=torch.float32, device=x.device)
+            frag = N.attention_kv_frag_workspace(1, n, h, x.device)
+        else:
+            qkv = torch.empty((n, 3 * d), dtype=torch.float32, device=x.device)
         for i in range(self.n_layers):
             L = f"encoder.layers.{i}"
             if self.consume_layerdrop_rng:
                 torch.rand([])
             a_qkv, a_o, a_1, a_2 = self._lin[i]
             _, bqkv, scale = self._qkv[i]
-            N.linear_bf16x3_presplit(xs, a_qkv, bqkv, n, 3 * d, "f32", out=qkv)
-            a = N.attention_qkv(qkv.view(b, t, 3 * d), h, scale)
-            N.split_rows_bf16x3(a.view(n, d), out=a_s)
+            if fused:
+                N.linear_qkv_frag_bf16x3(xs, a_qkv, bqkv, n, h, q=q, frag=frag)
+                N.attention_frag(q, frag, h, scale, planes=a_s)
+            else:
+                N.linear_bf16x3_presplit(xs, a_qkv, bqkv, n, 3 * d, "f32", out=qkv)
+                a = N.attention_qkv(qkv.view(b, t, 3 * d), h, scale)
+                N.split_rows_bf16x3(a.view(n, d), out=a_s)
             N.linear_bf16x3_presplit(a_s, a_o, None, n, d, "parts", 3, out=parts)
             N.bias_residual_layernorm_bf16x3(parts, w[L + ".attention.out_proj.bias"], x, w[L + ".layer_norm.weight"],
                                              w[L + ".layer_norm.bias"], 1e-5, y=x1, ys=x1s)
diff --git a/include/rvc_amd.h b/include/rvc_amd.h
--- a/include/rvc_amd.h
+++ b/include/rvc_amd.h
@@ -65,6 +65,13 @@
 int rvc_attention_qkv_f32(const float *qkv_dev, const float *emb_rel_k_dev, const float *emb_rel_v_dev, float *out_dev,
                           int batch, int64_t n_frames, int n_heads, int head_dim, float scale, void *workspace_dev,
                           size_t workspace_bytes, void *stream);
+
+int rvc_attention_kv_frag_bytes(int batch, int64_t n_frames, int n_heads, int head_dim, size_t *bytes);
+int rvc_attention_pack_kv(const float *qkv_dev, void *frag_dev, int batch, int64_t n_frames, int n_heads, int head_dim, void *stream);
+int rvc_attention_frag_workspace_bytes(int batch, int64_t n_frames, int n_heads, int head_dim, int n_splits, size_t *bytes);
+int rvc_attention_frag_bf16x3(const float *q_dev, int64_t q_row_stride, const void *frag_dev, float *out_dev, void *planes_dev,
+                              int64_t n_rows_padded, int batch, int64_t n_frames, int n_heads, int head_dim, float scale,
+                              int n_splits, void *workspace_dev, size_t workspace_bytes, void *stream);
 
 int rvc_bias_relu_add_f32(const float *x_dev, const float *bias_dev, const float *res_dev, float *out_dev, int batch,
                           int channels, int64_t inner, int relu, void *stream);
@@ -209,6 +216,8 @@
 int rvc_linear_bf16x3_presplit(const void *xs_dev, const void *a_dev, const float *bias_dev, float *y_dev, void *ys_dev,
                                int64_t n_rows, int64_t n_rows_padded, int in_features, int out_features, int mode, int k_parts,
                                void *stream);
+int rvc_linear_qkv_frag_bf16x3(const void *xs_dev, const void *a_dev, const float *bias_dev, float *q_dev, void *frag_dev,
+                               int64_t n_frames, int64_t n_rows_padded, int in_features, int n_heads, int head_dim, void *stream);
 int rvc_bias_residual_layernorm_bf16x3(const float *parts_dev, int n_parts, const float *bias_dev, const float *res_dev,
                                        const float *gamma_dev, const float *beta_dev, float eps, float *y_dev, void *ys_dev,
                                        int64_t n_rows, int64_t n_rows_padded, int features, void *stream);
```

Result: no change. 61.79 million, median of 4 (+0.6%).
